# SrinivasBaskar1995/DistributedVolunteerComputing

Hardware: AMD Instinct MI355X
Metric: samples/sec GPT-2-small local-SGD (higher is better)
Workload: dtype bf16; 1 GPU; model=gpt2, global_batch=64, per_peer_batch=64, seq_len=1024, parallelism=local-sgd dp1 H=4 allreduce=direct

## Files before the change

distributedvolunteercomputing_amd/config.py:

```python
from __future__ import annotations

import contextlib
import dataclasses
import os
import threading


def _bool(s: str) -> bool:
    return s.strip().lower() in ("1", "true", "yes", "on")


@dataclasses.dataclass
class RuntimeConfig:
    gemm: str = "lib"
    mlp: str = "fused"
    narrow_gemm: str = "lib"
    mlp_grad_fwd: bool = True
    bwd_batch: bool = True
    fc_dgrad_nt: bool = True
    lmhead_dgrad_nt: bool = True
    gemm_fwd: str = "lib"
    dgrad_ps: bool = True
    gemm_wgrad: str = "vcx"
    wgrad_wide: bool = True
    wgrad_ragged: bool = False
    gemm_select: bool = False
    wgrad_big_split_min_m: int = 16384
    async_wgrad: bool = False
    lmhead_chunk: int = 0
    force_reference_ops: bool = False
    tunableop: str = "on"
    tunableop_file: str = ""
    offload_arch: str = "gfx950"
    colour_native: bool = True
    register_source: bool = True
    sink_gpu: bool = True
    resnet_conv1x1: str = "gemm"
    conv_find: bool = True
    resnet_bn: str = "fused"
    bn_layer_ws: bool = True
    conv3x3_wgrad: str = "vcx"
    conv3x3_fwd: str = "vcx"
    engine_batch: int = 2
    resnet_join: bool = True
    resnet_proj_join: bool = True
    gloo_host: str = "127.0.0.1"
    p2p_backend: str = ""
    elastic_debug: bool = False
    elastic_liveness: bool = True
    elastic_stage_joins: str = "gloo"
    uplink_pipeline: str = "relay"
    shared_source_root: str = ""
    store_port_train: int = 29611
    store_port_video: int = 29612
    trace_dir: str = ""
    metrics_dir: str = ""


_ENV = {
    "gemm": ("VCX_GEMM", str),
    "mlp": ("VCX_MLP", str),
    "dgrad_ps": ("VCX_DGRAD_PS", _bool),
    "mlp_grad_fwd": ("VCX_MLP_GRAD_FWD", _bool),
    "bwd_batch": ("VCX_BWD_BATCH", _bool),
    "fc_dgrad_nt": ("VCX_FC_DGRAD_NT", _bool),
    "lmhead_dgrad_nt": ("VCX_LMHEAD_DGRAD_NT", _bool),
    "narrow_gemm": ("VCX_NARROW_GEMM", str),
    "resnet_conv1x1": ("VCX_RESNET_CONV1X1", str),
    "resnet_bn": ("VCX_RESNET_BN", str),
    "resnet_join": ("VCX_RESNET_JOIN", _bool),
    "engine_batch": ("VCX_ENGINE_BATCH", int),
    "conv3x3_wgrad": ("VCX_CONV3X3_WGRAD", str),
    "conv3x3_fwd": ("VCX_CONV3X3_FWD", str),
    "resnet_proj_join": ("VCX_RESNET_PROJ_JOIN", _bool),
    "bn_layer_ws": ("VCX_BN_LAYER_WS", _bool),
    "conv_find": ("VCX_CONV_FIND", _bool),
    "gemm_wgrad": ("VCX_GEMM_WGRAD", str),
    "gemm_fwd": ("VCX_GEMM_FWD", str),
    "wgrad_wide": ("VCX_WGRAD_WIDE", _bool),
    "wgrad_ragged": ("VCX_WGRAD_RAGGED", _bool),
    "gemm_select": ("VCX_GEMM_SELECT", _bool),
    "wgrad_big_split_min_m": ("VCX_WGRAD_BIG_SPLIT_MIN_M", int),
    "async_wgrad": ("VCX_ASYNC_WGRAD", _bool),
    "lmhead_chunk": ("VCX_LMHEAD_CHUNK", int),
    "force_reference_ops": ("VCX_FORCE_REFERENCE_OPS", _bool),
    "tunableop": ("VCX_TUNABLEOP", str),
    "tunableop_file": ("VCX_TUNABLEOP_FILE", str),
    "offload_arch": ("VCX_OFFLOAD_ARCH", str),
    "colour_native": ("VCX_COLOUR_NATIVE", _bool),
    "register_source": ("VCX_REGISTER_SOURCE", _bool),
    "sink_gpu": ("VCX_SINK_GPU", _bool),
    "gloo_host": ("VCX_GLOO_HOST", str),
    "p2p_backend": ("VCX_P2P_BACKEND", str),
    "elastic_debug": ("VCX_ELASTIC_DEBUG", _bool),
    "elastic_liveness": ("VCX_ELASTIC_LIVENESS", _bool),
    "elastic_stage_joins": ("VCX_ELASTIC_STAGE_JOINS", str),
    "uplink_pipeline": ("VCX_UPLINK_PIPELINE", str),
    "shared_source_root": ("VCX_SHARED_SOURCE_ROOT", str),
    "store_port_train": ("VCX_STORE_PORT", int),
    "store_port_video": ("VCX_STORE_PORT", int),
    "trace_dir": ("VCX_TRACE_DIR", str),
    "metrics_dir": ("VCX_METRICS_DIR", str),
}
_CHOICES = {"narrow_gemm": ("lib", "vision"), "conv3x3_wgrad": ("lib", "vcx"), "conv3x3_fwd": ("lib", "vcx"), "gemm": ("lib", "vcx"), "mlp": ("fused", "lib"), "gemm_wgrad": ("lib", "vcx"), "gemm_fwd": ("lib", "vcx"), "tunableop": ("on", "off"), "p2p_backend": ("", "gloo", "nccl"), "elastic_stage_joins": ("gloo", "off"),
            "uplink_pipeline": ("relay", "all", "off")}

_lock = threading.Lock()


def _validate(cfg: RuntimeConfig):
    for k, allowed in _CHOICES.items():
        if getattr(cfg, k) not in allowed:
            raise ValueError(f"config.{k} must be one of {allowed}, not {getattr(cfg, k)!r}")


def from_env(env=None) -> RuntimeConfig:
    env = os.environ if env is None else env
    cfg = RuntimeConfig()
    for field, (var, parse) in _ENV.items():
        if var in env and env[var] != "":
            try:
                setattr(cfg, field, parse(env[var]))
            except ValueError as e:
                raise ValueError(f"{var}={env[var]!r}: {e}") from None
    _validate(cfg)
    return cfg


_CONFIG = from_env()


def get() -> RuntimeConfig:
    return _CONFIG


def update(**kw) -> RuntimeConfig:
    with _lock:
        unknown = set(kw) - {f.name for f in dataclasses.fields(RuntimeConfig)}
        if unknown:
            raise AttributeError(f"unknown config fields: {sorted(unknown)}")
        new = dataclasses.replace(_CONFIG, **kw)
        _validate(new)
        for k, v in kw.items():
            setattr(_CONFIG, k, v)
    return _CONFIG


@contextlib.contextmanager
def override(**kw):
    old = {k: getattr(_CONFIG, k) for k in kw}
    update(**kw)
    try:
        yield _CONFIG
    finally:
        update(**old)


def describe() -> str:
    rows = []
    for f in dataclasses.fields(RuntimeConfig):
        var = _ENV.get(f.name, ("", None))[0]
        rows.append(f"{f.name:24s} {var:28s} {getattr(_CONFIG, f.name)!r}")
    return "\n".join(rows)
```

distributedvolunteercomputing_amd/csrc/bindings.cpp:

```cpp
#include <torch/extension.h>
#include <map>
#include <mutex>
#include <thread>
#include <tuple>
#include <c10/hip/HIPStream.h>
#include <hip/hip_runtime.h>

#include "kernels/vcx_api.h"

namespace {

hipStream_t cur_stream() { return c10::hip::getCurrentHIPStream().stream(); }

#define CHECK_CUDA(x) TORCH_CHECK((x).is_cuda(), #x " must be a GPU tensor")
#define CHECK_CONTIG(x) TORCH_CHECK((x).is_contiguous(), #x " must be contiguous")
#define CHECK_DT(x, dt) TORCH_CHECK((x).scalar_type() == (dt), #x " has wrong dtype ", (x).scalar_type())
#define CHECK_IN(x, dt) \
  CHECK_CUDA(x);        \
  CHECK_CONTIG(x);      \
  CHECK_DT(x, dt)

const auto kBF = at::kBFloat16;
const auto kF = at::kFloat;

void* opt_ptr(const c10::optional<at::Tensor>& t) { return t.has_value() ? t->data_ptr() : nullptr; }

void grad_sumsq(at::Tensor g, at::Tensor ostate) {
  CHECK_IN(g, kBF);
  CHECK_IN(ostate, kF);
  TORCH_CHECK(g.numel() % 8 == 0, "flat buffer length must be a multiple of 8");
  vcx_grad_sumsq(g.data_ptr(), g.numel(), ostate.data_ptr<float>(), cur_stream());
}

void adam_prologue(at::Tensor ostate, double max_norm) {
  CHECK_IN(ostate, kF);
  TORCH_CHECK(ostate.numel() >= 4);
  vcx_adam_prologue(ostate.data_ptr<float>(), (float)max_norm, cur_stream());
}

void adamw_flat(at::Tensor param, at::Tensor grad, at::Tensor master, at::Tensor m, at::Tensor v, int64_t n_decay,
                at::Tensor ostate, double beta1, double beta2, double eps, double wd) {
  CHECK_IN(param, kBF);
  CHECK_IN(grad, kBF);
  CHECK_IN(master, kF);
  CHECK_IN(m, kF);
  CHECK_IN(v, kF);
  CHECK_IN(ostate, kF);
  const int64_t n = param.numel();
  TORCH_CHECK(n % 8 == 0 && grad.numel() == n && master.numel() == n && m.numel() == n && v.numel() == n,
              "adamw_flat: buffers must share a length that is a multiple of 8");
  TORCH_CHECK(n_decay >= 0 && n_decay <= n && n_decay % 8 == 0);
  vcx_adamw_flat(param.data_ptr(), grad.data_ptr(), master.data_ptr<float>(), m.data_ptr<float>(),
                 v.data_ptr<float>(), n, n_decay, ostate.data_ptr<float>(), (float)beta1, (float)beta2, (float)eps,
                 (float)wd, cur_stream());
}

void check_compact(at::Tensor m_code, at::Tensor m_exp, at::Tensor v_half, at::Tensor v_exp, int64_t n,
                   const char* who) {
  CHECK_IN(m_code, at::kByte);
  CHECK_IN(m_exp, at::kByte);
  CHECK_IN(v_half, at::kHalf);
  CHECK_IN(v_exp, at::kByte);
  TORCH_CHECK(n % 32 == 0 && m_code.numel() == n && v_half.numel() == n && m_exp.numel() == n / 32 &&
                  v_exp.numel() == n / 32,
              who, ": a state of n elements (a multiple of 32) has n codes, n halves and n / 32 bytes of each exponent");
}

void adamw_flat_compact(at::Tensor param, at::Tensor grad, at::Tensor master, at::Tensor m_code, at::Tensor m_exp,
                        at::Tensor v_half, at::Tensor v_exp, int64_t n_decay, at::Tensor ostate, double beta1,
                        double beta2, double eps, double wd) {
  CHECK_IN(param, kBF);
  CHECK_IN(grad, kBF);
  CHECK_IN(master, kF);
  CHECK_IN(ostate, kF);
  const int64_t n = param.numel();
  TORCH_CHECK(grad.numel() == n && master.numel() == n, "adamw_flat_compact: buffers must share a length");
  check_compact(m_code, m_exp, v_half, v_exp, n, "adamw_flat_compact");
  TORCH_CHECK(ostate.numel() >= 4);
  TORCH_CHECK(n_decay >= 0 && n_decay <= n && n_decay % 8 == 0);
  vcx_adamw_flat_compact(param.data_ptr(), grad.data_ptr(), master.data_ptr<float>(), m_code.data_ptr<uint8_t>(),
                         m_exp.data_ptr<uint8_t>(), v_half.data_ptr(), v_exp.data_ptr<uint8_t>(), n, n_decay,
                         ostate.data_ptr<float>(), beta1, beta2, (float)eps, (float)wd, cur_stream());
}

void optstate_encode(at::Tensor m, at::Tensor v, at::Tensor m_code, at::Tensor m_exp, at::Tensor v_half,
                     at::Tensor v_exp) {
  CHECK_IN(m, kF);
  CHECK_IN(v, kF);
  const int64_t n = m.numel();
  TORCH_CHECK(v.numel() == n, "optstate_encode: m and v must share a length");
  check_compact(m_code, m_exp, v_half, v_exp, n, "optstate_encode");
  vcx_optstate_encode(m.data_ptr<float>(), v.data_ptr<float>(), m_code.data_ptr<uint8_t>(), m_exp.data_ptr<uint8_t>(),
                      v_half.data_ptr(), v_exp.data_ptr<uint8_t>(), n, cur_stream());
}

void optstate_decode(at::Tensor m_code, at::Tensor m_exp, at::Tensor v_half, at::Tensor v_exp, at::Tensor m,
                     at::Tensor v) {
  CHECK_IN(m, kF);
  CHECK_IN(v, kF);
  const int64_t n = m.numel();
  TORCH_CHECK(v.numel() == n, "optstate_decode: m and v must share a length");
  check_compact(m_code, m_exp, v_half, v_exp, n, "optstate_decode");
  vcx_optstate_decode(m_code.data_ptr<uint8_t>(), m_exp.data_ptr<uint8_t>(), v_half.data_ptr(),
                      v_exp.data_ptr<uint8_t>(), m.data_ptr<float>(), v.data_ptr<float>(), n, cur_stream());
}

void lsgd_delta(at::Tensor master, at::Tensor anchor, at::Tensor delta) {
  CHECK_IN(master, kF);
  CHECK_IN(anchor, kF);
  CHECK_IN(delta, kBF);
  const int64_t n = master.numel();
  TORCH_CHECK(n % 8 == 0 && anchor.numel() == n && delta.numel() == n);
  vcx_lsgd_delta(master.data_ptr<float>(), anchor.data_ptr<float>(), delta.data_ptr(), n, cur_stream());
}

void lsgd_apply(at::Tensor avg, at::Tensor anchor, at::Tensor master, at::Tensor param,
                c10::optional<at::Tensor> mom, double outer_lr, double mu, bool nesterov, double avg_scale) {
  CHECK_IN(avg, kBF);
  CHECK_IN(anchor, kF);
  CHECK_IN(master, kF);
  CHECK_IN(param, kBF);
  const int64_t n = avg.numel();
  TORCH_CHECK(n % 8 == 0 && anchor.numel() == n && master.numel() == n && param.numel() == n);
  if (mom.has_value()) {
    CHECK_IN((*mom), kF);
    TORCH_CHECK(mom->numel() == n);
  }
  vcx_lsgd_apply(avg.data_ptr(), anchor.data_ptr<float>(), master.data_ptr<float>(), param.data_ptr(),
                 mom.has_value() ? mom->data_ptr<float>() : nullptr, n, (float)outer_lr, (float)mu, nesterov ? 1 : 0,
                 (float)avg_scale, cur_stream());
}

void f32_to_bf16(at::Tensor src, at::Tensor dst) {
  CHECK_IN(src, kF);
  CHECK_IN(dst, kBF);
  TORCH_CHECK(src.numel() == dst.numel() && src.numel() % 8 == 0);
  vcx_f32_to_bf16(src.data_ptr<float>(), dst.data_ptr(), src.numel(), cur_stream());
}

bool gemm_nt_supported(int64_t M, int64_t N, int64_t K) { return vcx_gemm_nt_supported((int)M, (int)N, (int)K); }
bool gemm_nt_supported_epi(int64_t M, int64_t N, int64_t K, int64_t epi) {
  return vcx_gemm_nt_supported_epi((int)M, (int)N, (int)K, (int)epi);
}

void gemm_nt(at::Tensor a, at::Tensor b, at::Tensor c, c10::optional<at::Tensor> c2, c10::optional<at::Tensor> bias,
             c10::optional<at::Tensor> colsum, int64_t epi) {
  TORCH_CHECK(a.is_cuda() && a.dim() == 2 && b.dim() == 2 && c.dim() == 2, "gemm_nt: 2-D cuda tensors");
  TORCH_CHECK(a.scalar_type() == at::kBFloat16 && b.scalar_type() == at::kBFloat16 && c.scalar_type() == at::kBFloat16,
              "gemm_nt: bf16 operands");
  TORCH_CHECK(a.stride(1) == 1 && b.stride(1) == 1 && c.stride(1) == 1, "gemm_nt: K-contiguous rows");
  const int64_t M = a.size(0), K = a.size(1), N = b.size(0);
  TORCH_CHECK(b.size(1) == K && c.size(0) == M && c.size(1) == N, "gemm_nt: shape mismatch");
  TORCH_CHECK(vcx_gemm_nt_supported_epi((int)M, (int)N, (int)K, (int)epi),
              "gemm_nt: needs N % 256 == 0, K % 64 == 0, K >= 128, and M % 256 == 0 for epilogues 2/3");
  TORCH_CHECK(a.stride(0) % 8 == 0 && b.stride(0) % 8 == 0 && c.stride(0) % 8 == 0, "gemm_nt: 16-B aligned rows");
  for (const at::Tensor* t : {&a, &b, &c})
    TORCH_CHECK(reinterpret_cast<uintptr_t>(t->data_ptr()) % 16 == 0, "gemm_nt: 16-B aligned base pointers");
  TORCH_CHECK(epi >= 0 && epi <= 4, "gemm_nt: epilogue 0..4");
  void* c2p = nullptr;
  if (epi == 2 || epi == 3) {
    TORCH_CHECK(c2 && c2->sizes() == c.sizes() && c2->strides() == c.strides() && c2->scalar_type() == at::kBFloat16,
                "gemm_nt: epilogue 2/3 needs c2 like c");
    TORCH_CHECK(reinterpret_cast<uintptr_t>(c2->data_ptr()) % 16 == 0, "gemm_nt: 16-B aligned c2");
    c2p = c2->data_ptr();
  }
  const void* bp = nullptr;
  if (epi == 1 || epi == 2 || epi == 4) {
    TORCH_CHECK(bias && bias->numel() == N && bias->is_contiguous() && bias->scalar_type() == at::kBFloat16,
                "gemm_nt: bias [N] bf16");
    bp = bias->data_ptr();
  }
  float* cs = nullptr;
  if (epi == 3) {
    TORCH_CHECK(colsum && colsum->numel() == N && colsum->scalar_type() == at::kFloat && colsum->is_contiguous(),
                "gemm_nt: colsum [N] fp32");
    cs = colsum->data_ptr<float>();
  }
  vcx_gemm_nt(a.data_ptr(), b.data_ptr(), c.data_ptr(), c2p, bp, cs, (int)M, (int)N, (int)K, (int)a.stride(0),
              (int)b.stride(0), (int)c.stride(0), (int)epi, cur_stream());
}


bool gemm_ps_supported(int64_t M, int64_t N, int64_t K, int64_t epi) {
  return vcx_gemm_ps_supported((int)M, (int)N, (int)K, (int)epi);
}

void gemm_ps(at::Tensor a, at::Tensor b, at::Tensor c, c10::optional<at::Tensor> c2, c10::optional<at::Tensor> bias,
             c10::optional<at::Tensor> colsum, int64_t epi, int64_t grid_cap) {
  TORCH_CHECK(a.is_cuda() && a.dim() == 2 && b.dim() == 2 && c.dim() == 2, "gemm_ps: 2-D cuda tensors");
  TORCH_CHECK(a.scalar_type() == at::kBFloat16 && b.scalar_type() == at::kBFloat16 && c.scalar_type() == at::kBFloat16,
              "gemm_ps: bf16 operands");
  TORCH_CHECK(a.stride(1) == 1 && b.stride(1) == 1 && c.stride(1) == 1, "gemm_ps: K-contiguous rows");
  const int64_t M = a.size(0), K = a.size(1), N = b.size(0);
  TORCH_CHECK(b.size(1) == K && c.size(0) == M && c.size(1) == N, "gemm_ps: shape mismatch");
  TORCH_CHECK(vcx_gemm_ps_supported((int)M, (int)N, (int)K, (int)epi),
              "gemm_ps: needs M, N % 256 == 0, K % 128 == 0, K >= 256, epilogue 0 (store), 1 (bias), 2 (bias+GELU), "
              "4 (DGELU + bias grad), 5 (bias+GELU, c = gelu'(pre)) or 6 (c = acc * c2 + bias grad), N <= 16384 with "
              "a bias");
  TORCH_CHECK(a.stride(0) % 8 == 0 && b.stride(0) % 8 == 0 && c.stride(0) % 8 == 0, "gemm_ps: 16-B aligned rows");
  for (const at::Tensor* t : {&a, &b, &c})
    TORCH_CHECK(reinterpret_cast<uintptr_t>(t->data_ptr()) % 16 == 0, "gemm_ps: 16-B aligned base pointers");
  TORCH_CHECK(256 * std::max({a.stride(0), b.stride(0), c.stride(0)}) * 2 < (int64_t(1) << 31), "gemm_ps: rows too long");
  void* c2p = nullptr;
  if (epi == 2 || epi == 4 || epi == 5 || epi == 6) {
    TORCH_CHECK(c2 && c2->sizes() == c.sizes() && c2->strides() == c.strides() && c2->scalar_type() == at::kBFloat16,
                "gemm_ps: epilogues 2/4/5/6 need c2 like c");
    TORCH_CHECK(reinterpret_cast<uintptr_t>(c2->data_ptr()) % 16 == 0, "gemm_ps: 16-B aligned c2");
    c2p = c2->data_ptr();
  }
  const void* bp = nullptr;
  if (epi == 1 || epi == 2 || epi == 5) {
    TORCH_CHECK(bias && bias->numel() == N && bias->is_contiguous() && bias->scalar_type() == at::kBFloat16,
                "gemm_ps: bias [N] bf16");
    TORCH_CHECK(reinterpret_cast<uintptr_t>(bias->data_ptr()) % 16 == 0, "gemm_ps: 16-B aligned bias");
    bp = bias->data_ptr();
  }
  float* cs = nullptr;
  if (epi == 4 || epi == 6) {
    TORCH_CHECK(colsum && colsum->numel() == N && colsum->scalar_type() == at::kFloat && colsum->is_contiguous(),
                "gemm_ps: colsum [N] fp32");
    cs = colsum->data_ptr<float>();
  }
  vcx_gemm_ps(a.data_ptr(), b.data_ptr(), c.data_ptr(), c2p, bp, cs, (int)M, (int)N, (int)K, (int)a.stride(0),
              (int)b.stride(0), (int)c.stride(0), (int)epi, (int)grid_cap, cur_stream());
}

static float* bn_workspace(const at::Tensor& x, int64_t C) {
  static std::mutex mu;
  static auto* cache = new std::map<std::tuple<int, uintptr_t, int64_t, size_t>, at::Tensor>();
  const auto key = std::make_tuple((int)x.get_device(), (uintptr_t)cur_stream(), C,
                                   std::hash<std::thread::id>{}(std::this_thread::get_id()));
  std::lock_guard<std::mutex> lk(mu);
  auto it = cache->find(key);
  if (it == cache->end()) {
    hipStreamCaptureStatus cs = hipStreamCaptureStatusNone;
    TORCH_CHECK(hipStreamIsCapturing(cur_stream(), &cs) == hipSuccess && cs == hipStreamCaptureStatusNone,
                "bn: first call of this width on this stream/thread inside a graph capture; run one eager step first");
    it = cache->emplace(key, at::zeros({2 * C}, x.options().dtype(at::kFloat))).first;
  }
  return it->second.data_ptr<float>();
}

static float* check_layer_ws(const c10::optional<at::Tensor>& lws, const at::Tensor& x, int64_t C) {
  if (!lws || !lws->defined()) return nullptr;
  TORCH_CHECK(lws->is_cuda() && lws->get_device() == x.get_device() && lws->scalar_type() == at::kFloat &&
                  lws->is_contiguous() && lws->numel() == 4 * C, "bn: layer workspace fp32 [4C] on x's device");
  return lws->data_ptr<float>();
}

std::vector<at::Tensor> bn_fwd_train(at::Tensor x, c10::optional<at::Tensor> res, at::Tensor gamma, at::Tensor beta,
                                     c10::optional<at::Tensor> run_mean, c10::optional<at::Tensor> run_var, double eps,
                                     double momentum, bool relu, c10::optional<at::Tensor> nbt,
                                     c10::optional<at::Tensor> layer_ws) {
  TORCH_CHECK(x.is_cuda() && x.is_contiguous() && x.scalar_type() == at::kBFloat16, "bn: x bf16 contiguous NHWC");
  const int64_t C = x.size(-1), R = x.numel() / C;
  TORCH_CHECK(vcx_bn_supported((int)C) && R > 0, "bn: C must be a power of two in 8..2048");
  TORCH_CHECK(gamma.numel() == C && beta.numel() == C && gamma.scalar_type() == at::kBFloat16 &&
                  beta.scalar_type() == at::kBFloat16 && gamma.is_contiguous() && beta.is_contiguous(), "bn: gamma/beta bf16 [C]");
  if (res) TORCH_CHECK(res->sizes() == x.sizes() && res->is_contiguous() && res->scalar_type() == at::kBFloat16, "bn: residual like x");
  void *rm = nullptr, *rv = nullptr;
  int fp32 = 0;
  if (run_mean && run_mean->defined()) {
    TORCH_CHECK(run_var && run_mean->numel() == C && run_var->numel() == C && run_mean->is_contiguous() &&
                    run_var->is_contiguous() && run_mean->scalar_type() == run_var->scalar_type() &&
                    (run_mean->scalar_type() == at::kBFloat16 || run_mean->scalar_type() == at::kFloat), "bn: running stats [C]");
    rm = run_mean->data_ptr();
    rv = run_var->data_ptr();
    fp32 = run_mean->scalar_type() == at::kFloat;
  }
  int64_t* nb = nullptr;
  if (nbt && nbt->defined()) {
    TORCH_CHECK(nbt->is_cuda() && nbt->scalar_type() == at::kLong && nbt->numel() == 1 && nbt->get_device() == x.get_device(),
                "bn: num_batches_tracked int64 [1] on x's device");
    nb = nbt->data_ptr<int64_t>();
  }
  auto f = x.options().dtype(at::kFloat);
  at::Tensor st = at::empty({4, C}, f);
  at::Tensor y = at::empty_like(x);
  at::Tensor mask = relu ? at::empty({R, C / 8}, x.options().dtype(at::kByte)) : at::Tensor();
  float* lws = check_layer_ws(layer_ws, x, C);
  vcx_bn_fwd_train(x.data_ptr(), res ? res->data_ptr() : nullptr, y.data_ptr(), relu ? mask.data_ptr() : nullptr, R,
                   (int)C, gamma.data_ptr(), beta.data_ptr(), rm, rv, fp32, (float)eps, (float)momentum,
                   lws ? lws : bn_workspace(x, C), st[0].data_ptr<float>(), st[1].data_ptr<float>(),
                   st[2].data_ptr<float>(), st[3].data_ptr<float>(), nb, relu ? 1 : 0, lws ? 1 : 0, cur_stream());
  return {y, st[0], st[1], st[2], mask};
}

std::vector<at::Tensor> maxpool3s2_fwd(at::Tensor x) {
  TORCH_CHECK(x.is_cuda() && x.dim() == 4 && x.is_contiguous() && x.scalar_type() == at::kBFloat16 && x.size(3) % 8 == 0 &&
                  x.size(1) >= 1 && x.size(2) >= 1, "maxpool3s2: x bf16 contiguous NHWC, C % 8 == 0");
  const int64_t N = x.size(0), H = x.size(1), W = x.size(2), C = x.size(3);
  TORCH_CHECK(N * H * W * C < (1ll << 40) && H < (1 << 20) && W < (1 << 20), "maxpool3s2: size");
  const int64_t OH = (H - 1) / 2 + 1, OW = (W - 1) / 2 + 1;
  at::Tensor y = at::empty({N, OH, OW, C}, x.options());
  at::Tensor idx = at::empty({N, OH, OW, C}, x.options().dtype(at::kByte));
  vcx_maxpool3s2_fwd(x.data_ptr(), y.data_ptr(), idx.data_ptr(), (int)N, (int)H, (int)W, (int)C, (int)OH, (int)OW,
                     cur_stream());
  return {y, idx};
}

at::Tensor maxpool3s2_bwd(at::Tensor dy, at::Tensor idx, int64_t H, int64_t W) {
  TORCH_CHECK(dy.is_cuda() && dy.dim() == 4 && dy.is_contiguous() && dy.scalar_type() == at::kBFloat16 &&
                  idx.sizes() == dy.sizes() && idx.is_contiguous() && idx.scalar_type() == at::kByte &&
                  idx.get_device() == dy.get_device() && dy.size(3) % 8 == 0, "maxpool3s2_bwd: dy bf16 / idx u8 NHWC alike");
  const int64_t N = dy.size(0), OH = dy.size(1), OW = dy.size(2), C = dy.size(3);
  TORCH_CHECK(OH == (H - 1) / 2 + 1 && OW == (W - 1) / 2 + 1, "maxpool3s2_bwd: input size does not match");
  at::Tensor dx = at::empty({N, H, W, C}, dy.options());
  vcx_maxpool3s2_bwd(dy.data_ptr(), idx.data_ptr(), dx.data_ptr(), (int)N, (int)H, (int)W, (int)C, (int)OH, (int)OW,
                     cur_stream());
  return dx;
}

static void nhwc_check(const at::Tensor& t, const char* what) {
  TORCH_CHECK(t.is_cuda() && t.dim() == 4 && t.is_contiguous() && t.scalar_type() == at::kBFloat16 && t.size(3) % 8 == 0 &&
                  reinterpret_cast<uintptr_t>(t.data_ptr()) % 16 == 0 && t.numel() < (1ll << 40),
              what, ": bf16 contiguous NHWC [N, H, W, C], C % 8 == 0, 16-B aligned");
}

at::Tensor subsample_nhwc(at::Tensor x, int64_t s) {
  nhwc_check(x, "subsample_nhwc");
  TORCH_CHECK(s >= 1 && s <= 8, "subsample_nhwc: stride 1..8");
  const int64_t N = x.size(0), H = x.size(1), W = x.size(2), C = x.size(3);
  at::Tensor y = at::empty({N, (H - 1) / s + 1, (W - 1) / s + 1, C}, x.options());
  if (y.numel()) vcx_subsample_nhwc(x.data_ptr(), y.data_ptr(), (int)N, (int)H, (int)W, (int)C, (int)s, cur_stream());
  return y;
}

void subsample_add_nhwc(at::Tensor full, at::Tensor g, int64_t s) {
  nhwc_check(full, "subsample_add_nhwc");
  nhwc_check(g, "subsample_add_nhwc");
  TORCH_CHECK(s >= 1 && s <= 8 && full.get_device() == g.get_device(), "subsample_add_nhwc: stride 1..8, one device");
  const int64_t N = full.size(0), H = full.size(1), W = full.size(2), C = full.size(3);
  TORCH_CHECK(g.size(0) == N && g.size(1) == (H - 1) / s + 1 && g.size(2) == (W - 1) / s + 1 && g.size(3) == C,
              "subsample_add_nhwc: g must be [N, ceil(H / s), ceil(W / s), C]");
  if (g.numel()) vcx_subsample_add_nhwc(full.data_ptr(), g.data_ptr(), (int)N, (int)H, (int)W, (int)C, (int)s, cur_stream());
}

at::Tensor bcast_hw_nhwc(at::Tensor g, int64_t H, int64_t W, double scale) {
  TORCH_CHECK(g.is_cuda() && g.dim() == 2 && g.is_contiguous() && g.scalar_type() == at::kBFloat16 && g.size(1) % 8 == 0 &&
                  reinterpret_cast<uintptr_t>(g.data_ptr()) % 16 == 0 && H >= 1 && W >= 1,
              "bcast_hw_nhwc: g bf16 contiguous [N, C], C % 8 == 0");
  const int64_t N = g.size(0), C = g.size(1);
  TORCH_CHECK(N * H * W * C < (1ll << 40), "bcast_hw_nhwc: size");
  at::Tensor out = at::empty({N, H, W, C}, g.options());
  if (out.numel()) vcx_bcast_hw_nhwc(g.data_ptr(), out.data_ptr(), (int)N, (int)(H * W), (int)C, (float)scale, cur_stream());
  return out;
}

at::Tensor bn_apply(at::Tensor x, c10::optional<at::Tensor> res, at::Tensor scale, at::Tensor shift, bool relu) {
  TORCH_CHECK(x.is_cuda() && x.is_contiguous() && x.scalar_type() == at::kBFloat16, "bn: x bf16 contiguous NHWC");
  const int64_t C = x.size(-1), R = x.numel() / C;
  TORCH_CHECK(vcx_bn_supported((int)C), "bn: C must be a power of two in 8..2048");
  TORCH_CHECK(scale.numel() == C && shift.numel() == C && scale.scalar_type() == at::kFloat &&
                  shift.scalar_type() == at::kFloat && scale.is_contiguous() && shift.is_contiguous(), "bn: scale/shift fp32 [C]");
  if (res) TORCH_CHECK(res->sizes() == x.sizes() && res->is_contiguous() && res->scalar_type() == at::kBFloat16, "bn: residual like x");
  at::Tensor y = at::empty_like(x);
  vcx_bn_apply(x.data_ptr(), res ? res->data_ptr() : nullptr, y.data_ptr(), R, (int)C, scale.data_ptr<float>(),
               shift.data_ptr<float>(), relu ? 1 : 0, cur_stream());
  return y;
}

std::vector<at::Tensor> bn_bwd(at::Tensor dy, c10::optional<at::Tensor> mask, at::Tensor x, at::Tensor mean, at::Tensor rstd,
                               at::Tensor scale, bool relu, bool want_dres, c10::optional<at::Tensor> gw,
                               c10::optional<at::Tensor> gb, c10::optional<at::Tensor> layer_ws) {
  TORCH_CHECK(dy.is_cuda() && dy.is_contiguous() && x.is_contiguous() && dy.sizes() == x.sizes() &&
                  dy.scalar_type() == at::kBFloat16 && x.scalar_type() == at::kBFloat16, "bn_bwd: dy, x bf16 NHWC alike");
  const int64_t C = x.size(-1), R = x.numel() / C;
  TORCH_CHECK(relu == (mask && mask->defined()), "bn_bwd: the ReLU mask with relu (and only then)");
  if (relu)
    TORCH_CHECK(mask->is_cuda() && mask->is_contiguous() && mask->scalar_type() == at::kByte &&
                    mask->numel() * 8 == R * C && mask->get_device() == x.get_device(), "bn_bwd: mask uint8 [R, C / 8]");
  TORCH_CHECK(vcx_bn_supported((int)C), "bn: C must be a power of two in 8..2048");
  for (const at::Tensor* t : {&mean, &rstd, &scale})
    TORCH_CHECK(t->numel() == C && t->scalar_type() == at::kFloat && t->is_contiguous(), "bn_bwd: stats fp32 [C]");
  const bool flat = gw && gw->defined();
  TORCH_CHECK(flat == (gb && gb->defined()), "bn_bwd: gw and gb together");
  if (flat)
    for (const at::Tensor* t : {&*gw, &*gb})
      TORCH_CHECK(t->is_cuda() && t->get_device() == x.get_device() && t->numel() == C && t->is_contiguous() &&
                      t->scalar_type() == at::kBFloat16, "bn_bwd: gradient buffers bf16 [C]");
  at::Tensor sums = at::empty({2 * C}, x.options().dtype(at::kFloat));
  at::Tensor dx = at::empty_like(x);
  at::Tensor dres = want_dres ? at::empty_like(x) : at::Tensor();
  float* lws = check_layer_ws(layer_ws, x, C);
  vcx_bn_bwd(dy.data_ptr(), relu ? mask->data_ptr() : nullptr, x.data_ptr(), mean.data_ptr<float>(), rstd.data_ptr<float>(),
             scale.data_ptr<float>(), R, (int)C, lws ? lws : bn_workspace(x, C), sums.data_ptr<float>(),
             flat ? gw->data_ptr() : nullptr, flat ? gb->data_ptr() : nullptr, dx.data_ptr(),
             want_dres ? dres.data_ptr() : nullptr, relu ? 1 : 0, lws ? 1 : 0, cur_stream());
  return {dx, dres, sums.narrow(0, C, C), sums.narrow(0, 0, C)};
}

bool gemm_wg_supported(int64_t M, int64_t N, int64_t K, int64_t splits) {
  return vcx_gemm_wg_supported((int)M, (int)N, (int)K, (int)(splits > 0 ? splits : vcx_gemm_wg_splits((int)M, (int)N, (int)K)));
}

void gemm_wg(at::Tensor a, at::Tensor b, at::Tensor out, bool accumulate, int64_t splits, int64_t loaders) {
  TORCH_CHECK(a.is_cuda() && a.dim() == 2 && b.dim() == 2 && out.dim() == 2, "gemm_wg: 2-D cuda tensors");
  TORCH_CHECK(a.scalar_type() == at::kBFloat16 && b.scalar_type() == at::kBFloat16 && out.scalar_type() == at::kBFloat16,
              "gemm_wg: bf16 operands");
  TORCH_CHECK(a.stride(1) == 1 && b.stride(1) == 1 && out.is_contiguous(), "gemm_wg: row-major operands, contiguous out");
  const int64_t K = a.size(0), M = a.size(1), N = b.size(1);
  TORCH_CHECK(b.size(0) == K && out.size(0) == M && out.size(1) == N, "gemm_wg: shape mismatch");
  if (splits <= 0) splits = vcx_gemm_wg_splits((int)M, (int)N, (int)K);
  TORCH_CHECK(vcx_gemm_wg_supported((int)M, (int)N, (int)K, (int)splits),
              "gemm_wg: needs M % 128 == 0, N % 256 == 0, K % 64 == 0, K / 192 >= splits, split panels under 2 GB");
  TORCH_CHECK(loaders == 4 || loaders == 8, "gemm_wg: loaders 4 or 8");
  TORCH_CHECK(a.stride(0) % 8 == 0 && b.stride(0) % 8 == 0, "gemm_wg: 16-B aligned rows");
  const int64_t tok = ((K / 64 + splits - 1) / splits) * 64;
  TORCH_CHECK(tok * std::max(a.stride(0), b.stride(0)) * 2 < (int64_t(1) << 31) - (int64_t(1) << 20),
              "gemm_wg: a split's operand panel must stay under 2 GB (more splits)");
  for (const at::Tensor* t : {&a, &b, &out})
    TORCH_CHECK(reinterpret_cast<uintptr_t>(t->data_ptr()) % 16 == 0, "gemm_wg: 16-B aligned base pointers");
  at::Tensor ws = at::empty({splits, M, N}, a.options().dtype(at::kFloat));
  vcx_gemm_wg(a.data_ptr(), b.data_ptr(), ws.data_ptr<float>(), out.data_ptr(), (int)M, (int)N, (int)K,
              (int)a.stride(0), (int)b.stride(0), (int)splits, accumulate ? 1 : 0, (int)loaders, cur_stream());
}

bool gemm_f_supported(int64_t M, int64_t N, int64_t K) { return vcx_gemm_f_supported((int)M, (int)N, (int)K); }

static std::pair<int, at::Tensor> f_splits(int64_t M, int64_t N, int64_t K, int64_t splits, const at::Tensor& like) {
  if (splits < 0) splits = vcx_gemm_f_splits((int)M, (int)N, (int)K);
  if (splits == 0) splits = 1;
  TORCH_CHECK(vcx_gemm_f_split_ok((int)M, (int)N, (int)K, (int)splits),
              "gemm_f: the K slices (K / 32) must split into even counts >= 6");
  at::Tensor ws = splits > 1 ? at::empty({splits, M, N}, like.options().dtype(at::kFloat)) : at::Tensor();
  return {(int)splits, ws};
}

int64_t gemm_f_splits(int64_t M, int64_t N, int64_t K) { return vcx_gemm_f_splits((int)M, (int)N, (int)K); }

void gemm_f(at::Tensor a, at::Tensor b, at::Tensor out, c10::optional<at::Tensor> bias, int64_t waves, int64_t splits) {
  TORCH_CHECK(a.is_cuda() && a.dim() == 2 && b.dim() == 2 && out.dim() == 2, "gemm_f: 2-D cuda tensors");
  TORCH_CHECK(a.scalar_type() == at::kBFloat16 && b.scalar_type() == at::kBFloat16 && out.scalar_type() == at::kBFloat16,
              "gemm_f: bf16 operands");
  TORCH_CHECK(a.stride(1) == 1 && b.stride(1) == 1 && out.stride(1) == 1, "gemm_f: row-major operands");
  const int64_t M = a.size(0), K = a.size(1), N = b.size(0);
  TORCH_CHECK(b.size(1) == K && out.size(0) == M && out.size(1) == N, "gemm_f: shape mismatch");
  TORCH_CHECK(vcx_gemm_f_supported((int)M, (int)N, (int)K), "gemm_f: needs N % 128 == 0 or N == 64, K % 64 == 0, K >= 192");
  TORCH_CHECK(a.stride(0) % 8 == 0 && b.stride(0) % 8 == 0 && out.stride(0) % 8 == 0, "gemm_f: 16-B aligned rows");
  for (const at::Tensor* t : {&a, &b, &out})
    TORCH_CHECK(reinterpret_cast<uintptr_t>(t->data_ptr()) % 16 == 0, "gemm_f: 16-B aligned base pointers");
  TORCH_CHECK(a.get_device() == b.get_device() && a.get_device() == out.get_device(), "gemm_f: one device");
  const bool hb = bias && bias->defined();
  if (hb)
    TORCH_CHECK(bias->is_cuda() && bias->get_device() == a.get_device() && bias->numel() == N && bias->is_contiguous() &&
                    bias->scalar_type() == at::kBFloat16 && reinterpret_cast<uintptr_t>(bias->data_ptr()) % 8 == 0,
                "gemm_f: bias bf16 [N], contiguous, 8-B aligned");
  TORCH_CHECK(256 * std::max(a.stride(0), b.stride(0)) * 2 < (int64_t(1) << 31), "gemm_f: tile panels under 2 GB");
  auto [ns, ws] = f_splits(M, N, K, splits, a);
  TORCH_CHECK(ns == 1 || out.stride(0) % 4 == 0, "gemm_f: split output rows 8-B aligned");
  vcx_gemm_f(a.data_ptr(), b.data_ptr(), out.data_ptr(), hb ? bias->data_ptr() : nullptr, (int)M, (int)N, (int)K, (int)a.stride(0), (int)b.stride(0),
             (int)out.stride(0), (int)waves, ns, ns > 1 ? ws.data_ptr<float>() : nullptr, cur_stream());
}

bool gemm_f_conv3x3_supported(int64_t imgs, int64_t H, int64_t W, int64_t Cin, int64_t Cout, int64_t stride) {
  return vcx_gemm_f_conv3x3_supported((int)imgs, (int)H, (int)W, (int)Cin, (int)Cout, (int)stride);
}

void gemm_f_conv3x3(at::Tensor x, at::Tensor w, at::Tensor out, int64_t stride, c10::optional<at::Tensor> bias,
                    int64_t waves, int64_t splits, bool flip_taps) {
  TORCH_CHECK(x.is_cuda() && x.dim() == 4 && (w.dim() == 4 || w.dim() == 3) && out.dim() == 4,
              "gemm_f_conv3x3: x [N, H, W, Cin], w [Cout, 3, 3, Cin] or [9, Cout, Cin], out [N, Ho, Wo, Cout] on the GPU");
  for (const at::Tensor* t : {&x, &w, &out}) {
    TORCH_CHECK(t->scalar_type() == at::kBFloat16 && t->is_contiguous() && t->get_device() == x.get_device(),
                "gemm_f_conv3x3: contiguous bf16 tensors on one device");
    TORCH_CHECK(reinterpret_cast<uintptr_t>(t->data_ptr()) % 16 == 0, "gemm_f_conv3x3: 16-B aligned base pointers");
  }
  const bool tap_major = w.dim() == 3;
  const int64_t imgs = x.size(0), H = x.size(1), W = x.size(2), Cin = x.size(3), Cout = tap_major ? w.size(1) : w.size(0);
  TORCH_CHECK(tap_major ? (w.size(0) == 9 && w.size(2) == Cin) : (w.size(1) == 3 && w.size(2) == 3 && w.size(3) == Cin),
              "gemm_f_conv3x3: w [Cout, 3, 3, Cin] or tap-major [9, Cout, Cin]");
  TORCH_CHECK(stride == 1 || stride == 2, "gemm_f_conv3x3: stride 1 or 2");
  const int64_t Ho = (H - 1) / stride + 1, Wo = (W - 1) / stride + 1;
  TORCH_CHECK(out.size(0) == imgs && out.size(1) == Ho && out.size(2) == Wo && out.size(3) == Cout,
              "gemm_f_conv3x3: out [N, Ho, Wo, Cout]");
  TORCH_CHECK(vcx_gemm_f_conv3x3_supported((int)imgs, (int)H, (int)W, (int)Cin, (int)Cout, (int)stride),
              "gemm_f_conv3x3: needs Cin a power of two >= 64, Cout % 128 == 0 or Cout == 64, x under 2 GB");
  const bool hb = bias && bias->defined();
  if (hb)
    TORCH_CHECK(bias->is_cuda() && bias->get_device() == x.get_device() && bias->numel() == Cout &&
                    bias->is_contiguous() && bias->scalar_type() == at::kBFloat16, "gemm_f_conv3x3: bias bf16 [Cout]");
  auto [ns, ws] = f_splits(imgs * Ho * Wo, Cout, 9 * Cin, splits, x);
  vcx_gemm_f_conv3x3(x.data_ptr(), w.data_ptr(), out.data_ptr(), hb ? bias->data_ptr() : nullptr, (int)imgs, (int)H,
                     (int)W, (int)Cin, (int)Cout, (int)stride, (int)waves, ns, ns > 1 ? ws.data_ptr<float>() : nullptr,
                     flip_taps ? 1 : 0, tap_major ? 1 : 0, cur_stream());
}

bool gemm_wg_conv3x3_supported(int64_t Cout, int64_t Cin, int64_t imgs, int64_t H, int64_t W, int64_t stride) {
  if (stride != 1 && stride != 2) return false;
  const int64_t tokens = imgs * ((H - 1) / stride + 1) * ((W - 1) / stride + 1);
  if (tokens >= (int64_t(1) << 31)) return false;
  const int splits = vcx_gemm_wg_splits((int)Cout, (int)(9 * Cin), (int)tokens);
  return vcx_gemm_wg_conv3x3_supported((int)Cout, (int)Cin, (int)tokens, imgs * H * W * Cin * 2, splits);
}

void gemm_wg_conv3x3(at::Tensor dy, at::Tensor x, at::Tensor out, bool accumulate, int64_t stride, int64_t splits) {
  TORCH_CHECK(dy.is_cuda() && x.is_cuda() && out.is_cuda() && dy.dim() == 4 && x.dim() == 4 && out.dim() == 2,
              "gemm_wg_conv3x3: dy [N, Ho, Wo, Cout], x [N, H, W, Cin], out [Cout, 9 Cin] on the GPU");
  TORCH_CHECK(dy.scalar_type() == at::kBFloat16 && x.scalar_type() == at::kBFloat16 && out.scalar_type() == at::kBFloat16,
              "gemm_wg_conv3x3: bf16");
  TORCH_CHECK(dy.is_contiguous() && x.is_contiguous() && out.is_contiguous(), "gemm_wg_conv3x3: contiguous NHWC");
  const int64_t imgs = x.size(0), H = x.size(1), W = x.size(2), Cin = x.size(3), Cout = dy.size(3);
  TORCH_CHECK(stride == 1 || stride == 2, "gemm_wg_conv3x3: stride 1 or 2");
  const int64_t Ho = (H - 1) / stride + 1, Wo = (W - 1) / stride + 1;
  TORCH_CHECK(dy.size(0) == imgs && dy.size(1) == Ho && dy.size(2) == Wo, "gemm_wg_conv3x3: dy / x shapes");
  TORCH_CHECK(out.size(0) == Cout && out.size(1) == 9 * Cin, "gemm_wg_conv3x3: out [Cout, 9 Cin]");
  const int64_t tokens = imgs * Ho * Wo;
  TORCH_CHECK(tokens < (int64_t(1) << 31), "gemm_wg_conv3x3: size");
  if (splits <= 0) splits = vcx_gemm_wg_splits((int)Cout, (int)(9 * Cin), (int)tokens);
  TORCH_CHECK(vcx_gemm_wg_conv3x3_supported((int)Cout, (int)Cin, (int)tokens, imgs * H * W * Cin * 2, (int)splits),
              "gemm_wg_conv3x3: needs Cout % 128 == 0, Cin % 128 == 0, N Ho Wo % 64 == 0, N Ho Wo / 192 >= splits, "
              "x under 2 GB");
  for (const at::Tensor* t : {&dy, &x, &out})
    TORCH_CHECK(reinterpret_cast<uintptr_t>(t->data_ptr()) % 16 == 0, "gemm_wg_conv3x3: 16-B aligned base pointers");
  at::Tensor ws = at::empty({splits, Cout, 9 * Cin}, dy.options().dtype(at::kFloat));
  vcx_gemm_wg_conv3x3(dy.data_ptr(), x.data_ptr(), ws.data_ptr<float>(), out.data_ptr(), (int)Cout, (int)Cin, (int)imgs,
                      (int)H, (int)W, (int)stride, (int)splits, accumulate ? 1 : 0, cur_stream());
}

at::Tensor transpose_bf16(at::Tensor src, c10::optional<at::Tensor> dst) {
  TORCH_CHECK(src.is_cuda() && src.dim() == 2 && src.is_contiguous() && src.scalar_type() == at::kBFloat16,
              "transpose_bf16: contiguous 2-D bf16");
  at::Tensor out = dst ? *dst : at::empty({src.size(1), src.size(0)}, src.options());
  TORCH_CHECK(out.size(0) == src.size(1) && out.size(1) == src.size(0) && out.is_contiguous(), "transpose_bf16: dst");
  vcx_transpose_bf16(src.data_ptr(), out.data_ptr(), (int)src.size(0), (int)src.size(1), cur_stream());
  return out;
}

std::tuple<std::vector<at::Tensor>, int64_t> transpose_bf16_many(std::vector<at::Tensor> srcs,
                                                                 c10::optional<std::vector<at::Tensor>> dsts) {
  TORCH_CHECK(!dsts || dsts->size() == srcs.size(), "transpose_bf16_many: one dst per src");
  std::vector<at::Tensor> outs;
  std::vector<vcx::TransposeJob> jobs;
  outs.reserve(srcs.size());
  jobs.reserve(srcs.size());
  for (size_t i = 0; i < srcs.size(); ++i) {
    const at::Tensor& src = srcs[i];
    TORCH_CHECK(src.is_cuda() && src.dim() == 2 && src.is_contiguous() && src.scalar_type() == at::kBFloat16 &&
                    src.get_device() == srcs[0].get_device() && src.size(0) <= INT32_MAX && src.size(1) <= INT32_MAX,
                "transpose_bf16_many: contiguous 2-D bf16 on one device");
    at::Tensor out = dsts ? (*dsts)[i] : at::empty({src.size(1), src.size(0)}, src.options());
    TORCH_CHECK(out.dim() == 2 && out.size(0) == src.size(1) && out.size(1) == src.size(0) && out.is_contiguous() &&
                    out.scalar_type() == at::kBFloat16 && out.is_cuda() && out.get_device() == src.get_device(),
                "transpose_bf16_many: dst");
    vcx::TransposeJob j{};
    j.src = src.data_ptr();
    j.dst = out.data_ptr();
    j.R = (int)src.size(0);
    j.Cc = (int)src.size(1);
    jobs.push_back(j);
    outs.push_back(std::move(out));
  }
  int launches = 0;
  if (!jobs.empty()) {
    launches = vcx_transpose_bf16_many(jobs.data(), (int)jobs.size(), cur_stream());
    TORCH_CHECK(launches >= 0, "transpose_bf16_many: a matrix of more than 2^31 tiles");
  }
  return {std::move(outs), (int64_t)launches};
}

void add_f32_into_bf16(at::Tensor in, at::Tensor out, bool accumulate, bool zero_in) {
  TORCH_CHECK(in.is_cuda() && in.scalar_type() == at::kFloat && out.scalar_type() == at::kBFloat16 &&
                  in.numel() == out.numel() && in.is_contiguous() && out.is_contiguous() &&
                  in.get_device() == out.get_device() && in.numel() < (int64_t(1) << 31),
              "add_f32_into_bf16: fp32 in, bf16 out of equal size on one device");
  vcx_add_f32_into_bf16(in.data_ptr<float>(), out.data_ptr(), (int)in.numel(), accumulate ? 1 : 0, zero_in ? 1 : 0,
                        cur_stream());
}

void reduce_bcast_bf16(at::Tensor in, c10::optional<at::Tensor> out, c10::optional<at::Tensor> mine, int64_t P) {
  TORCH_CHECK(in.is_cuda() && in.scalar_type() == at::kBFloat16 && in.is_contiguous(), "reduce_bcast: bf16 cuda in");
  const int64_t n = in.numel() / P;
  TORCH_CHECK(P > 0 && n * P == in.numel() && n % 8 == 0, "reduce_bcast: numel must be P * n with n % 8 == 0");
  if (out) TORCH_CHECK(out->numel() == in.numel() && out->is_contiguous() && out->scalar_type() == at::kBFloat16,
                       "reduce_bcast: out must match in");
  if (mine) TORCH_CHECK(mine->numel() == n && mine->is_contiguous() && mine->scalar_type() == at::kBFloat16,
                        "reduce_bcast: mine must hold n bf16");
  vcx_reduce_bcast_bf16(in.data_ptr(), opt_ptr(out), opt_ptr(mine), (int)P, n, cur_stream());
}

int64_t check_robust_rows(const char* who, const at::Tensor& in, int64_t P, int64_t live_mask,
                          const c10::optional<at::Tensor>& out, const c10::optional<at::Tensor>& mine) {
  TORCH_CHECK(in.is_cuda() && in.scalar_type() == at::kBFloat16 && in.is_contiguous(), who,
              ": in must be a contiguous bf16 GPU tensor");
  TORCH_CHECK(P >= 1 && P <= 16, who, ": P must be in 1..16, got ", P);
  TORCH_CHECK(live_mask > 0 && (live_mask >> P) == 0, who,
              ": live_mask must name at least one of the P rows and no other, got ", live_mask);
  const int64_t n = in.numel() / P;
  TORCH_CHECK(n * P == in.numel() && n % 8 == 0, who, ": numel must be P * n with n % 8 == 0");
  auto aligned = [](const at::Tensor& t, uintptr_t a) { return reinterpret_cast<uintptr_t>(t.data_ptr()) % a == 0; };
  TORCH_CHECK(aligned(in, 16), who, ": in must be 16-byte aligned");
  if (out)
    TORCH_CHECK(out->is_cuda() && out->get_device() == in.get_device() && out->numel() == in.numel() &&
                    out->is_contiguous() && out->scalar_type() == at::kBFloat16 && aligned(*out, 16),
                who, ": out must match in (bf16, same length, 16-byte aligned)");
  if (mine)
    TORCH_CHECK(mine->is_cuda() && mine->get_device() == in.get_device() && mine->numel() == n &&
                    mine->is_contiguous() && mine->scalar_type() == at::kBFloat16 && aligned(*mine, 16),
                who, ": mine must hold n bf16, 16-byte aligned");
  return n;
}

void trimmed_reduce_bcast_bf16(at::Tensor in, c10::optional<at::Tensor> out, c10::optional<at::Tensor> mine, int64_t P,
                               int64_t trim, int64_t live_mask, double inv, c10::optional<at::Tensor> counts) {
  const int64_t n = check_robust_rows("trimmed_reduce_bcast", in, P, live_mask, out, mine);
  TORCH_CHECK(trim >= 0, "trimmed_reduce_bcast: trim must be >= 0");
  if (counts)
    TORCH_CHECK(counts->is_cuda() && counts->get_device() == in.get_device() && counts->numel() == P &&
                    counts->is_contiguous() && counts->scalar_type() == at::kLong,
                "trimmed_reduce_bcast: counts must hold P int64 on in's device");
  vcx_trimmed_reduce_bcast_bf16(in.data_ptr(), opt_ptr(out), opt_ptr(mine), (int)P, n, (int)std::min<int64_t>(trim, 16),
                                (uint32_t)live_mask, (float)inv, counts ? counts->data_ptr<int64_t>() : nullptr,
                                cur_stream());
}

void cclip_reduce_bcast_bf16(at::Tensor in, c10::optional<at::Tensor> out, c10::optional<at::Tensor> mine, int64_t P,
                             int64_t live_mask, double tau, int64_t iters, c10::optional<at::Tensor> weights) {
  const int64_t n = check_robust_rows("cclip_reduce_bcast", in, P, live_mask, out, mine);
  TORCH_CHECK(tau >= 0.0 && tau <= 3.4028234663852886e38,
              "cclip_reduce_bcast: tau must be finite and >= 0 (0: adaptive), got ", tau);
  TORCH_CHECK(iters >= 1 && iters <= 8, "cclip_reduce_bcast: iters must be in 1..8, got ", iters);
  if (weights)
    TORCH_CHECK(weights->is_cuda() && weights->get_device() == in.get_device() && weights->numel() == P &&
                    weights->is_contiguous() && weights->scalar_type() == at::kFloat,
                "cclip_reduce_bcast: weights must hold P fp32 on in's device");
  at::Tensor ws = at::empty({vcx_cclip_workspace_floats((int)P, n)}, in.options().dtype(at::kFloat));
  vcx_cclip_reduce_bcast_bf16(in.data_ptr(), opt_ptr(out), opt_ptr(mine), (int)P, n, (uint32_t)live_mask, (float)tau,
                              (int)iters, weights ? weights->data_ptr<float>() : nullptr, ws.data_ptr<float>(),
                              cur_stream());
}

void axpy_bf16(at::Tensor src, at::Tensor acc, double scale) {
  CHECK_IN(src, kBF);
  CHECK_IN(acc, kBF);
  TORCH_CHECK(src.numel() == acc.numel() && src.numel() % 8 == 0);
  vcx_axpy_bf16(src.data_ptr(), acc.data_ptr(), src.numel(), (float)scale, cur_stream());
}

void splitk_reduce(at::Tensor part, at::Tensor acc, bool accumulate) {
  CHECK_IN(part, kBF);
  CHECK_IN(acc, kBF);
  const int64_t n = acc.numel();
  TORCH_CHECK(n % 8 == 0 && part.numel() % n == 0, "splitk_reduce: part must be [S, acc.numel()], numel % 8 == 0");
  vcx_splitk_reduce(part.data_ptr(), acc.data_ptr(), (int)(part.numel() / n), n, accumulate ? 1 : 0, cur_stream());
}

std::vector<at::Tensor> ln_fwd(at::Tensor a, c10::optional<at::Tensor> b, at::Tensor w, c10::optional<at::Tensor> bias,
                               double eps, bool rms, c10::optional<at::Tensor> bb) {
  CHECK_IN(a, kBF);
  CHECK_IN(w, kBF);
  const int C = (int)a.size(-1);
  const int64_t R = a.numel() / C;
  TORCH_CHECK(C % 8 == 0 && C <= 8192, "layernorm: C must be a multiple of 8 and <= 8192");
  TORCH_CHECK(w.numel() == C);
  TORCH_CHECK(R < INT32_MAX);
  if (b.has_value()) {
    CHECK_IN((*b), kBF);
    TORCH_CHECK(b->sizes() == a.sizes());
  }
  if (bias.has_value()) {
    CHECK_IN((*bias), kBF);
    TORCH_CHECK(bias->numel() == C);
  }
  if (bb.has_value()) {
    CHECK_IN((*bb), kBF);
    TORCH_CHECK(bb->numel() == C && b.has_value(), "branch bias needs a branch tensor");
  }
  auto y = at::empty_like(a);
  at::Tensor xout = b.has_value() ? at::empty_like(a) : a;
  auto mean = at::empty({R}, a.options().dtype(kF));
  auto rstd = at::empty({R}, a.options().dtype(kF));
  vcx_ln_fwd(a.data_ptr(), opt_ptr(b), b.has_value() ? xout.data_ptr() : nullptr, y.data_ptr(), w.data_ptr(),
             opt_ptr(bias), mean.data_ptr<float>(), rstd.data_ptr<float>(), (int)R, C, (float)eps, rms ? 1 : 0,
             opt_ptr(bb), cur_stream());
  return {y, xout, mean, rstd};
}

at::Tensor grad_out(const c10::optional<at::Tensor>& given, int64_t n, const at::Tensor& like, int* mask, int bit) {
  if (given.has_value()) {
    CHECK_IN((*given), kBF);
    TORCH_CHECK(given->numel() == n, "gradient output has the wrong size");
    *mask |= 1 << bit;
    return *given;
  }
  return at::empty({n}, like.options());
}

std::vector<at::Tensor> ln_bwd(at::Tensor dy, at::Tensor x, at::Tensor w, at::Tensor mean, at::Tensor rstd,
                               c10::optional<at::Tensor> dres, bool has_bias, bool rms, bool has_bb,
                               c10::optional<at::Tensor> dw_out, c10::optional<at::Tensor> db_out,
                               c10::optional<at::Tensor> dbb_out) {
  CHECK_IN(dy, kBF);
  CHECK_IN(x, kBF);
  CHECK_IN(w, kBF);
  CHECK_IN(mean, kF);
  CHECK_IN(rstd, kF);
  const int C = (int)x.size(-1);
  const int64_t R = x.numel() / C;
  TORCH_CHECK(C % 8 == 0 && C <= 8192 && dy.sizes() == x.sizes() && w.numel() == C);
  TORCH_CHECK(mean.numel() == R && rstd.numel() == R);
  if (dres.has_value()) {
    CHECK_IN((*dres), kBF);
    TORCH_CHECK(dres->sizes() == x.sizes());
  }
  const int P = vcx_ln_bwd_partials((int)R, C);
  auto dx = at::empty_like(x);
  auto dw_part = at::empty({P, C}, x.options().dtype(kF));
  int mask = 0;
  at::Tensor dw = grad_out(dw_out, C, x, &mask, 0);
  at::Tensor db_part, db;
  if (has_bias) {
    db_part = at::empty({P, C}, x.options().dtype(kF));
    db = grad_out(db_out, C, x, &mask, 1);
  }
  at::Tensor dbb_part, dbb;
  if (has_bb) {
    dbb_part = at::empty({P, C}, x.options().dtype(kF));
    dbb = grad_out(dbb_out, C, x, &mask, 2);
  }
  vcx_ln_bwd(dy.data_ptr(), x.data_ptr(), w.data_ptr(), mean.data_ptr<float>(), rstd.data_ptr<float>(),
             opt_ptr(dres), dx.data_ptr(), dw_part.data_ptr<float>(), has_bias ? db_part.data_ptr<float>() : nullptr,
             dw.data_ptr(), has_bias ? db.data_ptr() : nullptr, (int)R, C, rms ? 1 : 0,
             has_bb ? dbb_part.data_ptr<float>() : nullptr, has_bb ? dbb.data_ptr() : nullptr,
             at::empty({3 * VCX_COLSUM_NB * C}, x.options().dtype(kF)).data_ptr<float>(), mask, cur_stream());
  return {dx, dw, db, dbb};
}

at::Tensor colsum_bf16(at::Tensor y, c10::optional<at::Tensor> out) {
  CHECK_IN(y, kBF);
  const int64_t F = y.size(-1), R = y.numel() / F;
  TORCH_CHECK(F % 8 == 0 && R > 0 && R < INT32_MAX, "colsum_bf16: last dim must be a multiple of 8");
  int mask = 0;
  at::Tensor o = grad_out(out, F, y, &mask, 0);
  auto part = at::empty({vcx_bias_gelu_partials((int)R), F}, y.options().dtype(kF));
  auto stage = at::empty({VCX_COLSUM_NB * F}, y.options().dtype(kF));
  vcx_colsum_bf16(y.data_ptr(), part.data_ptr<float>(), o.data_ptr(), (int)R, (int)F, mask, stage.data_ptr<float>(),
                  cur_stream());
  return o;
}

at::Tensor bias_gelu_fwd(at::Tensor x, at::Tensor b) {
  CHECK_IN(x, kBF);
  CHECK_IN(b, kBF);
  const int64_t F = x.size(-1), R = x.numel() / F;
  TORCH_CHECK(F % 8 == 0 && b.numel() == F && R < INT32_MAX);
  auto y = at::empty_like(x);
  vcx_bias_gelu_fwd(x.data_ptr(), b.data_ptr(), y.data_ptr(), (int)R, (int)F, cur_stream());
  return y;
}

std::vector<at::Tensor> bias_gelu_bwd(at::Tensor x, at::Tensor b, at::Tensor dy, c10::optional<at::Tensor> db_out) {
  CHECK_IN(x, kBF);
  CHECK_IN(b, kBF);
  CHECK_IN(dy, kBF);
  const int64_t F = x.size(-1), R = x.numel() / F;
  TORCH_CHECK(F % 8 == 0 && b.numel() == F && dy.sizes() == x.sizes() && R < INT32_MAX);
  auto dx = at::empty_like(x);
  auto part = at::empty({vcx_bias_gelu_partials((int)R), F}, x.options().dtype(kF));
  int mask = 0;
  auto db = grad_out(db_out, F, x, &mask, 0);
  auto stage = at::empty({VCX_COLSUM_NB * F}, x.options().dtype(kF));
  vcx_bias_gelu_bwd(x.data_ptr(), b.data_ptr(), dy.data_ptr(), dx.data_ptr(), part.data_ptr<float>(), db.data_ptr(),
                    (int)R, (int)F, stage.data_ptr<float>(), mask, cur_stream());
  return {dx, db};
}

at::Tensor gelu_fwd(at::Tensor x) {
  CHECK_IN(x, kBF);
  TORCH_CHECK(x.numel() % 8 == 0);
  auto y = at::empty_like(x);
  vcx_gelu_fwd(x.data_ptr(), y.data_ptr(), x.numel(), cur_stream());
  return y;
}

at::Tensor gelu_bwd(at::Tensor x, at::Tensor dy) {
  CHECK_IN(x, kBF);
  CHECK_IN(dy, kBF);
  TORCH_CHECK(x.numel() % 8 == 0 && dy.numel() == x.numel());
  auto dx = at::empty_like(x);
  vcx_gelu_bwd(x.data_ptr(), dy.data_ptr(), dx.data_ptr(), x.numel(), cur_stream());
  return dx;
}

at::Tensor swiglu_fwd(at::Tensor gu) {
  CHECK_IN(gu, kBF);
  const int64_t F2 = gu.size(-1);
  TORCH_CHECK(F2 % 16 == 0, "swiglu: feature dim must be a multiple of 16");
  const int64_t R = gu.numel() / F2;
  auto sizes = gu.sizes().vec();
  sizes.back() = F2 / 2;
  auto y = at::empty(sizes, gu.options());
  vcx_swiglu_fwd(gu.data_ptr(), y.data_ptr(), R, (int)(F2 / 2), cur_stream());
  return y;
}

at::Tensor swiglu_bwd(at::Tensor gu, at::Tensor dy) {
  CHECK_IN(gu, kBF);
  CHECK_IN(dy, kBF);
  const int64_t F2 = gu.size(-1);
  TORCH_CHECK(F2 % 16 == 0 && dy.numel() * 2 == gu.numel());
  auto dgu = at::empty_like(gu);
  vcx_swiglu_bwd(gu.data_ptr(), dy.data_ptr(), dgu.data_ptr(), gu.numel() / F2, (int)(F2 / 2), cur_stream());
  return dgu;
}

std::vector<at::Tensor> xent_fwd(at::Tensor logits, at::Tensor tgt, int64_t V) {
  CHECK_IN(logits, kBF);
  CHECK_IN(tgt, at::kLong);
  TORCH_CHECK(logits.dim() == 2);
  const int64_t R = logits.size(0), Vp = logits.size(1);
  TORCH_CHECK(Vp % 8 == 0 && V <= Vp && V > 0 && tgt.numel() == R);
  auto lse = at::empty({R}, logits.options().dtype(kF));
  auto loss = at::empty({R}, logits.options().dtype(kF));
  vcx_xent_fwd(logits.data_ptr(), tgt.data_ptr<int64_t>(), lse.data_ptr<float>(), loss.data_ptr<float>(), R, (int)V,
               (int)Vp, cur_stream());
  return {loss, lse};
}

void xent_bwd(at::Tensor logits, at::Tensor tgt, at::Tensor lse, at::Tensor gscale, at::Tensor dlogits, int64_t V) {
  CHECK_IN(logits, kBF);
  CHECK_IN(tgt, at::kLong);
  CHECK_IN(lse, kF);
  CHECK_IN(gscale, kF);
  CHECK_IN(dlogits, kBF);
  const int64_t R = logits.size(0), Vp = logits.size(1);
  TORCH_CHECK(logits.dim() == 2 && dlogits.sizes() == logits.sizes() && tgt.numel() == R && lse.numel() == R);
  TORCH_CHECK(Vp % 8 == 0 && V <= Vp && gscale.numel() >= 1);
  vcx_xent_bwd(logits.data_ptr(), tgt.data_ptr<int64_t>(), lse.data_ptr<float>(), gscale.data_ptr<float>(),
               dlogits.data_ptr(), R, (int)V, (int)Vp, cur_stream());
}

c10::optional<at::Tensor> xent_fused(at::Tensor logits, at::Tensor tgt, at::Tensor nvalid, int64_t V) {
  CHECK_IN(logits, kBF);
  CHECK_IN(tgt, at::kLong);
  CHECK_IN(nvalid, kF);
  TORCH_CHECK(logits.dim() == 2);
  const int64_t R = logits.size(0), Vp = logits.size(1);
  TORCH_CHECK(Vp % 8 == 0 && V <= Vp && V > 0 && tgt.numel() == R && nvalid.numel() >= 1);
  auto loss = at::empty({R}, logits.options().dtype(kF));
  if (!vcx_xent_fused(logits.data_ptr(), tgt.data_ptr<int64_t>(), nvalid.data_ptr<float>(), loss.data_ptr<float>(), R,
                      (int)V, (int)Vp, cur_stream()))
    return c10::nullopt;
  return loss;
}

void xent_rescale(at::Tensor d, at::Tensor dloss) {
  CHECK_IN(d, kBF);
  CHECK_IN(dloss, kF);
  TORCH_CHECK(d.numel() % 8 == 0 && dloss.numel() >= 1);
  vcx_xent_rescale(d.data_ptr(), dloss.data_ptr<float>(), d.numel(), cur_stream());
}

at::Tensor embed_fwd(at::Tensor idx, at::Tensor wte, c10::optional<at::Tensor> wpe, int64_t T) {
  CHECK_IN(idx, at::kLong);
  CHECK_IN(wte, kBF);
  TORCH_CHECK(wte.dim() == 2 && wte.size(1) % 8 == 0);
  const int64_t R = idx.numel(), V = wte.size(0), C = wte.size(1);
  TORCH_CHECK(T > 0 && R % T == 0);
  if (wpe.has_value()) {
    CHECK_IN((*wpe), kBF);
    TORCH_CHECK(wpe->dim() == 2 && wpe->size(1) == C && wpe->size(0) >= T, "position table too short");
  }
  auto out = at::empty({R, C}, wte.options());
  vcx_embed_fwd(idx.data_ptr<int64_t>(), wte.data_ptr(), opt_ptr(wpe), out.data_ptr(), R, (int)T, (int)C, (int)V,
                cur_stream());
  return out;
}

std::vector<at::Tensor> embed_bwd(at::Tensor idx, at::Tensor dx, int64_t V, int64_t T, int64_t Tpos,
                                  c10::optional<at::Tensor> wte_grad, c10::optional<at::Tensor> wpe_grad) {
  CHECK_IN(idx, at::kLong);
  CHECK_IN(dx, kBF);
  const int64_t R = idx.numel(), C = dx.size(-1);
  TORCH_CHECK(dx.numel() == R * C && C % 8 == 0 && C <= 8192 && T > 0 && R % T == 0 && Tpos >= 0 && Tpos >= (Tpos ? T : 0));
  auto scratch = at::zeros({V, C}, dx.options().dtype(kF));
  at::Tensor dwte, dwpe;
  int acc_wte = 0, acc_wpe = 0;
  if (wte_grad.has_value()) {
    CHECK_IN((*wte_grad), kBF);
    TORCH_CHECK(wte_grad->numel() == V * C);
    dwte = *wte_grad;
    acc_wte = 1;
  } else {
    dwte = at::empty({V, C}, dx.options());
  }
  if (Tpos > 0) {
    if (wpe_grad.has_value()) {
      CHECK_IN((*wpe_grad), kBF);
      TORCH_CHECK(wpe_grad->numel() == Tpos * C);
      dwpe = *wpe_grad;
      acc_wpe = 1;
    } else {
      dwpe = at::zeros({Tpos, C}, dx.options());
    }
  }
  vcx_embed_bwd(idx.data_ptr<int64_t>(), dx.data_ptr(), scratch.data_ptr<float>(), dwte.data_ptr(), acc_wte,
                Tpos > 0 ? dwpe.data_ptr() : nullptr, acc_wpe, R, (int)T, (int)C, (int)V, cur_stream());
  return {dwte, dwpe};
}

std::vector<at::Tensor> rope_qkv_fwd(at::Tensor qkv, at::Tensor cosv, at::Tensor sinv, int64_t Hq, int64_t Hkv) {
  CHECK_IN(qkv, kBF);
  CHECK_IN(cosv, kF);
  CHECK_IN(sinv, kF);
  TORCH_CHECK(qkv.dim() == 3, "rope_qkv: qkv must be [B, T, (Hq + 2 Hkv) * D]");
  const int64_t B = qkv.size(0), T = qkv.size(1), W = qkv.size(2);
  TORCH_CHECK(Hq > 0 && Hkv > 0 && W % (Hq + 2 * Hkv) == 0);
  const int64_t D = W / (Hq + 2 * Hkv);
  TORCH_CHECK(D % 8 == 0, "rope_qkv: head dim must be a multiple of 8");
  TORCH_CHECK(cosv.dim() == 2 && cosv.size(0) >= T && cosv.size(1) == D / 2 && sinv.sizes() == cosv.sizes(),
              "rope_qkv: cos/sin tables must be [>= T, D/2]");
  auto q = at::empty({B, Hq, T, D}, qkv.options());
  auto k = at::empty({B, Hkv, T, D}, qkv.options());
  auto v = at::empty({B, Hkv, T, D}, qkv.options());
  vcx_rope_qkv(qkv.data_ptr(), q.data_ptr(), k.data_ptr(), v.data_ptr(), cosv.data_ptr<float>(),
               sinv.data_ptr<float>(), (int)B, (int)T, (int)Hq, (int)Hkv, (int)D, 0, cur_stream());
  return {q, k, v};
}

at::Tensor rope_qkv_bwd(at::Tensor dq, at::Tensor dk, at::Tensor dv, at::Tensor cosv, at::Tensor sinv) {
  CHECK_IN(dq, kBF);
  CHECK_IN(dk, kBF);
  CHECK_IN(dv, kBF);
  CHECK_IN(cosv, kF);
  CHECK_IN(sinv, kF);
  TORCH_CHECK(dq.dim() == 4 && dk.dim() == 4 && dk.sizes() == dv.sizes());
  const int64_t B = dq.size(0), Hq = dq.size(1), T = dq.size(2), D = dq.size(3), Hkv = dk.size(1);
  TORCH_CHECK(dk.size(0) == B && dk.size(2) == T && dk.size(3) == D && D % 8 == 0);
  TORCH_CHECK(cosv.size(0) >= T && cosv.size(1) == D / 2 && sinv.sizes() == cosv.sizes());
  auto dqkv = at::empty({B, T, (Hq + 2 * Hkv) * D}, dq.options());
  vcx_rope_qkv(dqkv.data_ptr(), dq.data_ptr(), dk.data_ptr(), dv.data_ptr(), cosv.data_ptr<float>(),
               sinv.data_ptr<float>(), (int)B, (int)T, (int)Hq, (int)Hkv, (int)D, 1, cur_stream());
  return dqkv;
}

std::vector<at::Tensor> attn_fwd(at::Tensor qkv, double scale) {
  CHECK_IN(qkv, kBF);
  TORCH_CHECK(qkv.dim() == 5 && qkv.size(2) == 3 && qkv.size(4) == 64, "attn_fwd: qkv must be [B, T, 3, H, 64]");
  const int64_t B = qkv.size(0), T = qkv.size(1), H = qkv.size(3);
  TORCH_CHECK(B * H * ((T + 127) / 128) < INT32_MAX && T > 0);
  auto out = at::empty({B, T, H, 64}, qkv.options());
  auto lse = at::empty({B, H, T}, qkv.options().dtype(kF));
  vcx_attn_fwd_d64(qkv.data_ptr(), out.data_ptr(), lse.data_ptr<float>(), (int)B, (int)T, (int)H, (float)scale,
                   cur_stream());
  return {out, lse};
}

at::Tensor attn_bwd(at::Tensor qkv, at::Tensor out, at::Tensor dout, at::Tensor lse, double scale) {
  CHECK_IN(qkv, kBF);
  CHECK_IN(out, kBF);
  CHECK_IN(dout, kBF);
  CHECK_IN(lse, kF);
  TORCH_CHECK(qkv.dim() == 5 && qkv.size(2) == 3 && qkv.size(4) == 64);
  const int64_t B = qkv.size(0), T = qkv.size(1), H = qkv.size(3);
  TORCH_CHECK(out.sizes() == at::IntArrayRef({B, T, H, 64}) && dout.sizes() == out.sizes());
  TORCH_CHECK(lse.numel() == B * H * T);
  auto dqkv = at::empty_like(qkv);
  auto delta = at::empty({B, H, T}, lse.options());
  vcx_attn_bwd_d64(qkv.data_ptr(), out.data_ptr(), dout.data_ptr(), lse.data_ptr<float>(), delta.data_ptr<float>(),
                   dqkv.data_ptr(), nullptr, (int)B, (int)T, (int)H, (float)scale, cur_stream());
  return dqkv;
}

std::vector<at::Tensor> attn_bwd_bias(at::Tensor qkv, at::Tensor out, at::Tensor dout, at::Tensor lse, double scale,
                                      c10::optional<at::Tensor> db_out) {
  CHECK_IN(qkv, kBF);
  CHECK_IN(out, kBF);
  CHECK_IN(dout, kBF);
  CHECK_IN(lse, kF);
  TORCH_CHECK(qkv.dim() == 5 && qkv.size(2) == 3 && qkv.size(4) == 64);
  const int64_t B = qkv.size(0), T = qkv.size(1), H = qkv.size(3), F = 3 * H * 64;
  TORCH_CHECK(out.sizes() == at::IntArrayRef({B, T, H, 64}) && dout.sizes() == out.sizes());
  TORCH_CHECK(lse.numel() == B * H * T);
  auto dqkv = at::empty_like(qkv);
  auto delta = at::empty({B, H, T}, lse.options());
  const int P = vcx_attn_bias_partials((int)B, (int)T);
  auto part = at::empty({P, F}, lse.options());
  int mask = 0;
  at::Tensor db = grad_out(db_out, F, qkv, &mask, 0);
  auto stage = at::empty({VCX_COLSUM_NB * F}, lse.options());
  vcx_attn_bwd_d64(qkv.data_ptr(), out.data_ptr(), dout.data_ptr(), lse.data_ptr<float>(), delta.data_ptr<float>(),
                   dqkv.data_ptr(), part.data_ptr<float>(), (int)B, (int)T, (int)H, (float)scale, cur_stream());
  vcx_colsum_f32(part.data_ptr<float>(), db.data_ptr(), P, (int)F, mask, stage.data_ptr<float>(), cur_stream());
  return {dqkv, db};
}

static void check_hm(const at::Tensor& q, const at::Tensor& k, const at::Tensor& v) {
  CHECK_IN(q, kBF);
  CHECK_IN(k, kBF);
  CHECK_IN(v, kBF);
  TORCH_CHECK(q.dim() == 4 && k.dim() == 4 && k.sizes() == v.sizes(), "attn_hm: q [B,Hq,T,D], k/v [B,Hkv,T,D]");
  TORCH_CHECK(q.size(0) == k.size(0) && q.size(2) == k.size(2) && q.size(3) == k.size(3));
  TORCH_CHECK(q.size(3) == 64 || q.size(3) == 128, "attn_hm: head dim must be 64 or 128");
  TORCH_CHECK(q.size(1) % k.size(1) == 0, "attn_hm: Hq must be a multiple of Hkv");
}

std::vector<at::Tensor> attn_hm_fwd(at::Tensor q, at::Tensor k, at::Tensor v, double scale) {
  check_hm(q, k, v);
  const int64_t B = q.size(0), Hq = q.size(1), T = q.size(2), D = q.size(3), Hkv = k.size(1);
  auto out = at::empty({B, T, Hq, D}, q.options());
  auto lse = at::empty({B, Hq, T}, q.options().dtype(kF));
  vcx_attn_hm_fwd(q.data_ptr(), k.data_ptr(), v.data_ptr(), out.data_ptr(), lse.data_ptr<float>(), (int)B, (int)T,
                  (int)Hq, (int)Hkv, (int)D, (float)scale, cur_stream());
  return {out, lse};
}

std::vector<at::Tensor> attn_hm_bwd(at::Tensor q, at::Tensor k, at::Tensor v, at::Tensor out, at::Tensor dout,
                                    at::Tensor lse, double scale) {
  check_hm(q, k, v);
  CHECK_IN(out, kBF);
  CHECK_IN(dout, kBF);
  CHECK_IN(lse, kF);
  const int64_t B = q.size(0), Hq = q.size(1), T = q.size(2), D = q.size(3), Hkv = k.size(1);
  TORCH_CHECK(out.sizes() == at::IntArrayRef({B, T, Hq, D}) && dout.sizes() == out.sizes());
  TORCH_CHECK(lse.numel() == B * Hq * T);
  auto dq = at::empty_like(q), dk = at::empty_like(k), dv = at::empty_like(v);
  auto delta = at::empty({B, Hq, T}, lse.options());
  vcx_attn_hm_bwd(q.data_ptr(), k.data_ptr(), v.data_ptr(), out.data_ptr(), dout.data_ptr(), lse.data_ptr<float>(),
                  delta.data_ptr<float>(), dq.data_ptr(), dk.data_ptr(), dv.data_ptr(), (int)B, (int)T, (int)Hq,
                  (int)Hkv, (int)D, (float)scale, cur_stream());
  return {dq, dk, dv};
}

}

void vcx_register_vision(pybind11::module& m);
void vcx_register_compress(pybind11::module& m);
void vcx_register_lt(pybind11::module& m);
extern "C" const char* vcx_source_digest();

PYBIND11_MODULE(_C, m) {
  m.doc() = "gfx950 HIP kernels of distributedvolunteercomputing_amd";
  m.def("source_digest", [] { return std::string(vcx_source_digest()); });
  m.def("grad_sumsq", &grad_sumsq);
  m.def("adam_prologue", &adam_prologue);
  m.def("adamw_flat", &adamw_flat);
  m.def("adamw_flat_compact", &adamw_flat_compact);
  m.def("optstate_encode", &optstate_encode);
  m.def("optstate_decode", &optstate_decode);
  m.def("lsgd_delta", &lsgd_delta);
  m.def("lsgd_apply", &lsgd_apply);
  m.def("f32_to_bf16", &f32_to_bf16);
  m.def("axpy_bf16", &axpy_bf16);
  m.def("reduce_bcast_bf16", &reduce_bcast_bf16);
  m.def("trimmed_reduce_bcast_bf16", &trimmed_reduce_bcast_bf16);
  m.def("cclip_reduce_bcast_bf16", &cclip_reduce_bcast_bf16);
  m.def("cclip_max_workgroups", &vcx_cclip_max_workgroups);
  m.def("gemm_nt_supported", &gemm_nt_supported);
  m.def("gemm_nt_supported_epi", &gemm_nt_supported_epi);
  m.def("gemm_ps_supported", &gemm_ps_supported);
  m.def("bn_supported", [](int64_t C) { return vcx_bn_supported((int)C); });
  m.def("bn_fwd_train", &bn_fwd_train, py::arg("x"), py::arg("res"), py::arg("gamma"), py::arg("beta"),
        py::arg("run_mean"), py::arg("run_var"), py::arg("eps"), py::arg("momentum"), py::arg("relu"),
        py::arg("nbt") = py::none(), py::arg("layer_ws") = py::none());
  m.def("bn_apply", &bn_apply);
  m.def("maxpool3s2_fwd", &maxpool3s2_fwd);
  m.def("maxpool3s2_bwd", &maxpool3s2_bwd);
  m.def("bn_bwd", &bn_bwd, py::arg("dy"), py::arg("mask"), py::arg("x"), py::arg("mean"), py::arg("rstd"), py::arg("scale"),
        py::arg("relu"), py::arg("want_dres"), py::arg("gw") = py::none(), py::arg("gb") = py::none(),
        py::arg("layer_ws") = py::none());
  m.def("gemm_ps", &gemm_ps, py::arg("a"), py::arg("b"), py::arg("c"), py::arg("c2") = py::none(),
        py::arg("bias") = py::none(), py::arg("colsum") = py::none(), py::arg("epi") = 0, py::arg("grid_cap") = 0);
  m.def("gemm_f_supported", &gemm_f_supported, py::arg("M"), py::arg("N"), py::arg("K"));
  m.def("gemm_f_conv3x3_supported", &gemm_f_conv3x3_supported, py::arg("imgs"), py::arg("H"), py::arg("W"),
        py::arg("Cin"), py::arg("Cout"), py::arg("stride"));
  m.def("gemm_f_conv3x3", &gemm_f_conv3x3, py::arg("x"), py::arg("w"), py::arg("out"), py::arg("stride"),
        py::arg("bias") = py::none(), py::arg("waves") = 0, py::arg("splits") = -1, py::arg("flip_taps") = false);
  m.def("gemm_f_splits", &gemm_f_splits, py::arg("M"), py::arg("N"), py::arg("K"));
  m.def("gemm_f", &gemm_f, py::arg("a"), py::arg("b"), py::arg("out"), py::arg("bias") = py::none(),
        py::arg("waves") = 0, py::arg("splits") = -1);
  m.def("gemm_wg_supported", &gemm_wg_supported, py::arg("M"), py::arg("N"), py::arg("K"), py::arg("splits") = 0);
  m.def("gemm_wg_conv3x3_supported", &gemm_wg_conv3x3_supported, py::arg("Cout"), py::arg("Cin"), py::arg("imgs"),
        py::arg("H"), py::arg("W"), py::arg("stride"));
  m.def("gemm_wg_conv3x3", &gemm_wg_conv3x3, py::arg("dy"), py::arg("x"), py::arg("out"), py::arg("accumulate") = false,
        py::arg("stride") = 1, py::arg("splits") = 0);
  m.def("gemm_wg", &gemm_wg, py::arg("a"), py::arg("b"), py::arg("out"), py::arg("accumulate") = false,
        py::arg("splits") = 0, py::arg("loaders") = 8);
  m.def("gemm_nt", &gemm_nt, py::arg("a"), py::arg("b"), py::arg("c"), py::arg("c2") = py::none(),
        py::arg("bias") = py::none(), py::arg("colsum") = py::none(), py::arg("epi") = 0);
  m.def("transpose_bf16", &transpose_bf16, py::arg("src"), py::arg("dst") = py::none());
  m.def("transpose_bf16_many", &transpose_bf16_many, py::arg("srcs"), py::arg("dsts") = py::none());
  m.attr("JOB_TABLE_CAP") = (int64_t)vcx::JOBS_MAX;
  m.def("subsample_nhwc", &subsample_nhwc, py::arg("x"), py::arg("stride"));
  m.def("subsample_add_nhwc", &subsample_add_nhwc, py::arg("full"), py::arg("g"), py::arg("stride"));
  m.def("bcast_hw_nhwc", &bcast_hw_nhwc, py::arg("g"), py::arg("H"), py::arg("W"), py::arg("scale"));
  m.def("add_f32_into_bf16", &add_f32_into_bf16, py::arg("src"), py::arg("out"), py::arg("accumulate"),
        py::arg("zero_src") = false);
  m.def("splitk_reduce", &splitk_reduce);
  m.def("ln_fwd", &ln_fwd);
  m.def("ln_bwd", &ln_bwd, pybind11::arg("dy"), pybind11::arg("x"), pybind11::arg("w"), pybind11::arg("mean"),
        pybind11::arg("rstd"), pybind11::arg("dres"), pybind11::arg("has_bias"), pybind11::arg("rms"),
        pybind11::arg("has_bb"), pybind11::arg("dw_out") = pybind11::none(), pybind11::arg("db_out") = pybind11::none(),
        pybind11::arg("dbb_out") = pybind11::none());
  m.def("colsum_bf16", &colsum_bf16, pybind11::arg("y"), pybind11::arg("out") = pybind11::none());
  m.def("gelu_fwd", &gelu_fwd);
  m.def("bias_gelu_fwd", &bias_gelu_fwd);
  m.def("bias_gelu_bwd", &bias_gelu_bwd, pybind11::arg("x"), pybind11::arg("b"), pybind11::arg("dy"),
        pybind11::arg("db_out") = pybind11::none());
  m.def("gelu_bwd", &gelu_bwd);
  m.def("swiglu_fwd", &swiglu_fwd);
  m.def("swiglu_bwd", &swiglu_bwd);
  m.def("xent_fwd", &xent_fwd);
  m.def("xent_bwd", &xent_bwd);
  m.def("xent_fused", &xent_fused);
  m.def("xent_rescale", &xent_rescale);
  m.def("embed_fwd", &embed_fwd);
  m.def("embed_bwd", &embed_bwd, pybind11::arg("idx"), pybind11::arg("dx"), pybind11::arg("V"), pybind11::arg("T"),
        pybind11::arg("Tpos"), pybind11::arg("wte_grad") = pybind11::none(), pybind11::arg("wpe_grad") = pybind11::none());
  m.def("attn_fwd", &attn_fwd);
  m.def("attn_set_variant", &vcx_attn_set_variant, pybind11::arg("fwd_wpe"), pybind11::arg("fwd_dma"),
        pybind11::arg("bwd_dma"), pybind11::arg("stage_epi") = -1);
  m.def("rope_qkv_fwd", &rope_qkv_fwd);
  m.def("rope_qkv_bwd", &rope_qkv_bwd);
  m.def("attn_bwd", &attn_bwd);
  m.def("attn_hm_fwd", &attn_hm_fwd);
  m.def("attn_hm_bwd", &attn_hm_bwd);
  m.def("attn_hm_set_variant", &vcx_attn_hm_set_variant);
  m.def("attn_bwd_bias", &attn_bwd_bias, pybind11::arg("qkv"), pybind11::arg("out"), pybind11::arg("dout"),
        pybind11::arg("lse"), pybind11::arg("scale"), pybind11::arg("db_out") = pybind11::none());
  vcx_register_vision(m);
  vcx_register_compress(m);
  vcx_register_lt(m);
}
```

distributedvolunteercomputing_amd/csrc/kernels/norm_act.hip:

```cpp
#include <algorithm>
#include <cstdlib>
#include <type_traits>

#include "vcx_api.h"
#include "vcx_common.h"

namespace vcx {

template <int CH>
__global__ void __launch_bounds__(256) ln_fwd_kernel(const bf16* __restrict__ a, const bf16* __restrict__ b,
                                                      bf16* __restrict__ xout, bf16* __restrict__ y,
                                                      const bf16* __restrict__ w, const bf16* __restrict__ bias,
                                                      float* __restrict__ mean_out, float* __restrict__ rstd_out,
                                                      int R, int C, float eps, int rms, const bf16* __restrict__ bb) {
  const int lane = threadIdx.x & 63;
  const int row = blockIdx.x * 4 + (threadIdx.x >> 6);
  if (row >= R) return;
  const int C8 = C >> 3;
  const int64_t off = (int64_t)row * C;
  float v[CH][8];
  float sum = 0.f;
#pragma unroll
  for (int k = 0; k < CH; ++k) {
    const int c = lane + k * 64;
    if (c < C8) {
      bf16x8 av = *(const bf16x8*)(a + off + c * 8);
      if (b) {
        bf16x8 bv = *(const bf16x8*)(b + off + c * 8);
        bf16x8 s;
        float bias_b[8] = {0.f, 0.f, 0.f, 0.f, 0.f, 0.f, 0.f, 0.f};
        if (bb) {
          bf16x8 t = *(const bf16x8*)(bb + c * 8);
#pragma unroll
          for (int j = 0; j < 8; ++j) bias_b[j] = (float)t[j];
        }
#pragma unroll
        for (int j = 0; j < 8; ++j) {
          s[j] = (bf16)((float)av[j] + ((float)bv[j] + bias_b[j]));
          v[k][j] = (float)s[j];
        }
        *(bf16x8*)(xout + off + c * 8) = s;
      } else {
#pragma unroll
        for (int j = 0; j < 8; ++j) v[k][j] = (float)av[j];
      }
#pragma unroll
      for (int j = 0; j < 8; ++j) sum += v[k][j];
    }
  }
  const float invC = 1.f / (float)C;
  float mean = rms ? 0.f : wave_sum(sum) * invC;
  float var = 0.f;
#pragma unroll
  for (int k = 0; k < CH; ++k) {
    const int c = lane + k * 64;
    if (c < C8) {
#pragma unroll
      for (int j = 0; j < 8; ++j) {
        float d = v[k][j] - mean;
        var = fmaf(d, d, var);
      }
    }
  }
  var = wave_sum(var) * invC;
  const float rstd = rsqrtf(var + eps);
#pragma unroll
  for (int k = 0; k < CH; ++k) {
    const int c = lane + k * 64;
    if (c < C8) {
      bf16x8 wv = *(const bf16x8*)(w + c * 8);
      bf16x8 o;
      if (bias) {
        bf16x8 bv = *(const bf16x8*)(bias + c * 8);
#pragma unroll
        for (int j = 0; j < 8; ++j) o[j] = (bf16)fmaf((v[k][j] - mean) * rstd, (float)wv[j], (float)bv[j]);
      } else {
#pragma unroll
        for (int j = 0; j < 8; ++j) o[j] = (bf16)((v[k][j] - mean) * rstd * (float)wv[j]);
      }
      *(bf16x8*)(y + off + c * 8) = o;
    }
  }
  if (lane == 0) {
    mean_out[row] = mean;
    rstd_out[row] = rstd;
  }
}

template <int Q>
__global__ void __launch_bounds__(256) ln_fwd4_kernel(const bf16* __restrict__ a, const bf16* __restrict__ b,
                                                       bf16* __restrict__ xout, bf16* __restrict__ y,
                                                       const bf16* __restrict__ w, const bf16* __restrict__ bias,
                                                       float* __restrict__ mean_out, float* __restrict__ rstd_out,
                                                       int R, int C, float eps, int rms, const bf16* __restrict__ bb) {
  const int lane = threadIdx.x & 63;
  const int nw = gridDim.x * 4, gw = blockIdx.x * 4 + (threadIdx.x >> 6);
  float wv[Q][4], bv_[Q][4], bbv[Q][4];
#pragma unroll
  for (int k = 0; k < Q; ++k) {
    const int c = k * 256 + lane * 4;
    const bf16x4 t = *(const bf16x4*)(w + c);
    const bf16x4 u = bias ? *(const bf16x4*)(bias + c) : bf16x4{};
    const bf16x4 v = bb ? *(const bf16x4*)(bb + c) : bf16x4{};
#pragma unroll
    for (int j = 0; j < 4; ++j) {
      wv[k][j] = (float)t[j];
      bv_[k][j] = bias ? (float)u[j] : 0.f;
      bbv[k][j] = bb ? (float)v[j] : 0.f;
    }
  }
  const float invC = 1.f / (float)C;
  bf16x4 av[Q], bvv[Q];
  auto load_row = [&](int row, bf16x4(&aa)[Q], bf16x4(&bbx)[Q]) {
    const int64_t off = (int64_t)row * C + lane * 4;
#pragma unroll
    for (int k = 0; k < Q; ++k) {
      aa[k] = *(const bf16x4*)(a + off + k * 256);
      if (b) bbx[k] = *(const bf16x4*)(b + off + k * 256);
    }
  };
  if (gw < R) load_row(gw, av, bvv);
  for (int row = gw; row < R; row += nw) {
    bf16x4 nav[Q], nbv[Q];
    const int nxt = row + nw;
    if (nxt < R) load_row(nxt, nav, nbv);
    const int64_t off = (int64_t)row * C + lane * 4;
    float v[Q][4];
    float sum = 0.f;
#pragma unroll
    for (int k = 0; k < Q; ++k) {
      if (b) {
        bf16x4 sres;
#pragma unroll
        for (int j = 0; j < 4; ++j) {
          sres[j] = (bf16)((float)av[k][j] + ((float)bvv[k][j] + bbv[k][j]));
          v[k][j] = (float)sres[j];
        }
        *(bf16x4*)(xout + off + k * 256) = sres;
      } else {
#pragma unroll
        for (int j = 0; j < 4; ++j) v[k][j] = (float)av[k][j];
      }
#pragma unroll
      for (int j = 0; j < 4; ++j) sum += v[k][j];
    }
    const float mean = rms ? 0.f : wave_sum(sum) * invC;
    float var = 0.f;
#pragma unroll
    for (int k = 0; k < Q; ++k)
#pragma unroll
      for (int j = 0; j < 4; ++j) {
        const float d = v[k][j] - mean;
        var = fmaf(d, d, var);
      }
    const float rstd = rsqrtf(wave_sum(var) * invC + eps);
#pragma unroll
    for (int k = 0; k < Q; ++k) {
      bf16x4 o;
#pragma unroll
      for (int j = 0; j < 4; ++j) o[j] = (bf16)fmaf((v[k][j] - mean) * rstd, wv[k][j], bv_[k][j]);
      *(bf16x4*)(y + off + k * 256) = o;
    }
    if (lane == 0) {
      mean_out[row] = mean;
      rstd_out[row] = rstd;
    }
#pragma unroll
    for (int k = 0; k < Q; ++k) {
      av[k] = nav[k];
      if (b) bvv[k] = nbv[k];
    }
  }
}

template <int CH, bool RES, int VEC>
__global__ void __launch_bounds__(256) __attribute__((amdgpu_waves_per_eu(VEC == 4 ? 3 : 1))) ln_bwd_kernel(const bf16* __restrict__ dy, const bf16* __restrict__ x,
                                                      const bf16* __restrict__ w, const float* __restrict__ mean_in,
                                                      const float* __restrict__ rstd_in,
                                                      const bf16* __restrict__ dres, bf16* __restrict__ dx,
                                                      float* __restrict__ dw_part, float* __restrict__ db_part,
                                                      int R, int C, int rms, float* __restrict__ dbb_part) {
  const int lane = threadIdx.x & 63;
  const int gw = blockIdx.x * 4 + (threadIdx.x >> 6);
  const int nw = gridDim.x * 4;
  using BV = std::conditional_t<VEC == 8, bf16x8, bf16x4>;
  const int C8 = C / VEC;
  const float invC = 1.f / (float)C;
  float dwacc[CH][VEC], dbacc[CH][VEC], wreg[CH][VEC], dxacc[CH][VEC];
#pragma unroll
  for (int k = 0; k < CH; ++k) {
    const int c = lane + k * 64;
#pragma unroll
    for (int j = 0; j < VEC; ++j) {
      dwacc[k][j] = 0.f;
      dbacc[k][j] = 0.f;
      wreg[k][j] = 0.f;
      dxacc[k][j] = 0.f;
    }
    if (c < C8) {
      BV wv = *(const BV*)(w + c * VEC);
#pragma unroll
      for (int j = 0; j < VEC; ++j) wreg[k][j] = (float)wv[j];
    }
  }
  BV cd[CH], cx[CH], cr[CH];
  float cmean = 0.f, crstd = 0.f;
  auto load = [&](int row, BV(&d)[CH], BV(&xv)[CH], BV(&rv)[CH], float& mu, float& rs) {
    const int64_t off = (int64_t)row * C;
    mu = mean_in[row];
    rs = rstd_in[row];
#pragma unroll
    for (int k = 0; k < CH; ++k) {
      const int c = lane + k * 64;
      if (c < C8) {
        d[k] = *(const BV*)(dy + off + c * VEC);
        xv[k] = *(const BV*)(x + off + c * VEC);
        if (RES) rv[k] = *(const BV*)(dres + off + c * VEC);
      }
    }
  };
  if (gw < R) load(gw, cd, cx, cr, cmean, crstd);
  for (int row = gw; row < R; row += nw) {
    BV nd[CH], nx[CH], nr[CH];
    float nmean = 0.f, nrstd = 0.f;
    if (row + nw < R) load(row + nw, nd, nx, nr, nmean, nrstd);
    const int64_t off = (int64_t)row * C;
    float s1 = 0.f, s2 = 0.f;
#pragma unroll
    for (int k = 0; k < CH; ++k) {
      const int c = lane + k * 64;
      if (c < C8) {
#pragma unroll
        for (int j = 0; j < VEC; ++j) {
          const float d = (float)cd[k][j];
          const float xh = ((float)cx[k][j] - cmean) * crstd;
          const float g = d * wreg[k][j];
          s1 += g;
          s2 = fmaf(g, xh, s2);
          dwacc[k][j] = fmaf(d, xh, dwacc[k][j]);
          dbacc[k][j] += d;
        }
      }
    }
    s1 = rms ? 0.f : wave_sum(s1) * invC;
    s2 = wave_sum(s2) * invC;
    const float k2 = crstd * crstd * s2, mk2 = cmean * k2;
#pragma unroll
    for (int k = 0; k < CH; ++k) {
      const int c = lane + k * 64;
      if (c < C8) {
        BV o;
#pragma unroll
        for (int j = 0; j < VEC; ++j) {
          const float gs = fmaf((float)cd[k][j], wreg[k][j], -s1);
          const float v = fmaf(crstd, gs, -fmaf((float)cx[k][j], k2, -mk2)) + (RES ? (float)cr[k][j] : 0.f);
          o[j] = (bf16)v;
          dxacc[k][j] += v;
        }
        *(BV*)(dx + off + c * VEC) = o;
      }
    }
#pragma unroll
    for (int k = 0; k < CH; ++k) {
      cd[k] = nd[k];
      cx[k] = nx[k];
      if (RES) cr[k] = nr[k];
    }
    cmean = nmean;
    crstd = nrstd;
  }
  if constexpr (CH * VEC <= 32) {
    __shared__ __attribute__((aligned(16))) float red[4][CH * 64 * VEC];
    const int w = threadIdx.x >> 6;
    auto reduce_out = [&](float(&acc)[CH][VEC], float* part) {
#pragma unroll
      for (int k = 0; k < CH; ++k) {
        const int c = lane + k * 64;
        if (c < C8) {
#pragma unroll
          for (int j = 0; j < VEC; j += 4)
            *(f32x4*)(&red[w][c * VEC + j]) = f32x4{acc[k][j], acc[k][j + 1], acc[k][j + 2], acc[k][j + 3]};
        }
      }
      __syncthreads();
      for (int i = threadIdx.x; i < C; i += 256)
        part[(int64_t)blockIdx.x * C + i] = (red[0][i] + red[1][i]) + (red[2][i] + red[3][i]);
      __syncthreads();
    };
    reduce_out(dwacc, dw_part);
    if (db_part) reduce_out(dbacc, db_part);
    if (dbb_part) reduce_out(dxacc, dbb_part);
  } else {
    static_assert(VEC == 8, "per-wave partial rows are written as 8-column chunks");
#pragma unroll
    for (int k = 0; k < CH; ++k) {
      const int c = lane + k * 64;
      if (c < C8) {
        float* dwp = dw_part + (int64_t)gw * C + c * 8;
        *(f32x4*)dwp = f32x4{dwacc[k][0], dwacc[k][1], dwacc[k][2], dwacc[k][3]};
        *(f32x4*)(dwp + 4) = f32x4{dwacc[k][4], dwacc[k][5], dwacc[k][6], dwacc[k][7]};
        if (db_part) {
          float* dbp = db_part + (int64_t)gw * C + c * 8;
          *(f32x4*)dbp = f32x4{dbacc[k][0], dbacc[k][1], dbacc[k][2], dbacc[k][3]};
          *(f32x4*)(dbp + 4) = f32x4{dbacc[k][4], dbacc[k][5], dbacc[k][6], dbacc[k][7]};
        }
        if (dbb_part) {
          float* p = dbb_part + (int64_t)gw * C + c * 8;
          *(f32x4*)p = f32x4{dxacc[k][0], dxacc[k][1], dxacc[k][2], dxacc[k][3]};
          *(f32x4*)(p + 4) = f32x4{dxacc[k][4], dxacc[k][5], dxacc[k][6], dxacc[k][7]};
        }
      }
    }
  }
}

__device__ __forceinline__ float gelu_f(float x);
__device__ __forceinline__ float gelu_grad_f(float x);

template <int TPB>
__global__ void __launch_bounds__(TPB) bias_gelu_fwd_kernel(const bf16* __restrict__ x, const bf16* __restrict__ b,
                                                            bf16* __restrict__ y, int R, int F) {
  const int c8 = blockIdx.x * TPB + threadIdx.x;
  if (c8 * 8 >= F) return;
  bf16x8 bv = *(const bf16x8*)(b + c8 * 8);
  float bf[8];
#pragma unroll
  for (int j = 0; j < 8; ++j) bf[j] = (float)bv[j];
  const int G = gridDim.y;
  int r = blockIdx.y;
  bf16x8 v[4];
  auto load4 = [&](int r0, bf16x8(&vv)[4]) {
#pragma unroll
    for (int u = 0; u < 4; ++u) vv[u] = *(const bf16x8*)(x + (int64_t)(r0 + u * G) * F + c8 * 8);
  };
  if (r + 3 * G < R) load4(r, v);
  for (; r + 3 * G < R; r += 4 * G) {
    bf16x8 nv[4];
    const bool more = r + 7 * G < R;
    if (more) load4(r + 4 * G, nv);
#pragma unroll
    for (int u = 0; u < 4; ++u) {
      bf16x8 o;
#pragma unroll
      for (int j = 0; j < 8; ++j) o[j] = (bf16)gelu_f((float)v[u][j] + bf[j]);
      *(bf16x8*)(y + (int64_t)(r + u * G) * F + c8 * 8) = o;
    }
    if (more) {
#pragma unroll
      for (int u = 0; u < 4; ++u) v[u] = nv[u];
    }
  }
  for (; r < R; r += G) {
    const int64_t off = (int64_t)r * F + c8 * 8;
    bf16x8 v1 = *(const bf16x8*)(x + off);
    bf16x8 o;
#pragma unroll
    for (int j = 0; j < 8; ++j) o[j] = (bf16)gelu_f((float)v1[j] + bf[j]);
    *(bf16x8*)(y + off) = o;
  }
}

template <int TPB>
__global__ void __launch_bounds__(TPB) bias_gelu_bwd_kernel(const bf16* __restrict__ x, const bf16* __restrict__ b,
                                                            const bf16* __restrict__ dy, bf16* __restrict__ dx,
                                                            float* __restrict__ dbias_part, int R, int F) {
  const int c8 = blockIdx.x * TPB + threadIdx.x;
  if (c8 * 8 >= F) return;
  bf16x8 bv = *(const bf16x8*)(b + c8 * 8);
  float bf[8], acc[8];
#pragma unroll
  for (int j = 0; j < 8; ++j) {
    bf[j] = (float)bv[j];
    acc[j] = 0.f;
  }
  const int G = gridDim.y;
  int r = blockIdx.y;
  bf16x8 v[4], g[4];
  auto load4 = [&](int r0, bf16x8(&vv)[4], bf16x8(&gg)[4]) {
#pragma unroll
    for (int u = 0; u < 4; ++u) {
      const int64_t off = (int64_t)(r0 + u * G) * F + c8 * 8;
      vv[u] = *(const bf16x8*)(x + off);
      gg[u] = *(const bf16x8*)(dy + off);
    }
  };
  if (r + 3 * G < R) load4(r, v, g);
  for (; r + 3 * G < R; r += 4 * G) {
    bf16x8 nv[4], ng[4];
    const bool more = r + 7 * G < R;
    if (more) load4(r + 4 * G, nv, ng);
#pragma unroll
    for (int u = 0; u < 4; ++u) {
      bf16x8 o;
#pragma unroll
      for (int j = 0; j < 8; ++j) {
        const float d = (float)g[u][j] * gelu_grad_f((float)v[u][j] + bf[j]);
        o[j] = (bf16)d;
        acc[j] += d;
      }
      *(bf16x8*)(dx + (int64_t)(r + u * G) * F + c8 * 8) = o;
    }
    if (more) {
#pragma unroll
      for (int u = 0; u < 4; ++u) {
        v[u] = nv[u];
        g[u] = ng[u];
      }
    }
  }
  for (; r < R; r += G) {
    const int64_t off = (int64_t)r * F + c8 * 8;
    bf16x8 v1 = *(const bf16x8*)(x + off);
    bf16x8 g1 = *(const bf16x8*)(dy + off);
    bf16x8 o;
#pragma unroll
    for (int j = 0; j < 8; ++j) {
      const float d = (float)g1[j] * gelu_grad_f((float)v1[j] + bf[j]);
      o[j] = (bf16)d;
      acc[j] += d;
    }
    *(bf16x8*)(dx + off) = o;
  }
  float* p = dbias_part + (int64_t)blockIdx.y * F + c8 * 8;
  *(f32x4*)p = f32x4{acc[0], acc[1], acc[2], acc[3]};
  *(f32x4*)(p + 4) = f32x4{acc[4], acc[5], acc[6], acc[7]};
}



template <int TPB>
__global__ void __launch_bounds__(TPB) colsum_part_bf16_kernel(const bf16* __restrict__ y, float* __restrict__ part,
                                                               int R, int F) {
  const int c8 = blockIdx.x * TPB + threadIdx.x;
  if (c8 * 8 >= F) return;
  float acc[8] = {0.f, 0.f, 0.f, 0.f, 0.f, 0.f, 0.f, 0.f};
  const int G = gridDim.y;
  int r = blockIdx.y;
  for (; r + 3 * G < R; r += 4 * G) {
    bf16x8 v[4];
#pragma unroll
    for (int u = 0; u < 4; ++u) v[u] = *(const bf16x8*)(y + (int64_t)(r + u * G) * F + c8 * 8);
#pragma unroll
    for (int u = 0; u < 4; ++u)
#pragma unroll
      for (int j = 0; j < 8; ++j) acc[j] += (float)v[u][j];
  }
  for (; r < R; r += G) {
    bf16x8 v = *(const bf16x8*)(y + (int64_t)r * F + c8 * 8);
#pragma unroll
    for (int j = 0; j < 8; ++j) acc[j] += (float)v[j];
  }
  float* p = part + (int64_t)blockIdx.y * F + c8 * 8;
  *(f32x4*)p = f32x4{acc[0], acc[1], acc[2], acc[3]};
  *(f32x4*)(p + 4) = f32x4{acc[4], acc[5], acc[6], acc[7]};
}

__global__ void __launch_bounds__(256) colsum_stage1_kernel(const float* __restrict__ p0, const float* __restrict__ p1,
                                                            const float* __restrict__ p2, float* __restrict__ stage,
                                                            int P, int C) {
  __shared__ float red[4][64];
  const int lane = threadIdx.x & 63, w = threadIdx.x >> 6;
  const int out = blockIdx.z, NB = gridDim.y, by = blockIdx.y;
  const float* part = out == 0 ? p0 : (out == 1 ? p1 : p2);
  const int c = blockIdx.x * 64 + lane;
  const int r0 = (int)((int64_t)P * by / NB), r1 = (int)((int64_t)P * (by + 1) / NB);
  float acc = 0.f;
  if (c < C) {
    int r = r0 + w;
    for (; r + 12 < r1; r += 16) {
      const float a0 = part[(int64_t)r * C + c], a1 = part[(int64_t)(r + 4) * C + c];
      const float a2 = part[(int64_t)(r + 8) * C + c], a3 = part[(int64_t)(r + 12) * C + c];
      acc += (a0 + a1) + (a2 + a3);
    }
    for (; r < r1; r += 4) acc += part[(int64_t)r * C + c];
  }
  red[w][lane] = acc;
  __syncthreads();
  if (w == 0 && c < C) stage[((int64_t)out * NB + by) * C + c] = (red[0][lane] + red[1][lane]) + (red[2][lane] + red[3][lane]);
}

__global__ void __launch_bounds__(64) colsum_stage2_kernel(const float* __restrict__ stage, int NB, int C,
                                                           bf16* __restrict__ o0, bf16* __restrict__ o1,
                                                           bf16* __restrict__ o2, int accum_mask) {
  const int out = blockIdx.y;
  const int c = blockIdx.x * 64 + threadIdx.x;
  if (c >= C) return;
  const float* st = stage + (int64_t)out * NB * C + c;
  float v[VCX_COLSUM_NB];
#pragma unroll
  for (int i = 0; i < VCX_COLSUM_NB; ++i) v[i] = st[(int64_t)i * C];
  float acc = 0.f;
#pragma unroll
  for (int i = 0; i < VCX_COLSUM_NB; ++i) acc += v[i];
  bf16* o = out == 0 ? o0 : (out == 1 ? o1 : o2);
  if ((accum_mask >> out) & 1) acc += (float)o[c];
  o[c] = (bf16)acc;
}

__device__ __forceinline__ float gelu_f(float x) {
  const float c0 = -2.f * 0.7978845608028654f * 1.4426950408889634f, k1 = 0.044715f;
  const float e = __builtin_amdgcn_exp2f(c0 * fmaf(k1 * x, x * x, x));
  return x * __builtin_amdgcn_rcpf(1.f + e);
}
__device__ __forceinline__ float gelu_grad_f(float x) {
  const float k0 = 0.7978845608028654f, k1 = 0.044715f;
  const float c0 = -2.f * k0 * 1.4426950408889634f;
  const float x2 = x * x;
  const float e = __builtin_amdgcn_exp2f(c0 * fmaf(k1 * x, x2, x));
  const float sg = __builtin_amdgcn_rcpf(1.f + e);
  const float du2 = 2.f * k0 * fmaf(3.f * k1, x2, 1.f);
  return fmaf(x * sg * (1.f - sg), du2, sg);
}

__global__ void __launch_bounds__(256) gelu_fwd_kernel(const bf16* __restrict__ x, bf16* __restrict__ y,
                                                        int64_t n8) {
  for (int64_t i = blockIdx.x * 256ll + threadIdx.x; i < n8; i += (int64_t)gridDim.x * 256) {
    bf16x8 v = *(const bf16x8*)(x + i * 8);
    bf16x8 o;
#pragma unroll
    for (int j = 0; j < 8; ++j) o[j] = (bf16)gelu_f((float)v[j]);
    *(bf16x8*)(y + i * 8) = o;
  }
}

__global__ void __launch_bounds__(256) gelu_bwd_kernel(const bf16* __restrict__ x, const bf16* __restrict__ dy,
                                                        bf16* __restrict__ dx, int64_t n8) {
  for (int64_t i = blockIdx.x * 256ll + threadIdx.x; i < n8; i += (int64_t)gridDim.x * 256) {
    bf16x8 v = *(const bf16x8*)(x + i * 8);
    bf16x8 g = *(const bf16x8*)(dy + i * 8);
    bf16x8 o;
#pragma unroll
    for (int j = 0; j < 8; ++j) o[j] = (bf16)((float)g[j] * gelu_grad_f((float)v[j]));
    *(bf16x8*)(dx + i * 8) = o;
  }
}

__global__ void __launch_bounds__(256) swiglu_fwd_kernel(const bf16* __restrict__ gu, bf16* __restrict__ y,
                                                          int64_t R, int F) {
  const int F8 = F >> 3;
  const int64_t n8 = R * F8;
  for (int64_t i = blockIdx.x * 256ll + threadIdx.x; i < n8; i += (int64_t)gridDim.x * 256) {
    const int64_t r = i / F8, c = i - r * F8;
    bf16x8 g = *(const bf16x8*)(gu + r * 2 * F + c * 8);
    bf16x8 u = *(const bf16x8*)(gu + r * 2 * F + F + c * 8);
    bf16x8 o;
#pragma unroll
    for (int j = 0; j < 8; ++j) {
      float gf = (float)g[j];
      o[j] = (bf16)(gf / (1.f + __expf(-gf)) * (float)u[j]);
    }
    *(bf16x8*)(y + r * F + c * 8) = o;
  }
}

__global__ void __launch_bounds__(256) swiglu_bwd_kernel(const bf16* __restrict__ gu, const bf16* __restrict__ dy,
                                                          bf16* __restrict__ dgu, int64_t R, int F) {
  const int F8 = F >> 3;
  const int64_t n8 = R * F8;
  for (int64_t i = blockIdx.x * 256ll + threadIdx.x; i < n8; i += (int64_t)gridDim.x * 256) {
    const int64_t r = i / F8, c = i - r * F8;
    bf16x8 g = *(const bf16x8*)(gu + r * 2 * F + c * 8);
    bf16x8 u = *(const bf16x8*)(gu + r * 2 * F + F + c * 8);
    bf16x8 d = *(const bf16x8*)(dy + r * F + c * 8);
    bf16x8 dg, du;
#pragma unroll
    for (int j = 0; j < 8; ++j) {
      float gf = (float)g[j], uf = (float)u[j], df = (float)d[j];
      float sg = 1.f / (1.f + __expf(-gf));
      float silu = gf * sg;
      du[j] = (bf16)(df * silu);
      dg[j] = (bf16)(df * uf * sg * (1.f + gf * (1.f - sg)));
    }
    *(bf16x8*)(dgu + r * 2 * F + c * 8) = dg;
    *(bf16x8*)(dgu + r * 2 * F + F + c * 8) = du;
  }
}

__global__ void __launch_bounds__(256) xent_fwd_kernel(const bf16* __restrict__ logits, const int64_t* __restrict__ tgt,
                                                        float* __restrict__ lse_out, float* __restrict__ loss_out,
                                                        int V, int Vp) {
  __shared__ float sm[4], ss[4];
  const int64_t row = blockIdx.x;
  const bf16* lr = logits + row * Vp;
  const int V8 = V >> 3;
  float m = -INFINITY, s = 0.f;
  for (int c = threadIdx.x; c < V8; c += 256) {
    bf16x8 v = *(const bf16x8*)(lr + c * 8);
    float f[8], cm = -INFINITY;
#pragma unroll
    for (int j = 0; j < 8; ++j) {
      f[j] = (float)v[j];
      cm = fmaxf(cm, f[j]);
    }
    if (cm > m) {
      s *= __expf(m - cm);
      m = cm;
    }
#pragma unroll
    for (int j = 0; j < 8; ++j) s += __expf(f[j] - m);
  }
  for (int c = V8 * 8 + threadIdx.x; c < V; c += 256) {
    float f = (float)lr[c];
    if (f > m) {
      s *= __expf(m - f);
      m = f;
    }
    s += __expf(f - m);
  }
#pragma unroll
  for (int o = 32; o > 0; o >>= 1) {
    float om = __shfl_xor(m, o, 64), os = __shfl_xor(s, o, 64);
    float nm = fmaxf(m, om);
    s = (m == -INFINITY ? 0.f : s * __expf(m - nm)) + (om == -INFINITY ? 0.f : os * __expf(om - nm));
    m = nm;
  }
  const int lane = threadIdx.x & 63, wid = threadIdx.x >> 6;
  if (lane == 0) {
    sm[wid] = m;
    ss[wid] = s;
  }
  __syncthreads();
  if (threadIdx.x == 0) {
    float M = sm[0];
    for (int i = 1; i < 4; ++i) M = fmaxf(M, sm[i]);
    float S = 0.f;
    for (int i = 0; i < 4; ++i) S += (sm[i] == -INFINITY) ? 0.f : ss[i] * __expf(sm[i] - M);
    const float lse = M + __logf(S);
    lse_out[row] = lse;
    const int64_t t = tgt[row];
    loss_out[row] = (t >= 0 && t < V) ? (lse - (float)lr[t]) : 0.f;
  }
}

__global__ void __launch_bounds__(256) xent_bwd_kernel(const bf16* logits, const int64_t* __restrict__ tgt,
                                                        const float* __restrict__ lse_in,
                                                        const float* __restrict__ gscale, bf16* dlogits, int V,
                                                        int Vp) {
  const int64_t row = blockIdx.x;
  const int64_t t = tgt[row];
  const float lse = lse_in[row];
  const float sc = (t >= 0) ? gscale[0] : 0.f;
  const bf16* lr = logits + row * Vp;
  bf16* dr = dlogits + row * Vp;
  const int Vp8 = Vp >> 3;
  for (int c = threadIdx.x; c < Vp8; c += 256) {
    bf16x8 v = *(const bf16x8*)(lr + c * 8);
    bf16x8 o;
#pragma unroll
    for (int j = 0; j < 8; ++j) {
      const int col = c * 8 + j;
      float p = (col < V) ? __expf((float)v[j] - lse) : 0.f;
      if (col == t) p -= 1.f;
      o[j] = (bf16)(p * sc);
    }
    *(bf16x8*)(dr + c * 8) = o;
  }
}

template <int TPB, int NV, int WPE = 6, bool KEEP_E = false>
__global__ void __launch_bounds__(TPB) __attribute__((amdgpu_waves_per_eu(WPE))) xent_fused_kernel(
    bf16* __restrict__ logits, const int64_t* __restrict__ tgt, const float* __restrict__ nvalid,
    float* __restrict__ loss_out, int V, int Vp) {
  constexpr int NW = TPB / 64;
  __shared__ float red[2][NW];
  __shared__ float tlogit;
  const int64_t row = blockIdx.x;
  bf16* lr = logits + row * Vp;
  const int tid = threadIdx.x, lane = tid & 63, wid = tid >> 6;
  const int Vp8 = Vp >> 3;
  const int64_t t = tgt[row];
  if (tid == 0) tlogit = (t >= 0 && t < V) ? (float)lr[t] : 0.f;
  constexpr float L2E = 1.4426950408889634f;
  bf16x8 v[NV];
#pragma unroll
  for (int k = 0; k < NV; ++k) {
    const int c = tid + k * TPB;
    if (c < Vp8) v[k] = *(const bf16x8*)(lr + c * 8);
  }
  float m = -INFINITY;
#pragma unroll
  for (int k = 0; k < NV; ++k) {
    const int c = tid + k * TPB;
    if (c < Vp8) {
#pragma unroll
      for (int j = 0; j < 8; ++j)
        if (c * 8 + j < V) m = fmaxf(m, (float)v[k][j]);
    }
  }
  m = wave_max(m);
  if (lane == 0) red[0][wid] = m;
  __syncthreads();
  float M = red[0][0];
#pragma unroll
  for (int i = 1; i < NW; ++i) M = fmaxf(M, red[0][i]);
  const float M2 = M * L2E;
  float sum = 0.f;
#pragma unroll
  for (int k = 0; k < NV; ++k) {
    const int c = tid + k * TPB;
    if (c < Vp8) {
#pragma unroll
      for (int j = 0; j < 8; ++j) {
        if (c * 8 + j < V) {
          const float e = __builtin_amdgcn_exp2f(fmaf((float)v[k][j], L2E, -M2));
          sum += e;
          if constexpr (KEEP_E) v[k][j] = (bf16)e;
        }
      }
    }
  }
  sum = wave_sum(sum);
  if (lane == 0) red[1][wid] = sum;
  __syncthreads();
  float S = 0.f;
#pragma unroll
  for (int i = 0; i < NW; ++i) S += red[1][i];
  const float lse2 = M2 + __builtin_amdgcn_logf(S);
  const float sc = (t >= 0) ? 1.f / nvalid[0] : 0.f;
  const float invS = 1.f / S;
#pragma unroll
  for (int k = 0; k < NV; ++k) {
    const int c = tid + k * TPB;
    if (c < Vp8) {
      bf16x8 o;
#pragma unroll
      for (int j = 0; j < 8; ++j) {
        const int col = c * 8 + j;
        float p;
        if constexpr (KEEP_E)
          p = (col < V) ? (float)v[k][j] * invS : 0.f;
        else
          p = (col < V) ? __builtin_amdgcn_exp2f(fmaf((float)v[k][j], L2E, -lse2)) : 0.f;
        if (col == t) p -= 1.f;
        o[j] = (bf16)(p * sc);
      }
      *(bf16x8*)(lr + c * 8) = o;
    }
  }
  if (tid == 0) loss_out[row] = (t >= 0) ? lse2 * (1.f / L2E) - tlogit : 0.f;
}

__global__ void __launch_bounds__(256) xent_rescale_kernel(bf16* __restrict__ d, const float* __restrict__ dloss,
                                                           int64_t n8) {
  const float g = dloss[0];
  if (g == 1.f) return;
  for (int64_t i = blockIdx.x * 256ll + threadIdx.x; i < n8; i += (int64_t)gridDim.x * 256) {
    bf16x8 v = *(const bf16x8*)(d + i * 8);
#pragma unroll
    for (int j = 0; j < 8; ++j) v[j] = (bf16)((float)v[j] * g);
    *(bf16x8*)(d + i * 8) = v;
  }
}

}

using namespace vcx;

#define VCX_LN_DISPATCH(CHV, ...)                     \
  switch (CHV) {                                      \
    case 1: { constexpr int CH = 1; __VA_ARGS__; } break; \
    case 2: { constexpr int CH = 2; __VA_ARGS__; } break; \
    case 3: { constexpr int CH = 3; __VA_ARGS__; } break; \
    case 4: { constexpr int CH = 4; __VA_ARGS__; } break; \
    case 5: case 6: { constexpr int CH = 6; __VA_ARGS__; } break; \
    case 7: case 8: { constexpr int CH = 8; __VA_ARGS__; } break; \
    default: { constexpr int CH = 16; __VA_ARGS__; } break; \
  }

void vcx_ln_fwd(const void* a, const void* b, void* xout, void* y, const void* w, const void* bias, float* mean,
                float* rstd, int R, int C, float eps, int rms, const void* bb, hipStream_t s) {
  static const bool fwd4 = [] {
    const char* e = getenv("VCX_LN_FWD4");
    return !(e && atoi(e) == 0);
  }();
  if (fwd4 && C % 256 == 0 && C <= 1024) {
    static const int resident = [] {
      int dev = 0, n = 256;
      (void)hipGetDevice(&dev);
      (void)hipDeviceGetAttribute(&n, hipDeviceAttributeMultiprocessorCount, dev);
      return 5 * n;
    }();
    const int blocks = std::min((R + 3) / 4, resident);
    auto go = [&](auto kern) {
      hipLaunchKernelGGL(kern, dim3(blocks), dim3(256), 0, s, (const bf16*)a, (const bf16*)b, (bf16*)xout, (bf16*)y,
                         (const bf16*)w, (const bf16*)bias, mean, rstd, R, C, eps, rms, (const bf16*)bb);
    };
    switch (C / 256) {
      case 1: go(ln_fwd4_kernel<1>); return;
      case 2: go(ln_fwd4_kernel<2>); return;
      case 3: go(ln_fwd4_kernel<3>); return;
      default: go(ln_fwd4_kernel<4>); return;
    }
  }
  const int ch = (C / 8 + 63) / 64;
  dim3 grid((R + 3) / 4);
  VCX_LN_DISPATCH(ch, hipLaunchKernelGGL(ln_fwd_kernel<CH>, grid, dim3(256), 0, s, (const bf16*)a,
                                         (const bf16*)b, (bf16*)xout, (bf16*)y, (const bf16*)w,
                                         (const bf16*)bias, mean, rstd, R, C, eps, rms, (const bf16*)bb));
}


static void colsums(const float* p0, const float* p1, const float* p2, void* o0, void* o1, void* o2, int nout, int P,
                    int C, float* stage, hipStream_t s, int accum_mask = 0) {
  hipLaunchKernelGGL(colsum_stage1_kernel, dim3((C + 63) / 64, VCX_COLSUM_NB, nout), dim3(256), 0, s, p0, p1, p2,
                     stage, P, C);
  hipLaunchKernelGGL(colsum_stage2_kernel, dim3((C + 63) / 64, nout), dim3(64), 0, s, stage, VCX_COLSUM_NB, C,
                     (bf16*)o0, (bf16*)o1, (bf16*)o2, accum_mask);
}

static int bias_gelu_groups(int R) { return R < 1024 ? (R > 0 ? R : 1) : 1024; }

int vcx_bias_gelu_partials(int R) { return bias_gelu_groups(R); }

static int bias_gelu_tpb(int F) {
  const int F8 = F / 8;
  return F8 % 256 == 0 ? 256 : F8 % 128 == 0 ? 128 : 64;
}

#define VCX_TPB_DISPATCH(tpb, ...) \
  do {                               \
    if (tpb == 256) {                \
      constexpr int TPB = 256;       \
      __VA_ARGS__;                   \
    } else if (tpb == 128) {         \
      constexpr int TPB = 128;       \
      __VA_ARGS__;                   \
    } else {                         \
      constexpr int TPB = 64;        \
      __VA_ARGS__;                   \
    }                                \
  } while (0)

void vcx_bias_gelu_fwd(const void* x, const void* b, void* y, int R, int F, hipStream_t s) {
  const int tpb = bias_gelu_tpb(F);
  dim3 grid((F / 8 + tpb - 1) / tpb, R < 1024 ? (R > 0 ? R : 1) : 1024);
  VCX_TPB_DISPATCH(tpb, hipLaunchKernelGGL(bias_gelu_fwd_kernel<TPB>, grid, dim3(TPB), 0, s, (const bf16*)x,
                                           (const bf16*)b, (bf16*)y, R, F));
}

void vcx_bias_gelu_bwd(const void* x, const void* b, const void* dy, void* dx, float* part, void* db, int R, int F,
                       float* stage, int accumulate, hipStream_t s) {
  const int G = bias_gelu_groups(R);
  const int tpb = bias_gelu_tpb(F);
  dim3 grid((F / 8 + tpb - 1) / tpb, G);
  VCX_TPB_DISPATCH(tpb, hipLaunchKernelGGL(bias_gelu_bwd_kernel<TPB>, grid, dim3(TPB), 0, s, (const bf16*)x,
                                           (const bf16*)b, (const bf16*)dy, (bf16*)dx, part, R, F));
  colsums(part, nullptr, nullptr, db, nullptr, nullptr, 1, G, F, stage, s, accumulate ? 1 : 0);
}

static int ln_bwd_blocks(int R, int C) {
  const int cap = C == 768 ? 768 : 1024;
  const int g = (R + 3) / 4;
  return g > cap ? cap : g;
}

int vcx_ln_bwd_partials(int R, int C) {
  const int ch = (C / 8 + 63) / 64;
  return ch <= 4 ? ln_bwd_blocks(R, C) : ln_bwd_blocks(R, C) * 4;
}

void vcx_ln_bwd(const void* dy, const void* x, const void* w, const float* mean, const float* rstd, const void* dres,
                void* dx, float* dw_part, float* db_part, void* dw, void* db, int R, int C, int rms, float* dbb_part,
                void* dbb, float* stage, int accum_mask, hipStream_t s) {
  const int ch = (C / 8 + 63) / 64;
  const int P = vcx_ln_bwd_partials(R, C);
  dim3 grid(ln_bwd_blocks(R, C));
  if (C == 768) {
    if (dres)
      hipLaunchKernelGGL((ln_bwd_kernel<3, true, 4>), grid, dim3(256), 0, s, (const bf16*)dy, (const bf16*)x,
                         (const bf16*)w, mean, rstd, (const bf16*)dres, (bf16*)dx, dw_part, db_part, R, C, rms,
                         dbb_part);
    else
      hipLaunchKernelGGL((ln_bwd_kernel<3, false, 4>), grid, dim3(256), 0, s, (const bf16*)dy, (const bf16*)x,
                         (const bf16*)w, mean, rstd, (const bf16*)nullptr, (bf16*)dx, dw_part, db_part, R, C, rms,
                         dbb_part);
  } else if (dres) {
    VCX_LN_DISPATCH(ch, hipLaunchKernelGGL((ln_bwd_kernel<CH, true, 8>), grid, dim3(256), 0, s, (const bf16*)dy,
                                           (const bf16*)x, (const bf16*)w, mean, rstd, (const bf16*)dres,
                                           (bf16*)dx, dw_part, db_part, R, C, rms, dbb_part));
  } else {
    VCX_LN_DISPATCH(ch, hipLaunchKernelGGL((ln_bwd_kernel<CH, false, 8>), grid, dim3(256), 0, s, (const bf16*)dy,
                                           (const bf16*)x, (const bf16*)w, mean, rstd, (const bf16*)nullptr,
                                           (bf16*)dx, dw_part, db_part, R, C, rms, dbb_part));
  }
  const float* ps[3] = {dw_part, nullptr, nullptr};
  void* os[3] = {dw, nullptr, nullptr};
  int slot_mask = accum_mask & 1;
  int n = 1;
  if (db_part && db) {
    slot_mask |= ((accum_mask >> 1) & 1) << n;
    ps[n] = db_part;
    os[n++] = db;
  }
  if (dbb_part && dbb) {
    slot_mask |= ((accum_mask >> 2) & 1) << n;
    ps[n] = dbb_part;
    os[n++] = dbb;
  }
  colsums(ps[0], ps[1], ps[2], os[0], os[1], os[2], n, P, C, stage, s, slot_mask);
}

void vcx_colsum_f32(const float* part, void* out, int P, int C, int accumulate, float* stage, hipStream_t s) {
  colsums(part, nullptr, nullptr, out, nullptr, nullptr, 1, P, C, stage, s, accumulate ? 1 : 0);
}

void vcx_colsum_bf16(const void* y, float* part, void* out, int R, int F, int accumulate, float* stage,
                     hipStream_t s) {
  const int G = bias_gelu_groups(R);
  const int tpb = bias_gelu_tpb(F);
  dim3 grid((F / 8 + tpb - 1) / tpb, G);
  VCX_TPB_DISPATCH(tpb, hipLaunchKernelGGL(colsum_part_bf16_kernel<TPB>, grid, dim3(TPB), 0, s, (const bf16*)y, part,
                                           R, F));
  colsums(part, nullptr, nullptr, out, nullptr, nullptr, 1, G, F, stage, s, accumulate ? 1 : 0);
}

void vcx_gelu_fwd(const void* x, void* y, int64_t n, hipStream_t s) {
  hipLaunchKernelGGL(gelu_fwd_kernel, dim3(stream_grid(n / 8, 256)), dim3(256), 0, s, (const bf16*)x, (bf16*)y,
                     n / 8);
}

void vcx_gelu_bwd(const void* x, const void* dy, void* dx, int64_t n, hipStream_t s) {
  hipLaunchKernelGGL(gelu_bwd_kernel, dim3(stream_grid(n / 8, 256)), dim3(256), 0, s, (const bf16*)x,
                     (const bf16*)dy, (bf16*)dx, n / 8);
}

void vcx_swiglu_fwd(const void* gu, void* y, int64_t R, int F, hipStream_t s) {
  hipLaunchKernelGGL(swiglu_fwd_kernel, dim3(stream_grid(R * (F / 8), 256)), dim3(256), 0, s, (const bf16*)gu,
                     (bf16*)y, R, F);
}

void vcx_swiglu_bwd(const void* gu, const void* dy, void* dgu, int64_t R, int F, hipStream_t s) {
  hipLaunchKernelGGL(swiglu_bwd_kernel, dim3(stream_grid(R * (F / 8), 256)), dim3(256), 0, s, (const bf16*)gu,
                     (const bf16*)dy, (bf16*)dgu, R, F);
}

void vcx_xent_fwd(const void* logits, const int64_t* tgt, float* lse, float* loss, int64_t R, int V, int Vp,
                  hipStream_t s) {
  hipLaunchKernelGGL(xent_fwd_kernel, dim3(R), dim3(256), 0, s, (const bf16*)logits, tgt, lse, loss, V, Vp);
}

void vcx_xent_bwd(const void* logits, const int64_t* tgt, const float* lse, const float* gscale, void* dlogits,
                  int64_t R, int V, int Vp, hipStream_t s) {
  hipLaunchKernelGGL(xent_bwd_kernel, dim3(R), dim3(256), 0, s, (const bf16*)logits, tgt, lse, gscale,
                     (bf16*)dlogits, V, Vp);
}

int vcx_xent_fused(void* logits, const int64_t* tgt, const float* nvalid, float* loss, int64_t R, int V, int Vp,
                   hipStream_t s) {
  const int Vp8 = Vp / 8;
  dim3 grid(R);
  static const int tpb = [] {
    const char* e = getenv("VCX_XENT_TPB");
    return e ? atoi(e) : 768;
  }();
  if (tpb == 256 && Vp8 <= 256 * 25) {
    hipLaunchKernelGGL((xent_fused_kernel<256, 25, 4>), grid, dim3(256), 0, s, (bf16*)logits, tgt, nvalid, loss, V, Vp);
    return 1;
  }
  if (tpb == 512 && Vp8 <= 512 * 13) {
    hipLaunchKernelGGL((xent_fused_kernel<512, 13, 5>), grid, dim3(512), 0, s, (bf16*)logits, tgt, nvalid, loss, V, Vp);
    return 1;
  }
  static const bool keep_e = [] {
    const char* e = getenv("VCX_XENT_KEEP_E");
    return !(e && atoi(e) == 0);
  }();
  if (Vp8 <= 768 * 4)
    hipLaunchKernelGGL((xent_fused_kernel<768, 4>), grid, dim3(768), 0, s, (bf16*)logits, tgt, nvalid, loss, V, Vp);
  else if (Vp8 <= 768 * 9 && keep_e)
    hipLaunchKernelGGL((xent_fused_kernel<768, 9, 6, true>), grid, dim3(768), 0, s, (bf16*)logits, tgt, nvalid, loss,
                       V, Vp);
  else if (Vp8 <= 768 * 9)
    hipLaunchKernelGGL((xent_fused_kernel<768, 9>), grid, dim3(768), 0, s, (bf16*)logits, tgt, nvalid, loss, V, Vp);
  else
    return 0;
  return 1;
}

void vcx_xent_rescale(void* d, const float* dloss, int64_t n, hipStream_t s) {
  hipLaunchKernelGGL(xent_rescale_kernel, dim3(stream_grid(n / 8, 256)), dim3(256), 0, s, (bf16*)d, dloss, n / 8);
}
```

distributedvolunteercomputing_amd/csrc/kernels/vcx_api.h:

```cpp
#pragma once
#include <hip/hip_runtime.h>
#include <stdint.h>

#include "job_table.h"

void vcx_grad_sumsq(const void* g, int64_t n, float* ostate, hipStream_t s);
void vcx_adam_prologue(float* ostate, float max_norm, hipStream_t s);
void vcx_adamw_flat(void* param, const void* grad, float* master, float* m, float* v, int64_t n, int64_t n_decay,
                    const float* ostate, float beta1, float beta2, float eps, float wd, hipStream_t s);
void vcx_adamw_flat_compact(void* param, const void* grad, float* master, uint8_t* m_code, uint8_t* m_exp,
                            void* v_half, uint8_t* v_exp, int64_t n, int64_t n_decay, const float* ostate,
                            double beta1, double beta2, float eps, float wd, hipStream_t s);
void vcx_optstate_encode(const float* m, const float* v, uint8_t* m_code, uint8_t* m_exp, void* v_half,
                         uint8_t* v_exp, int64_t n, hipStream_t s);
void vcx_optstate_decode(const uint8_t* m_code, const uint8_t* m_exp, const void* v_half, const uint8_t* v_exp,
                         float* m, float* v, int64_t n, hipStream_t s);
void vcx_lsgd_delta(const float* master, const float* anchor, void* delta, int64_t n, hipStream_t s);
void vcx_lsgd_apply(const void* avg, float* anchor, float* master, void* param, float* mom, int64_t n,
                    float outer_lr, float mu, int nesterov, float avg_scale, hipStream_t s);
void vcx_f32_to_bf16(const float* src, void* dst, int64_t n, hipStream_t s);
void vcx_axpy_bf16(const void* src, void* acc, int64_t n, float scale, hipStream_t s);
bool vcx_gemm_wg_supported(int M, int N, int K, int splits);
int vcx_gemm_wg_splits(int M, int N, int K);
void vcx_gemm_wg(const void* A, const void* B, float* Cpart, void* out, int M, int N, int K, int lda, int ldb,
                 int splits, int accumulate, int loaders, hipStream_t s);
bool vcx_gemm_wg_conv3x3_supported(int Cout, int Cin, int tokens, int64_t xbytes, int splits);
void vcx_gemm_wg_conv3x3(const void* dy, const void* x, float* Cpart, void* out, int Cout, int Cin, int imgs, int H,
                         int W, int stride, int splits, int accumulate, hipStream_t s);
bool vcx_gemm_f_supported(int M, int N, int K);
bool vcx_gemm_f_split_ok(int M, int N, int K, int splits);
int vcx_gemm_f_splits(int M, int N, int K);
void vcx_gemm_f(const void* A, const void* B, void* C, const void* bias, int M, int N, int K, int lda, int ldb,
                int ldc, int waves, int splits, float* ws, hipStream_t s);
bool vcx_gemm_f_conv3x3_supported(int imgs, int H, int W, int Cin, int Cout, int stride);
void vcx_gemm_f_conv3x3(const void* x, const void* w, void* y, const void* bias, int imgs, int H, int W, int Cin,
                        int Cout, int stride, int waves, int splits, float* ws, int flip, int tap_major,
                        hipStream_t s);
bool vcx_gemm_nt_supported(int M, int N, int K);
bool vcx_gemm_nt_supported_epi(int M, int N, int K, int epi);
void vcx_gemm_nt(const void* A, const void* B, void* C, void* C2, const void* bias, float* colsum, int M, int N, int K,
                 int lda, int ldb, int ldc, int epi, hipStream_t s);
bool vcx_gemm_ps_supported(int M, int N, int K, int epi);
int vcx_gemm_ps_grid(int M, int N, int grid_cap);
void vcx_gemm_ps(const void* A, const void* B, void* C, void* C2, const void* bias, float* colsum, int M, int N,
                 int K, int lda, int ldb, int ldc, int epi, int grid_cap, hipStream_t s);
void vcx_transpose_bf16(const void* src, void* dst, int R, int Cc, hipStream_t s);
int vcx_transpose_bf16_many(const vcx::TransposeJob* jobs, int n, hipStream_t s);
void vcx_add_f32_into_bf16(float* in, void* out, int n, int accumulate, int zero_in, hipStream_t s);
void vcx_reduce_bcast_bf16(const void* in, void* out, void* mine, int P, int64_t n, hipStream_t s);
void vcx_splitk_reduce(const void* part, void* acc, int S, int64_t n, int accumulate, hipStream_t s);

void vcx_trimmed_reduce_bcast_bf16(const void* in, void* out, void* mine, int P, int64_t n, int trim,
                                   uint32_t live_mask, float inv, int64_t* counts, hipStream_t s);
void vcx_cclip_reduce_bcast_bf16(const void* in, void* out, void* mine, int P, int64_t n, uint32_t live_mask, float tau,
                                 int iters, float* weights, float* workspace, hipStream_t s);
int64_t vcx_cclip_workspace_floats(int P, int64_t n);
int vcx_cclip_max_workgroups();

void vcx_ln_fwd(const void* a, const void* b, void* xout, void* y, const void* w, const void* bias, float* mean,
                float* rstd, int R, int C, float eps, int rms, const void* bb, hipStream_t s);
int vcx_bias_gelu_partials(int R);
void vcx_bias_gelu_fwd(const void* x, const void* b, void* y, int R, int F, hipStream_t s);
constexpr int VCX_COLSUM_NB = 32;
void vcx_bias_gelu_bwd(const void* x, const void* b, const void* dy, void* dx, float* part, void* db, int R, int F,
                       float* stage, int accumulate, hipStream_t s);
void vcx_colsum_f32(const float* part, void* out, int P, int C, int accumulate, float* stage, hipStream_t s);
void vcx_colsum_bf16(const void* y, float* part, void* out, int R, int F, int accumulate, float* stage,
                     hipStream_t s);
int vcx_ln_bwd_partials(int R, int C);
void vcx_ln_bwd(const void* dy, const void* x, const void* w, const float* mean, const float* rstd, const void* dres,
                void* dx, float* dw_part, float* db_part, void* dw, void* db, int R, int C, int rms, float* dbb_part,
                void* dbb, float* stage, int accum_mask, hipStream_t s);
void vcx_gelu_fwd(const void* x, void* y, int64_t n, hipStream_t s);
void vcx_gelu_bwd(const void* x, const void* dy, void* dx, int64_t n, hipStream_t s);
void vcx_swiglu_fwd(const void* gu, void* y, int64_t R, int F, hipStream_t s);
void vcx_swiglu_bwd(const void* gu, const void* dy, void* dgu, int64_t R, int F, hipStream_t s);
void vcx_xent_fwd(const void* logits, const int64_t* tgt, float* lse, float* loss, int64_t R, int V, int Vp,
                  hipStream_t s);
int vcx_xent_fused(void* logits, const int64_t* tgt, const float* nvalid, float* loss, int64_t R, int V, int Vp,
                   hipStream_t s);
void vcx_xent_rescale(void* d, const float* dloss, int64_t n, hipStream_t s);
void vcx_xent_bwd(const void* logits, const int64_t* tgt, const float* lse, const float* gscale, void* dlogits,
                  int64_t R, int V, int Vp, hipStream_t s);

void vcx_attn_fwd_d64(const void* qkv, void* out, float* lse, int B, int T, int H, float scale, hipStream_t s);
void vcx_attn_set_variant(int fwd_wpe, int fwd_dma, int bwd_dma, int stage_epi);
void vcx_attn_bwd_d64(const void* qkv, const void* out, const void* dout, const float* lse, float* delta, void* dqkv,
                      float* bias_part, int B, int T, int H, float scale, hipStream_t s);
int vcx_attn_bias_partials(int B, int T);
void vcx_attn_hm_fwd(const void* q, const void* k, const void* v, void* out, float* lse, int B, int T, int Hq, int Hkv,
                     int D, float scale, hipStream_t s);
void vcx_attn_hm_set_variant(int dkv_split);
void vcx_attn_hm_bwd(const void* q, const void* k, const void* v, const void* out, const void* dout, const float* lse,
                     float* delta, void* dq, void* dk, void* dv, int B, int T, int Hq, int Hkv, int D, float scale,
                     hipStream_t s);

void vcx_rope_qkv(void* qkv, void* q, void* k, void* v, const float* cosv, const float* sinv, int B, int T, int Hq,
                  int Hkv, int D, int backward, hipStream_t s);

void vcx_embed_fwd(const int64_t* idx, const void* wte, const void* wpe, void* out, int64_t R, int T, int C, int V,
                   hipStream_t s);
void vcx_embed_bwd(const int64_t* idx, const void* dx, float* dwte_scratch, void* dwte, int accum_wte, void* dwpe,
                   int accum_wpe, int64_t R, int T, int C, int V, hipStream_t s);
bool vcx_bn_supported(int C);
void vcx_bn_fwd_train(const void* x, const void* res, void* y, void* mask, int64_t R, int C, const void* gamma,
                      const void* beta, void* run_mean, void* run_var, int run_fp32, float eps, float momentum, float* ws,
                      float* mean, float* rstd, float* scale, float* shift, int64_t* nbt, int relu, int layer_ws,
                      hipStream_t s);
void vcx_subsample_nhwc(const void* x, void* y, int N, int H, int W, int C, int s, hipStream_t st);
void vcx_subsample_add_nhwc(void* full, const void* g, int N, int H, int W, int C, int s, hipStream_t st);
void vcx_bcast_hw_nhwc(const void* g, void* out, int N, int HW, int C, float scale, hipStream_t st);
void vcx_maxpool3s2_fwd(const void* x, void* y, void* idx, int N, int H, int W, int C, int OH, int OW, hipStream_t s);
void vcx_maxpool3s2_bwd(const void* dy, const void* idx, void* dx, int N, int H, int W, int C, int OH, int OW,
                        hipStream_t s);
void vcx_bn_apply(const void* x, const void* res, void* y, int64_t R, int C, const float* scale, const float* shift,
                  int relu, hipStream_t s);
void vcx_bn_bwd(const void* dy, const void* mask, const void* x, const float* mean, const float* rstd, const float* scale,
                int64_t R, int C, float* ws, float* sums, void* gw, void* gb, void* dx, void* dres, int relu,
                int layer_ws, hipStream_t s);
```

distributedvolunteercomputing_amd/ops/__init__.py:

```python
from ._lib import available as native_available, native
from .activations import bias_gelu, gelu, swiglu
from .attention import causal_attention, fused_bias_grad_ok, gqa_attention
from .embedding import embed
from .linear import gemm_nt, linear, mlp_gelu, native_linear_ok, set_gemm_backend, wgrad
from .linear import linear_wants_wt, mlp_wants_wt, transpose_weights
from .loss import cross_entropy, lm_head_cross_entropy
from .norm import add_layernorm, add_rmsnorm, layernorm, rmsnorm
from .rope import rope_qkv
from .optim import (CompactState, adamw_flat_compact, adamw_step, adamw_step_compact, axpy_bf16,
                    check_compact_betas, f32_to_bf16, lsgd_apply, lsgd_delta, new_ostate, reduce_bcast_bf16)
from .robust import (centered_clip_reference, cclip_reduce_bcast_bf16, trimmed_mean_reference,
                     trimmed_reduce_bcast_bf16)
```

distributedvolunteercomputing_amd/ops/attention.py:

```python
from __future__ import annotations

import math

import torch
import torch.nn.functional as F

from ._lib import grad_buffer, native, use_native


class _Attn(torch.autograd.Function):
    @staticmethod
    def forward(ctx, qkv, scale, bias):
        C = native()
        out, lse = C.attn_fwd(qkv, scale)
        ctx.save_for_backward(qkv, out, lse)
        ctx.scale = scale
        ctx.bias = bias
        return out

    @staticmethod
    def backward(ctx, dout):
        qkv, out, lse = ctx.saved_tensors
        C = native()
        bias, ctx.bias = ctx.bias, None
        if bias is None or not ctx.needs_input_grad[2]:
            return C.attn_bwd(qkv, out, dout.contiguous(), lse, ctx.scale), None, None
        gb = grad_buffer(bias)
        dqkv, db = C.attn_bwd_bias(qkv, out, dout.contiguous(), lse, ctx.scale, gb)
        return dqkv, None, (None if gb is not None else db.view_as(bias))


def _ref(qkv, scale):
    q, k, v = qkv.permute(2, 0, 3, 1, 4).unbind(0)
    y = F.scaled_dot_product_attention(q, k, v, is_causal=True, scale=scale)
    return y.transpose(1, 2)


def fused_bias_grad_ok(qkv: torch.Tensor) -> bool:
    return use_native(qkv) and qkv.shape[-1] == 64 and qkv.dtype == torch.bfloat16


def causal_attention(qkv: torch.Tensor, scale: float | None = None, bias: torch.Tensor | None = None) -> torch.Tensor:
    D = qkv.shape[-1]
    scale = 1.0 / math.sqrt(D) if scale is None else scale
    if fused_bias_grad_ok(qkv):
        return _Attn.apply(qkv.contiguous(), scale, bias)
    assert bias is None, "bias gradient fusion needs the native hd64 bf16 attention path"
    return _ref(qkv, scale)


class _AttnHM(torch.autograd.Function):
    @staticmethod
    def forward(ctx, q, k, v, scale):
        out, lse = native().attn_hm_fwd(q, k, v, scale)
        ctx.save_for_backward(q, k, v, out, lse)
        ctx.scale = scale
        return out

    @staticmethod
    def backward(ctx, dout):
        q, k, v, out, lse = ctx.saved_tensors
        dq, dk, dv = native().attn_hm_bwd(q, k, v, out, dout.contiguous(), lse, ctx.scale)
        return dq, dk, dv, None


_GQA_SDPA = [True]


def _ref_gqa(q, k, v, scale):
    rep = q.shape[1] // k.shape[1]
    if rep > 1 and _GQA_SDPA[0]:
        try:
            return F.scaled_dot_product_attention(q, k, v, is_causal=True, scale=scale, enable_gqa=True).transpose(1, 2)
        except (RuntimeError, TypeError):
            _GQA_SDPA[0] = False
    if rep > 1:
        k = k.repeat_interleave(rep, dim=1)
        v = v.repeat_interleave(rep, dim=1)
    return F.scaled_dot_product_attention(q, k, v, is_causal=True, scale=scale).transpose(1, 2)


def gqa_attention(q: torch.Tensor, k: torch.Tensor, v: torch.Tensor, scale: float | None = None) -> torch.Tensor:
    D = q.shape[-1]
    scale = 1.0 / math.sqrt(D) if scale is None else scale
    if use_native(q) and q.dtype == torch.bfloat16 and D in (64, 128) and q.shape[1] % k.shape[1] == 0:
        return _AttnHM.apply(q.contiguous(), k.contiguous(), v.contiguous(), scale)
    return _ref_gqa(q, k, v, scale)
```

distributedvolunteercomputing_amd/ops/linear.py:

```python
from __future__ import annotations

import torch
import torch.nn.functional as F


from .. import config
from ._lib import grad_buffer, native, use_native

MIN_ROWS_PER_SPLIT = 2048


def set_gemm_backend(name: str):
    config.update(gemm="lib" if name == "lib" else "vcx")


def gemm_nt_ok(M: int, N: int, K: int, t) -> bool:
    return (config.get().gemm == "vcx" and use_native(t) and t.dtype == torch.bfloat16
            and bool(native().gemm_nt_supported(M, N, K)))


def gemm_nt(a, b, bias=None, out=None):
    a = a if a.stride(-1) == 1 else a.contiguous()
    out = torch.empty(a.shape[0], b.shape[0], device=a.device, dtype=a.dtype) if out is None else out
    native().gemm_nt(a, b, out, None, bias, None, 1 if bias is not None else 0)
    return out


_ZERO_BIAS: dict = {}


def narrow_gemm_ok(M: int, N: int, K: int, t) -> bool:
    return (config.get().narrow_gemm == "vision" and ((N <= 64 and M >= 131072) or (N <= 128 and M >= 393216))
            and K % 32 == 0 and use_native(t) and t.dtype == torch.bfloat16 and t.is_contiguous())


def narrow_gemm(a, w):
    from . import vision as V

    zb = _ZERO_BIAS.get((w.shape[0], w.device))
    if zb is None:
        zb = _ZERO_BIAS[(w.shape[0], w.device)] = torch.zeros(w.shape[0], device=w.device)
    return V.gemm_bias_act(a, w.contiguous(), zb, False)


def gemm_f_ok(M: int, N: int, K: int, t) -> bool:
    return (config.get().gemm_fwd == "vcx" and use_native(t) and t.dtype == torch.bfloat16 and t.is_contiguous()
            and bool(native().gemm_f_supported(M, N, K)))


def gemm_f(a, w, bias=None):
    out = torch.empty(a.shape[0], w.shape[0], device=a.device, dtype=a.dtype)
    native().gemm_f(a, w.contiguous(), out, bias)
    return out


def transpose_weight(w):
    return native().transpose_bf16(w.contiguous())


def transpose_weights(ws, out=None):
    ws = [w.contiguous() for w in ws]
    if out is not None and not (len(out) == len(ws) and all(
            o.shape == (w.shape[1], w.shape[0]) and o.device == w.device and o.dtype == w.dtype for o, w in zip(out, ws))):
        out = None
    return native().transpose_bf16_many(ws, out)[0]


def linear_wants_wt(M: int, w, t) -> bool:
    N, K = _w2(w).shape
    return (gemm_nt_ok(M, K, N, t) or gemm_f_ok(M, K, N, t) or narrow_gemm_ok(M, K, N, t) or dgrad_ps_ok(M, K, N, t))


def mlp_wants_wt(x, w1, w2):
    mode = _mlp_mode(x, w1, w2)
    if mode is None:
        M = x.numel() // x.shape[-1]
        return linear_wants_wt(M, w1, x), linear_wants_wt(M, w2, x)
    return mode == "nt" or bool(config.get().fc_dgrad_nt), True


_CHOICE: dict = {}


def _torch_mm(a, b, trans_a, trans_b, bias):
    if trans_b and not trans_a:
        return F.linear(a, b, bias)
    y = torch.mm(a.t() if trans_a else a, b.t() if trans_b else b)
    return y if bias is None else y.add_(bias)


def _lt_mm(a, b, trans_a, trans_b, bias):
    C = native()
    M = a.shape[1] if trans_a else a.shape[0]
    N = b.shape[0] if trans_b else b.shape[1]
    out = torch.empty(M, N, device=a.device, dtype=a.dtype)
    epi = C.LT_EPI_DEFAULT if bias is None else C.LT_EPI_BIAS
    if not C.lt_matmul(a, b, out, trans_a, trans_b, epi, bias):
        return None
    return out


def _time_ms(fn, reps=3):
    fn()
    e0, e1 = torch.cuda.Event(enable_timing=True), torch.cuda.Event(enable_timing=True)
    e0.record()
    for _ in range(reps):
        fn()
    e1.record()
    e1.synchronize()
    return e0.elapsed_time(e1) / reps


def mm(a, b, trans_a: bool = False, trans_b: bool = False, bias=None):
    if not (config.get().gemm_select and a.is_cuda and a.dtype == torch.bfloat16 and a.is_contiguous() and b.is_contiguous()):
        return _torch_mm(a, b, trans_a, trans_b, bias)
    key = (tuple(a.shape), tuple(b.shape), trans_a, trans_b, bias is not None)
    c = _CHOICE.get(key)
    if c is None:
        if torch.cuda.is_current_stream_capturing():
            return _torch_mm(a, b, trans_a, trans_b, bias)
        t_torch = _time_ms(lambda: _torch_mm(a, b, trans_a, trans_b, bias))
        c = "torch"
        if _lt_mm(a, b, trans_a, trans_b, bias) is not None:
            if _time_ms(lambda: _lt_mm(a, b, trans_a, trans_b, bias)) < 0.97 * t_torch:
                c = "lt"
        _CHOICE[key] = c
    if c == "lt":
        y = _lt_mm(a, b, trans_a, trans_b, bias)
        if y is not None:
            return y
    return _torch_mm(a, b, trans_a, trans_b, bias)


def gemm_choices() -> dict:
    return dict(_CHOICE)




def _splits(M: int, N: int, K: int) -> int:
    if N * K >= 16 * 1024 * 1024:
        if M < config.get().wgrad_big_split_min_m:
            return 1
        s = 4
    elif M >= 262144:
        s = 64
    else:
        s = 16
    while s > 1 and (M % s or M // s < MIN_ROWS_PER_SPLIT):
        s //= 2
    return s


def gemm_wg_ok(M: int, N: int, K: int, t) -> bool:
    cfg = config.get()
    tiles = ((N + 255) // 256) * (K // 256)
    wide = cfg.wgrad_wide and K <= 1024 and M >= 32768 and tiles > 128
    one_round = 128 < tiles <= 256 and M >= 4096
    return (cfg.gemm_wgrad == "vcx" and use_native(t) and t.dtype == torch.bfloat16
            and (tiles <= 128 or one_round or wide) and (N % 256 == 0 or wide or cfg.wgrad_ragged)
            and bool(native().gemm_wg_supported(N, K, M)))


def wgrad(dy2: torch.Tensor, x2: torch.Tensor, out: torch.Tensor | None = None, accumulate: bool = False):
    M, N = dy2.shape
    K = x2.shape[1]
    if gemm_wg_ok(M, N, K, dy2) and dy2.stride(1) == 1 and x2.stride(1) == 1 and (out is None or out.is_contiguous()):
        if out is None:
            out = torch.empty(N, K, device=dy2.device, dtype=dy2.dtype)
            accumulate = False
        native().gemm_wg(dy2, x2, out, accumulate)
        return out
    S = _splits(M, N, K)
    if S == 1 or not use_native(dy2) or (N * K) % 8:
        if out is None:
            return dy2.t().mm(x2)
        if accumulate:
            out.addmm_(dy2.t(), x2)
        else:
            torch.mm(dy2.t(), x2, out=out)
        return out
    part = torch.bmm(dy2.view(S, M // S, N).transpose(1, 2), x2.view(S, M // S, K))
    if out is None:
        out = torch.empty(N, K, device=dy2.device, dtype=dy2.dtype)
        accumulate = False
    native().splitk_reduce(part, out, accumulate)
    return out


_SIDE: dict = {}
_JOIN_PENDING: dict = {}


def _side_stream(dev):
    st = _SIDE.get(dev)
    if st is None:
        st = _SIDE[dev] = torch.cuda.Stream(device=dev)
    return st


def _queue_join(main, side, key):
    if _JOIN_PENDING.get(key):
        return
    _JOIN_PENDING[key] = True

    def _join():
        main.wait_stream(side)
        _JOIN_PENDING[key] = False

    torch.autograd.Variable._execution_engine.queue_callback(_join)


def _param_grads(dy2, x2, w, bias, want_w, want_b):
    dw = db = None
    N = w.shape[0]
    g = w.grad if want_w else None
    gw = g if g is not None and g.is_contiguous() and g.dtype == w.dtype and g.shape == w.shape else None
    gb = grad_buffer(bias) if want_b else None
    if want_w:
        if gw is not None:
            wgrad(dy2, x2, out=gw.view(N, -1), accumulate=True)
        else:
            dw = wgrad(dy2, x2).view(w.shape)
    if want_b:
        if gb is not None and (N % 8) == 0:
            native().colsum_bf16(dy2, gb)
        elif (N % 8) == 0:
            db = native().colsum_bf16(dy2)
        else:
            db = dy2.sum(0, dtype=torch.float32).to(dy2.dtype)
    return dw, db


def _w2(w):
    return w if w.dim() == 2 else w.view(w.shape[0], -1)


class GradJoin:

    def __init__(self):
        self.pending = None
        self.ran = False

    def take(self):
        g, self.pending = self.pending, None
        return g


class _ResidualTap(torch.autograd.Function):
    @staticmethod
    def forward(ctx, x, join):
        ctx.join = join
        join.pending, join.ran = None, False
        return x.view_as(x)

    @staticmethod
    def backward(ctx, g):
        join, ctx.join = ctx.join, None
        if join.ran or g.dim() != 4:
            return g, None
        gh = g.permute(0, 2, 3, 1)
        if not gh.is_contiguous():
            return g, None
        join.pending = gh.reshape(-1, gh.shape[-1])
        return None, None


def residual_tap(x: torch.Tensor, join: GradJoin) -> torch.Tensor:
    return _ResidualTap.apply(x, join)


class _SubsampleTap(torch.autograd.Function):
    @staticmethod
    def forward(ctx, x, join, s):
        ctx.join, ctx.s = join, s
        ctx.full = (x.shape[0], x.shape[2], x.shape[3], x.shape[1])
        join.ran = False
        xh = x.permute(0, 2, 3, 1)
        ctx.hip = _nhwc_hip_ok(xh)
        if ctx.hip:
            return native().subsample_nhwc(xh, s)
        return xh[:, ::s, ::s, :].contiguous()

    @staticmethod
    def backward(ctx, g):
        join, ctx.join = ctx.join, None
        s, (N, H, W, C) = ctx.s, ctx.full
        base = join.take()
        if base is not None and base.is_contiguous() and base.numel() == N * H * W * C:
            full = base.view(N, H, W, C)
            if ctx.hip and g.is_contiguous() and _nhwc_hip_ok(g) and full.dtype == g.dtype:
                native().subsample_add_nhwc(full, g, s)
            else:
                full[:, ::s, ::s, :].add_(g)
        else:
            join.ran = True
            full = g.new_zeros(N, H, W, C)
            full[:, ::s, ::s, :] = g
        return full.permute(0, 3, 1, 2), None, None


def _nhwc_hip_ok(t: torch.Tensor) -> bool:
    return (use_native(t) and t.dtype == torch.bfloat16 and t.dim() == 4 and t.is_contiguous() and t.shape[3] % 8 == 0
            and t.data_ptr() % 16 == 0)


def subsample_tap(x: torch.Tensor, join: GradJoin, stride: int) -> torch.Tensor:
    return _SubsampleTap.apply(x, join, stride)


class _Linear(torch.autograd.Function):
    @staticmethod
    def forward(ctx, x, w, b, bias_grad_elsewhere=False, join=None, deposit=False, wt=None):
        ctx.save_for_backward(x, w)
        ctx.has_bias = b is not None and not bias_grad_elsewhere
        ctx.bias = b
        ctx.join, ctx.deposit = join, deposit
        ctx.wt = wt
        if deposit:
            join.pending, join.ran = None, False
        x2 = x.reshape(-1, x.shape[-1])
        w = _w2(w)
        if gemm_nt_ok(x2.shape[0], w.shape[0], x2.shape[1], x2):
            return gemm_nt(x2, w, b).view(*x.shape[:-1], w.shape[0])
        if gemm_f_ok(x2.shape[0], w.shape[0], x2.shape[1], x2) and (b is None or b.is_contiguous()):
            return gemm_f(x2, w, b).view(*x.shape[:-1], w.shape[0])
        if b is None and narrow_gemm_ok(x2.shape[0], w.shape[0], x2.shape[1], x2):
            return narrow_gemm(x2, w).view(*x.shape[:-1], w.shape[0])
        return mm(x2, w, trans_b=True, bias=b).view(*x.shape[:-1], w.shape[0])

    @staticmethod
    def backward(ctx, dy):
        x, w_param = ctx.saved_tensors
        w = _w2(w_param)
        N, K = w.shape
        dy2 = dy.reshape(-1, N)
        x2 = x.reshape(-1, K)
        dy2 = dy2.contiguous()
        dx = None
        join, ctx.join = ctx.join, None
        deposit = ctx.deposit
        if deposit:
            join, depo = None, join
        base = join.take() if join is not None else None
        if join is not None and base is None:
            join.ran = True
        if ctx.needs_input_grad[0] and base is not None and base.shape == (dy2.shape[0], K) and base.is_contiguous():
            dx = base.addmm_(dy2, w).view(x.shape)
        elif base is not None:
            dx = (mm(dy2, w) + base).view(x.shape) if ctx.needs_input_grad[0] else None
        elif ctx.needs_input_grad[0]:
            wt = ctx.wt
            if gemm_nt_ok(dy2.shape[0], K, N, dy2):
                dx = gemm_nt(dy2, transpose_weight(w) if wt is None else wt).view(x.shape)
            elif gemm_f_ok(dy2.shape[0], K, N, dy2):
                dx = gemm_f(dy2, transpose_weight(w) if wt is None else wt).view(x.shape)
            elif narrow_gemm_ok(dy2.shape[0], K, N, dy2):
                dx = narrow_gemm(dy2, transpose_weight(w) if wt is None else wt).view(x.shape)
            elif dgrad_ps_ok(dy2.shape[0], K, N, dy2):
                dx = torch.empty(dy2.shape[0], K, device=dy2.device, dtype=dy2.dtype)
                native().gemm_ps(dy2, transpose_weight(w) if wt is None else wt, dx)
                dx = dx.view(x.shape)
            elif wt is not None:
                dx = mm(dy2, wt, trans_b=True).view(x.shape)
            else:
                dx = mm(dy2, w).view(x.shape)
        if deposit and dx is not None and not depo.ran and dx.is_contiguous():
            depo.pending, dx = dx.view(-1, K), None
        want_w = bool(ctx.needs_input_grad[1])
        want_b = bool(ctx.has_bias and ctx.needs_input_grad[2])
        bias, ctx.bias = ctx.bias, None
        w = w_param
        flat_w = w.grad is not None and w.grad.is_contiguous() and w.grad.dtype == w.dtype
        flat_b = (not want_b) or grad_buffer(bias) is not None
        if config.get().async_wgrad and dy2.is_cuda and flat_w and flat_b and (want_w or want_b):
            main = torch.cuda.current_stream(dy2.device)
            side = _side_stream(dy2.device)
            side.wait_stream(main)
            with torch.cuda.stream(side):
                _param_grads(dy2, x2, w, bias, want_w, want_b)
            dy2.record_stream(side)
            x2.record_stream(side)
            _queue_join(main, side, dy2.device)
            return dx, None, None, None, None, None, None
        dw, db = _param_grads(dy2, x2, w, bias, want_w, want_b)
        return dx, dw, db, None, None, None, None


def native_linear_ok(w: torch.Tensor) -> bool:
    return use_native(w) and w.dtype == torch.bfloat16 and torch.is_grad_enabled() and w.requires_grad


def linear(x: torch.Tensor, w: torch.Tensor, b: torch.Tensor | None = None,
           bias_grad_elsewhere: bool = False, join: GradJoin | None = None, deposit: bool = False,
           wt: torch.Tensor | None = None) -> torch.Tensor:
    if native_linear_ok(w):
        return _Linear.apply(x, w, b, bias_grad_elsewhere, join, deposit, wt)
    assert join is None, "a GradJoin needs the native linear path (its backward consumes the joined gradient)"
    return F.linear(x, _w2(w), b)


def dgrad_ps_ok(M: int, N: int, K: int, t) -> bool:
    return (config.get().dgrad_ps and K <= 2304 and use_native(t) and t.dtype == torch.bfloat16
            and t.is_contiguous() and bool(native().gemm_ps_supported(M, N, K, 0)))


def gemm_ps_ok(M: int, N: int, K: int, epi: int, t) -> bool:
    return (config.get().mlp == "fused" and use_native(t) and t.dtype == torch.bfloat16
            and bool(native().gemm_ps_supported(M, N, K, epi)))


class _MlpGelu(torch.autograd.Function):

    @staticmethod
    def forward(ctx, x, w1, b1, w2, ps, w1t=None, w2t=None):
        C = native()
        x2 = x.reshape(-1, x.shape[-1])
        M, F_ = x2.shape[0], w1.shape[0]
        pre = torch.empty(M, F_, device=x.device, dtype=x.dtype)
        act = torch.empty_like(pre)
        if ps:
            C.gemm_ps(x2, w1, pre, act, b1, None, 5 if config.get().mlp_grad_fwd else 2)
            y = gemm_f(act, w2) if gemm_f_ok(M, w2.shape[0], F_, act) else mm(act, w2, trans_b=True)
        else:
            C.gemm_nt(x2, w1, pre, act, b1, None, 2)
            y = gemm_nt(act, w2)
        ctx.save_for_backward(x2, w1, b1, w2, pre, act)
        ctx.xshape = x.shape
        ctx.ps = ps
        ctx.w1t, ctx.w2t = w1t, w2t
        ctx.grad_fwd = bool(ps and config.get().mlp_grad_fwd)
        return y.view(*x.shape[:-1], w2.shape[0])

    @staticmethod
    def backward(ctx, dy):
        C = native()
        x2, w1, b1, w2, pre, act = ctx.saved_tensors
        dy2 = dy.reshape(-1, dy.shape[-1]).contiguous()
        M, F_ = pre.shape
        gb = grad_buffer(b1) if ctx.needs_input_grad[2] else None
        cs = _colsum_buffer(F_, dy.device) if gb is not None else torch.zeros(F_, device=dy.device, dtype=torch.float32)
        dpre = torch.empty_like(pre)
        w1t = ctx.w1t
        w2t = transpose_weight(w2) if ctx.w2t is None else ctx.w2t
        if ctx.ps:
            C.gemm_ps(dy2, w2t, dpre, pre, None, cs, 6 if ctx.grad_fwd else 4)
        else:
            C.gemm_nt(dy2, w2t, dpre, pre, None, cs, 3)
        dw2, _ = _param_grads(dy2, act, w2, None, ctx.needs_input_grad[3], False)
        dw1, _ = _param_grads(dpre, x2, w1, None, ctx.needs_input_grad[1], False)
        db1 = None
        if ctx.needs_input_grad[2]:
            if gb is not None:
                C.add_f32_into_bf16(cs, gb, True, True)
            else:
                db1 = cs.to(b1.dtype)
        dx = None
        if ctx.needs_input_grad[0]:
            if not ctx.ps:
                dx = gemm_nt(dpre, transpose_weight(w1) if w1t is None else w1t)
            elif w1t is not None and config.get().fc_dgrad_nt:
                dx = mm(dpre, w1t, trans_b=True)
            else:
                dx = mm(dpre, w1)
            dx = dx.view(ctx.xshape)
        return dx, dw1, db1, dw2, None, None, None


_COLSUM = {}


def _colsum_buffer(n: int, device) -> torch.Tensor:
    key = (n, device, torch.cuda.current_stream(device).cuda_stream)
    buf = _COLSUM.get(key)
    if buf is None:
        buf = _COLSUM[key] = torch.zeros(n, device=device, dtype=torch.float32)
    return buf


def mlp_gelu_ok(x, w1, w2) -> bool:
    return _mlp_mode(x, w1, w2) is not None


def _mlp_mode(x, w1, w2):
    if not (native_linear_ok(w1) and x.dtype == torch.bfloat16):
        return None
    M = x.numel() // x.shape[-1]
    F_, C_ = w1.shape
    if gemm_ps_ok(M, F_, C_, 2, x) and gemm_ps_ok(M, F_, w2.shape[0], 4, x):
        return "ps"
    if (gemm_nt_ok(M, F_, C_, x) and gemm_nt_ok(M, w2.shape[0], F_, x) and gemm_nt_ok(M, C_, w2.shape[0], x)
            and gemm_nt_ok(M, F_, w2.shape[0], x)):
        return "nt"
    return None


def mlp_gelu(x, w1, b1, w2, w1t=None, w2t=None):
    mode = _mlp_mode(x, w1, w2)
    if mode is not None:
        return _MlpGelu.apply(x, w1, b1, w2, mode == "ps", w1t, w2t)
    from .activations import bias_gelu

    return linear(bias_gelu(linear(x, w1, wt=w1t), b1), w2, wt=w2t)
```

distributedvolunteercomputing_amd/ops/norm.py:

```python
from __future__ import annotations

import torch

from ._lib import grad_buffer, native, use_native


def _ref_ln(x, w, b, eps, rms):
    xf = x.float()
    if rms:
        var = xf.pow(2).mean(-1, keepdim=True)
        y = xf * torch.rsqrt(var + eps)
    else:
        mu = xf.mean(-1, keepdim=True)
        var = (xf - mu).pow(2).mean(-1, keepdim=True)
        y = (xf - mu) * torch.rsqrt(var + eps)
    y = y * w.float()
    if b is not None:
        y = y + b.float()
    return y.to(x.dtype)


class _AddLN(torch.autograd.Function):
    @staticmethod
    def forward(ctx, a, b, w, bias, eps, rms, bb):
        C = native()
        y, x, mean, rstd = C.ln_fwd(a.contiguous(), None if b is None else b.contiguous(), w, bias, eps, rms, bb)
        ctx.save_for_backward(x, w, mean, rstd)
        ctx.params = (w, bias, bb)
        ctx.has_b = b is not None
        ctx.has_bias = bias is not None
        ctx.has_bb = bb is not None
        ctx.rms = rms
        ctx.set_materialize_grads(False)
        if b is None:
            x = x.view_as(x)
        return y, x

    @staticmethod
    def backward(ctx, dy, dx_res):
        if dy is None:
            if dx_res is None:
                return None, None, None, None, None, None, None
            dbb = None
            if ctx.has_bb:
                dbb = dx_res.reshape(-1, dx_res.shape[-1]).float().sum(0).to(dx_res.dtype)
            return dx_res, (dx_res if ctx.has_b else None), None, None, None, None, dbb
        x, w, mean, rstd = ctx.saved_tensors
        C = native()
        dres = None if dx_res is None else dx_res.contiguous()
        pw, pbias, pbb = ctx.params
        gw, gb, gbb = grad_buffer(pw), grad_buffer(pbias) if ctx.has_bias else None, grad_buffer(pbb) if ctx.has_bb else None
        dx, dw, dbias, dbb = C.ln_bwd(dy.contiguous(), x, w, mean, rstd, dres, ctx.has_bias, ctx.rms, ctx.has_bb,
                                      gw, gb, gbb)
        dw = None if gw is not None else dw
        dbias = None if gb is not None else dbias
        dbb = None if gbb is not None else dbb
        return dx, (dx if ctx.has_b else None), dw, dbias, None, None, dbb


def add_layernorm(a, b, weight, bias=None, eps: float = 1e-5, rms: bool = False, branch_bias=None):
    if use_native(a):
        y, x = _AddLN.apply(a, b, weight, bias, eps, rms, branch_bias)
        return y, x
    if b is None:
        x = a
    else:
        x = a + (b if branch_bias is None else b + branch_bias)
    return _ref_ln(x, weight, bias, eps, rms), x


def layernorm(x, weight, bias=None, eps: float = 1e-5):
    return add_layernorm(x, None, weight, bias, eps, False)[0]


def rmsnorm(x, weight, eps: float = 1e-6):
    return add_layernorm(x, None, weight, None, eps, True)[0]


def add_rmsnorm(a, b, weight, eps: float = 1e-6):
    return add_layernorm(a, b, weight, None, eps, True)
```

distributedvolunteercomputing_amd/parallel/local_sgd.py:

```python
from __future__ import annotations

import contextlib
import time
from dataclasses import dataclass, field

import torch

from .. import ops
from ..utils.trace import NULL_TRACER
from ..ops.robust import AGGREGATES, check_clip, effective_trim
from .collectives import allreduce_sum_, cclip_mean_, robust_mean_
from .compression import Quant8Compressor
from .flat_params import FlatBuffers, FlatParams
from .peer_group import PeerFailure


@dataclass
class LocalSGDConfig:
    lr: float = 6e-4
    betas: tuple = (0.9, 0.95)
    eps: float = 1e-8
    weight_decay: float = 0.1
    max_grad_norm: float = 1.0
    H: int = 4
    algo: str = "direct"
    outer_lr: float = 1.0
    outer_momentum: float = 0.0
    nesterov: bool = False
    comm_dtype: torch.dtype = torch.bfloat16
    compression: str = "none"
    topk_ratio: float = 0.01
    powersgd_rank: int = 4
    opt_state: str = "fp32"
    aggregate: str = "mean"
    trim: int = 1
    clip_tau: float = 0.0
    clip_iters: int = 3
    robust_q8: bool = False

    def __post_init__(self):
        check_aggregate(self.aggregate, self.trim, self.clip_tau, self.clip_iters)


def check_aggregate(aggregate, trim, clip_tau=0.0, clip_iters=3):
    if aggregate not in AGGREGATES:
        raise ValueError(f"aggregate must be one of {AGGREGATES}, got {aggregate!r}")
    if not isinstance(trim, int) or trim < 0:
        raise ValueError(f"trim must be an integer >= 0, got {trim!r}")
    check_clip(clip_tau, clip_iters)


@dataclass
class StepStats:
    step: int
    loss: float | None
    synced: bool
    sync_ms: float = 0.0
    members: int = 1
    extra: dict = field(default_factory=dict)


class LocalSGDTrainer:
    def __init__(self, model: torch.nn.Module, cfg: LocalSGDConfig, *, group=None, membership=None,
                 device=None, compressor=None, tracer=None):
        self.model = model
        self.cfg = cfg
        self.device = device or next(model.parameters()).device
        self.flat = FlatParams(model, dtype=torch.bfloat16, device=self.device)
        self.buffers = FlatBuffers(model)
        n = self.flat.numel
        self.master = self.flat.param.float()
        if cfg.opt_state not in ("fp32", "compact"):
            raise ValueError(f"opt_state must be 'fp32' or 'compact', got {cfg.opt_state!r}")
        check_aggregate(cfg.aggregate, cfg.trim, cfg.clip_tau, cfg.clip_iters)
        self.delta_hook = None
        self.wire_hook = None
        self.trim_share = None
        self.nonfinite_share = None
        self.clip_weight = None
        self._trim_clip_logged = False
        self.cstate = None
        if cfg.opt_state == "compact":
            ops.check_compact_betas(cfg.betas)
            self.m = self.v = None
            self.cstate = ops.CompactState.zeros(n, self.device)
        else:
            self.m = torch.zeros(n, dtype=torch.float32, device=self.device)
            self.v = torch.zeros(n, dtype=torch.float32, device=self.device)
        self.anchor = self.master.clone()
        self.delta = torch.zeros(n, dtype=cfg.comm_dtype, device=self.device)
        self.outer_mom = torch.zeros(n, dtype=torch.float32, device=self.device) if cfg.outer_momentum > 0 else None
        self.ostate = ops.new_ostate(self.device, cfg.lr)
        self.membership = membership
        self.group = membership.group if membership is not None else group
        self.compressor = compressor
        self.tracer = tracer or NULL_TRACER
        self.t = 0
        self.sync_count = 0
        self.last_sync_ms = 0.0
        self.t_sync_end = None
        self.failed_rounds = 0
        self.admit_split = None
        self.last_round_stages = None
        self.time_reduce = False
        self.reduce_log: list[tuple[float, int]] = []

    def set_lr(self, lr: float):
        self.ostate[1].fill_(lr)

    def forward_backward(self, x, y):
        self.flat.zero_grad()
        loss = self.model(x, y)
        loss.backward()
        return loss

    def optimizer_step(self):
        c = self.cfg
        kw = dict(n_decay=self.flat.n_decay, beta1=c.betas[0], beta2=c.betas[1], eps=c.eps, wd=c.weight_decay,
                  max_norm=c.max_grad_norm)
        if self.cstate is not None:
            ops.adamw_step_compact(self.flat.param, self.flat.grad, self.master, self.cstate, self.ostate, **kw)
        else:
            ops.adamw_step(self.flat.param, self.flat.grad, self.master, self.m, self.v, self.ostate, **kw)

    def capture(self, x, y, warmup: int = 3):
        assert x.is_cuda, "graph capture needs GPU tensors"
        self.graph = None
        self._gx = x.clone()
        self._gy = y.clone()
        s = torch.cuda.Stream()
        s.wait_stream(torch.cuda.current_stream())
        with torch.cuda.stream(s):
            for _ in range(warmup):
                self.step(self._gx, self._gy)
        torch.cuda.current_stream().wait_stream(s)
        torch.cuda.synchronize()
        graph = torch.cuda.CUDAGraph()
        with torch.cuda.graph(graph, capture_error_mode="thread_local"):
            self._gloss = self.forward_backward(self._gx, self._gy)
            self.optimizer_step()
        self.graph = graph
        return self

    def step(self, x, y) -> StepStats:
        tr = self.tracer
        if getattr(self, "graph", None) is not None:
            if x.data_ptr() != self._gx.data_ptr():
                self._gx.copy_(x, non_blocking=True)
                self._gy.copy_(y, non_blocking=True)
            with tr.span("local_step_graph"):
                self.graph.replay()
            loss = self._gloss
        else:
            with tr.span("fwd_bwd"):
                loss = self.forward_backward(x, y)
            with tr.span("adamw"):
                self.optimizer_step()
        self.t += 1
        synced = False
        if self.t % self.cfg.H == 0:
            with tr.span("average"):
                self.sync()
            synced = True
        return StepStats(self.t, None, synced, self.last_sync_ms, self.group.size if self.group else 1,
                         {"loss_t": loss.detach()})

    def sync(self):
        t0 = time.perf_counter()
        if self.membership is None:
            res = self._reduce(())
            self._apply(res)
            self.buffers.average_(self.group, self.cfg.aggregate, self.cfg.trim)
        else:
            self._sync_elastic()
        self.sync_count += 1
        self.last_sync_ms = (time.perf_counter() - t0) * 1e3
        self.t_sync_end = time.time()

    def _sync_elastic(self):
        mem = self.membership
        t0 = time.perf_counter()
        grp, _, newcomers = mem.sync_round()
        t1 = time.perf_counter()
        self.last_round_stages = None
        while True:
            self.group = grp
            snap = self.compressor.snapshot() if (self.compressor is not None and grp.size > 1) else None
            try:
                with mem.guard():
                    t2 = time.perf_counter()
                    adopted = self._admit_newcomers(newcomers) if newcomers else None
                    self._dev_sync()
                    t3 = time.perf_counter()
                    res = self._reduce(newcomers)
                    bufs = self.buffers.averaged(grp, self.cfg.aggregate, self.cfg.trim, self._voters(grp, newcomers))
                    self._dev_sync()
                    t4 = time.perf_counter()
                self._adopt(adopted)
                self._apply(res, bufs)
                if newcomers:
                    self._dev_sync()
                    t5 = time.perf_counter()
                    ad = self.admit_split or {}
                    self.last_round_stages = {
                        "sync_round_ms": round((t1 - t0) * 1e3, 3),
                        "peer_wait_ms": round(ad.get("peer_wait_ms", 0.0), 3),
                        "comm_init_ms": round(ad.get("comm_init_ms", 0.0), 3),
                        "broadcast_ms": round(ad.get("broadcast_ms", 0.0), 3),
                        "reduce_ms": round((t4 - t3) * 1e3, 3),
                        "guard_verdict_apply_ms": round(((t5 - t1) - (t4 - t2)) * 1e3, 3),
                        "broadcast_bytes": ad.get("bytes", 0),
                    }
                return
            except PeerFailure:
                if snap is not None:
                    self.compressor.restore(snap)
                self.delta = torch.zeros_like(self.delta)
                self.failed_rounds += 1
                grp, _, newcomers = mem.recover()

    def _reduce(self, newcomers=()):
        g = self.group
        c = self.cfg
        robust = c.aggregate != "mean"
        if robust:
            check_aggregate(c.aggregate, c.trim, c.clip_tau, c.clip_iters)
            if c.aggregate == "cclip" and self.compressor is not None:
                raise ValueError(f"aggregate='cclip' cannot be combined with the {type(self.compressor).__name__} "
                                 "compressor: the rule measures every peer's l2 distance from the centre on the "
                                 "uncompressed shard; top-k and PowerSGD never put the peers' own values on the "
                                 "shard owner, and over the q8 records the rule is not defined yet")
            if self.compressor is not None and not isinstance(self.compressor, Quant8Compressor):
                raise ValueError(f"aggregate={c.aggregate!r} cannot be combined with the "
                                 f"{type(self.compressor).__name__} compressor: a coordinate-wise rule needs every "
                                 "peer's own value of every coordinate on the shard owner, and top-k sends a "
                                 "different set of coordinates from every peer while PowerSGD sums low-rank "
                                 "factors; q8 is the compressor that works with the robust rules")
            if self.compressor is not None and not c.robust_q8:
                raise ValueError(f"aggregate={c.aggregate!r} is combined with the q8 compressor only on request: set "
                                 "LocalSGDConfig.robust_q8 (the rule then runs on the peers' decoded 8-bit records: "
                                 "the aggregate is quantised again, and a non-finite coordinate comes out as 0 and "
                                 "is counted in nonfinite_share)")
            if c.algo != "direct":
                raise ValueError(f"aggregate={c.aggregate!r} runs over the 'direct' exchange only, got "
                                 f"algo={c.algo!r}")
        if g is None or g.size == 1:
            return None
        ops.lsgd_delta(self.master, self.anchor, self.delta)
        if self.delta_hook is not None:
            self.delta_hook(self.delta)
        if isinstance(self.compressor, Quant8Compressor):
            self.compressor.wire_hook = self.wire_hook
        if robust:
            return self._reduce_robust(g, newcomers)
        contributors = max(1, g.size - len(newcomers))
        if self.compressor is not None:
            avg = self.compressor.allreduce_mean(self.delta, g)
            return avg, g.size / contributors
        with self._timed_reduce():
            allreduce_sum_(self.delta, g, self.cfg.algo)
        return self.delta, 1.0 / contributors

    @contextlib.contextmanager
    def _timed_reduce(self):
        if not self.time_reduce:
            yield
            return
        self._dev_sync()
        t0 = time.perf_counter()
        yield
        self._dev_sync()
        self.reduce_log.append(((time.perf_counter() - t0) * 1e3, self.delta.numel() * self.delta.element_size()))

    @staticmethod
    def _voters(g, newcomers):
        if not newcomers:
            return None
        live = [i for i, m in enumerate(g.members) if m not in newcomers]
        return live or None

    def _reduce_robust(self, g, newcomers):
        c = self.cfg
        live = self._voters(g, newcomers)
        K = g.size if live is None else len(live)
        if c.aggregate == "cclip":
            with self._timed_reduce():
                w = cclip_mean_(self.delta, g, c.clip_tau, c.clip_iters, live)
            self.clip_weight = w.tolist()
            return self.delta, 1.0
        trim = effective_trim(c.aggregate, c.trim, K)
        if trim > (K - 1) // 2 and not self._trim_clip_logged:
            self._trim_clip_logged = True
            print(f"[local-sgd] trim={trim} clipped to {(K - 1) // 2}: only {K} peers vote "
                  f"(a trimmed mean needs K >= 2 trim + 1)", flush=True)
        if self.compressor is not None:
            avg, counts, nonfinite = self.compressor.allreduce_robust(self.delta, g, trim, live)
            self.trim_share = (counts.double() / self.delta.numel()).tolist()
            self.nonfinite_share = nonfinite / self.delta.numel()
            return avg, 1.0
        with self._timed_reduce():
            counts = robust_mean_(self.delta, g, trim, live)
        self.trim_share = (counts.double() / self.delta.numel()).tolist()
        return self.delta, 1.0

    def _apply(self, res, bufs=None):
        if bufs is not None:
            self.buffers.load_fp32(bufs)
        if res is None:
            self.anchor.copy_(self.master)
            return
        avg, scale = res
        c = self.cfg
        ops.lsgd_apply(avg, self.anchor, self.master, self.flat.param, self.outer_mom, outer_lr=c.outer_lr,
                       mu=c.outer_momentum, nesterov=c.nesterov, avg_scale=scale)

    def _average(self, newcomers=()):
        self._apply(self._reduce(newcomers))

    def _admit_newcomers(self, newcomers):
        g = self.group
        members = g.members
        cont = [i for i, m in enumerate(members) if m not in newcomers]
        if not cont:
            return None
        root = cont[0]
        dev = self.anchor.device
        parts = [self.anchor] + ([self.outer_mom] if self.outer_mom is not None else [])
        nb = self.buffers.numel if self.buffers else 0
        n = sum(p.numel() for p in parts) + nb
        bdev = dev if g.backend == "nccl" else torch.device("cpu")
        if g.rank == root:
            pack = torch.cat([p.reshape(-1).to(bdev) for p in parts]
                             + ([self.buffers.as_fp32().to(bdev)] if nb else []))
        else:
            pack = torch.empty(n, dtype=torch.float32, device=bdev)
        tw = time.perf_counter()
        self._admission_checkin(g)
        t0 = time.perf_counter()
        g.broadcast_(torch.zeros(1, dtype=torch.float32, device=bdev), root)
        self._dev_sync()
        t1 = time.perf_counter()
        g.broadcast_(pack, root)
        self._dev_sync()
        t2 = time.perf_counter()
        self.admit_split = {"peer_wait_ms": (t0 - tw) * 1e3, "comm_init_ms": (t1 - t0) * 1e3,
                            "broadcast_ms": (t2 - t1) * 1e3, "bytes": int(n * 4)}
        return pack if members[g.rank] in newcomers else None

    def _admission_checkin(self, g):
        mem = self.membership
        if mem is None or g.size <= 1:
            return
        key = f"vcx/el/admit_in/{mem.gen}"
        mem.store.add(key, 1)
        while int(mem.store.add(key, 0)) < g.size:
            if mem.tripped():
                raise PeerFailure(f"gen {mem.gen}: aborted during the admission check-in ({mem.abort_reason()})")
            time.sleep(0.001)

    def _dev_sync(self):
        if self.anchor.is_cuda:
            torch.cuda.synchronize(self.anchor.device)

    def _adopt(self, pack):
        if pack is None:
            return
        pack = pack.to(self.anchor.device)
        n0 = self.anchor.numel()
        self.anchor.copy_(pack[:n0])
        pos = n0
        if self.outer_mom is not None:
            self.outer_mom.copy_(pack[pos:pos + n0])
            pos += n0
        if self.buffers:
            self.buffers.load_fp32(pack[pos:pos + self.buffers.numel])
        self.master.copy_(self.anchor)
        ops.f32_to_bf16(self.anchor, self.flat.param)

    def join_running_job(self):
        mem = self.membership
        grp, newcomers = mem.group, mem.newcomers
        dev_sync = (lambda: torch.cuda.synchronize(self.anchor.device)) if self.anchor.is_cuda else (lambda: None)
        while True:
            self.group = grp
            try:
                t0 = time.perf_counter()
                with mem.guard():
                    dev_sync()
                    t2 = time.perf_counter()
                    t1 = t2 - mem.last_go_wait_ms * 1e-3
                    adopted = self._admit_newcomers(newcomers)
                    dev_sync()
                    t3 = time.perf_counter()
                    res = self._reduce(newcomers)
                    bufs = self.buffers.averaged(grp, self.cfg.aggregate, self.cfg.trim, self._voters(grp, newcomers))
                    dev_sync()
                    t4 = time.perf_counter()
                self._adopt(adopted)
                self._apply(res, bufs)
                dev_sync()
                t5 = time.perf_counter()
                ad = self.admit_split or {}
                st = {"connect_ms": (t1 - t0) * 1e3, "wait_round_ms": (t2 - t1) * 1e3,
                      "peer_wait_ms": ad.get("peer_wait_ms", 0.0), "comm_init_ms": ad.get("comm_init_ms", 0.0), "broadcast_ms": ad.get("broadcast_ms", (t3 - t2) * 1e3),
                      "reduce_ms": (t4 - t3) * 1e3,
                      "verdict_apply_ms": (t5 - t4) * 1e3, "admission_round_ms": (t5 - t2) * 1e3,
                      "broadcast_bytes": ad.get("bytes", int(self.anchor.numel() * 4 * (2 if self.outer_mom is not None else 1)))}
                self.admit_stages = {k: (round(v, 2) if isinstance(v, float) else v) for k, v in st.items()}
                return
            except PeerFailure:
                self.delta = torch.zeros_like(self.delta)
                self.failed_rounds += 1
                grp, _, newcomers = mem.recover()

    def state_tensors(self):
        if self.cstate is not None:
            moments = dict(zip(self.cstate.FIELDS, self.cstate.arrays()))
        else:
            moments = {"m": self.m, "v": self.v}
        return {"master": self.master, **moments, "anchor": self.anchor, "ostate": self.ostate}

    def checkpoint_slice(self):
        P = 1 if self.group is None else self.group.size
        r = 0 if self.group is None else self.group.rank
        lo, hi = self.flat.shard_bounds(r, P)
        m, v = self.cstate.to_fp32() if self.cstate is not None else (self.m, self.v)
        t = {"master": self.anchor[lo:hi], "m": mean_slice(self.group, m, lo, hi),
             "v": mean_slice(self.group, v, lo, hi)}
        if self.outer_mom is not None:
            t["outer_mom"] = self.outer_mom[lo:hi]
        if self.compressor is not None:
            t["ef"] = mean_slice(self.group, self.compressor.state_dict()["ef"], lo, hi)
        return lo, hi, t

    def checkpoint_global(self) -> dict:
        out = {}
        if self.buffers:
            out["buffers"] = self.buffers.as_fp32()
        if self.compressor is not None and "Q" in self.compressor.state_dict():
            out["psgd_Q"] = self.compressor.state_dict()["Q"]
        return out

    def restore(self, reader):
        reader.check_layout(self.flat)
        n = self.flat.numel
        dev = self.device
        self.master.copy_(reader.read_range("master", 0, n).to(dev))
        self.anchor.copy_(self.master)
        m, v = reader.read_range("m", 0, n).to(dev), reader.read_range("v", 0, n).to(dev)
        if self.cstate is not None:
            self.cstate.load_fp32(m, v)
        else:
            self.m.copy_(m)
            self.v.copy_(v)
        if self.outer_mom is not None:
            self.outer_mom.copy_(reader.read_range("outer_mom", 0, n).to(dev))
        _, ost = reader.params()
        self.ostate.copy_(ost.to(dev))
        ops.f32_to_bf16(self.master, self.flat.param)
        restore_extras(self, reader)
        self.t = reader.step


def mean_slice(group, buf, lo, hi):
    if group is None or group.size == 1:
        return buf[lo:hi]
    P = group.size
    if buf.numel() % P == 0 and hi - lo == buf.numel() // P:
        out = torch.empty(hi - lo, dtype=buf.dtype, device=buf.device)
        group.reduce_scatter_(out, buf)
    else:
        tmp = buf.clone()
        group.allreduce_(tmp)
        out = tmp[lo:hi]
    return out.div_(P)


def restore_extras(trainer, reader):
    bufs = reader.global_tensor("buffers")
    if bufs is not None and trainer.buffers:
        trainer.buffers.load_fp32(bufs)
    comp = trainer.compressor
    if comp is not None and reader.has_key("ef"):
        d = {"ef": reader.read_range("ef", 0, trainer.flat.numel)}
        q = reader.global_tensor("psgd_Q")
        if q is not None:
            d["Q"] = q
        elif "Q" in comp.state_dict():
            d["Q"] = comp.state_dict()["Q"]
        comp.load_state_dict(d)
```

Baseline: 1112 samples/s.

## Defer bias/norm column-sum reductions to one batched launch after backward

Adds a ColsumPool that, during loss.backward, collects the fp32 partial-sum buffers from layernorm, attention-bias and MLP-bias backward passes instead of reducing each one immediately. After backward it runs batched two-stage column-sum kernels over a job table. This replaces many small per-layer reduction launches and their staging allocations with a few launches, and reuses the partial buffers across steps. Separately, attention-style linears that have a cached transposed weight no longer take the gemm_ps dgrad path and use the NT dgrad path instead. The cost is extra persistent fp32 partial memory and the deferred reductions losing any overlap with the rest of backward.

```diff
diff --git a/distributedvolunteercomputing_amd/config.py b/distributedvolunteercomputing_amd/config.py
--- a/distributedvolunteercomputing_amd/config.py
+++ b/distributedvolunteercomputing_amd/config.py
@@ -19,6 +19,8 @@
     bwd_batch: bool = True
     fc_dgrad_nt: bool = True
     lmhead_dgrad_nt: bool = True
+    dgrad_nt_attn: bool = True
+    colsum_defer: bool = True
     gemm_fwd: str = "lib"
     dgrad_ps: bool = True
     gemm_wgrad: str = "vcx"
@@ -65,6 +67,8 @@
     "bwd_batch": ("VCX_BWD_BATCH", _bool),
     "fc_dgrad_nt": ("VCX_FC_DGRAD_NT", _bool),
     "lmhead_dgrad_nt": ("VCX_LMHEAD_DGRAD_NT", _bool),
+    "dgrad_nt_attn": ("VCX_DGRAD_NT_ATTN", _bool),
+    "colsum_defer": ("VCX_COLSUM_DEFER", _bool),
     "narrow_gemm": ("VCX_NARROW_GEMM", str),
     "resnet_conv1x1": ("VCX_RESNET_CONV1X1", str),
     "resnet_bn": ("VCX_RESNET_BN", str),
diff --git a/distributedvolunteercomputing_amd/csrc/bindings.cpp b/distributedvolunteercomputing_amd/csrc/bindings.cpp
--- a/distributedvolunteercomputing_amd/csrc/bindings.cpp
+++ b/distributedvolunteercomputing_amd/csrc/bindings.cpp
@@ -689,7 +689,7 @@
 std::vector<at::Tensor> ln_bwd(at::Tensor dy, at::Tensor x, at::Tensor w, at::Tensor mean, at::Tensor rstd,
                                c10::optional<at::Tensor> dres, bool has_bias, bool rms, bool has_bb,
                                c10::optional<at::Tensor> dw_out, c10::optional<at::Tensor> db_out,
-                               c10::optional<at::Tensor> dbb_out) {
+                               c10::optional<at::Tensor> dbb_out, c10::optional<at::Tensor> parts, bool defer) {
   CHECK_IN(dy, kBF);
   CHECK_IN(x, kBF);
   CHECK_IN(w, kBF);
@@ -704,26 +704,90 @@
     TORCH_CHECK(dres->sizes() == x.sizes());
   }
   const int P = vcx_ln_bwd_partials((int)R, C);
+  const int64_t nparts = 1 + (has_bias ? 1 : 0) + (has_bb ? 1 : 0);
+  if (parts) {
+    CHECK_IN((*parts), kF);
+    TORCH_CHECK(parts->dim() == 3 && parts->size(0) == nparts && parts->size(1) == P && parts->size(2) == C,
+                "ln_bwd: parts must be [outputs, ln_bwd_partials(R, C), C] fp32");
+  }
+  TORCH_CHECK(!defer || parts, "ln_bwd: defer needs the caller's parts");
+  int64_t slot = 0;
+  auto part_rows = [&]() { return parts ? parts->select(0, slot++) : at::empty({P, C}, x.options().dtype(kF)); };
   auto dx = at::empty_like(x);
-  auto dw_part = at::empty({P, C}, x.options().dtype(kF));
+  auto dw_part = part_rows();
   int mask = 0;
   at::Tensor dw = grad_out(dw_out, C, x, &mask, 0);
   at::Tensor db_part, db;
   if (has_bias) {
-    db_part = at::empty({P, C}, x.options().dtype(kF));
+    db_part = part_rows();
     db = grad_out(db_out, C, x, &mask, 1);
   }
   at::Tensor dbb_part, dbb;
   if (has_bb) {
-    dbb_part = at::empty({P, C}, x.options().dtype(kF));
+    dbb_part = part_rows();
     dbb = grad_out(dbb_out, C, x, &mask, 2);
   }
   vcx_ln_bwd(dy.data_ptr(), x.data_ptr(), w.data_ptr(), mean.data_ptr<float>(), rstd.data_ptr<float>(),
              opt_ptr(dres), dx.data_ptr(), dw_part.data_ptr<float>(), has_bias ? db_part.data_ptr<float>() : nullptr,
              dw.data_ptr(), has_bias ? db.data_ptr() : nullptr, (int)R, C, rms ? 1 : 0,
              has_bb ? dbb_part.data_ptr<float>() : nullptr, has_bb ? dbb.data_ptr() : nullptr,
-             at::empty({3 * VCX_COLSUM_NB * C}, x.options().dtype(kF)).data_ptr<float>(), mask, cur_stream());
+             defer ? nullptr : at::empty({3 * VCX_COLSUM_NB * C}, x.options().dtype(kF)).data_ptr<float>(), mask,
+             defer ? 1 : 0, cur_stream());
   return {dx, dw, db, dbb};
+}
+
+at::Tensor colsum_f32(at::Tensor part, c10::optional<at::Tensor> out) {
+  CHECK_IN(part, kF);
+  TORCH_CHECK(part.dim() == 2 && part.size(0) < INT32_MAX && part.size(1) > 0 && part.size(1) < INT32_MAX,
+              "colsum_f32: part [P, C] fp32");
+  const int64_t P = part.size(0), C = part.size(1);
+  int mask = 0;
+  at::Tensor o = out ? grad_out(out, C, part, &mask, 0) : at::empty({C}, part.options().dtype(kBF));
+  auto stage = at::empty({VCX_COLSUM_NB * C}, part.options());
+  vcx_colsum_f32(part.data_ptr<float>(), o.data_ptr(), (int)P, (int)C, mask, stage.data_ptr<float>(), cur_stream());
+  return o;
+}
+
+int64_t colsum_finish_stage_floats(std::vector<int64_t> widths) {
+  std::vector<vcx::ColsumJob> jobs(widths.size());
+  for (size_t i = 0; i < widths.size(); ++i) {
+    TORCH_CHECK(widths[i] >= 0 && widths[i] < INT32_MAX, "colsum_finish_stage_floats: width");
+    jobs[i] = vcx::ColsumJob{};
+    jobs[i].C = (int)widths[i];
+  }
+  return vcx::colsum_stage_floats_max(jobs.data(), (int)jobs.size());
+}
+
+int64_t colsum_finish_many(std::vector<at::Tensor> parts, std::vector<at::Tensor> outs, std::vector<bool> accumulate,
+                           std::vector<bool> zero_src, at::Tensor stage) {
+  const size_t n = parts.size();
+  TORCH_CHECK(outs.size() == n && accumulate.size() == n && zero_src.size() == n,
+              "colsum_finish_many: one out, accumulate and zero_src per part");
+  if (n == 0) return 0;
+  CHECK_IN(stage, kF);
+  std::vector<vcx::ColsumJob> jobs(n);
+  for (size_t i = 0; i < n; ++i) {
+    const at::Tensor& p = parts[i];
+    const at::Tensor& o = outs[i];
+    CHECK_IN(p, kF);
+    CHECK_IN(o, kBF);
+    const int64_t C = o.numel();
+    TORCH_CHECK((p.dim() == 1 || p.dim() == 2) && p.size(-1) == C && C < INT32_MAX && p.numel() / (C ? C : 1) < INT32_MAX &&
+                    p.get_device() == stage.get_device() && o.get_device() == stage.get_device(),
+                "colsum_finish_many: part [P, C] fp32 and out [C] bf16 on the stage's device");
+    vcx::ColsumJob j{};
+    j.part = p.data_ptr<float>();
+    j.P = C ? (int)(p.numel() / C) : 0;
+    j.C = (int)C;
+    j.out = o.data_ptr();
+    j.accumulate = accumulate[i] ? 1 : 0;
+    j.zero_src = zero_src[i] ? 1 : 0;
+    jobs[i] = j;
+  }
+  TORCH_CHECK(stage.numel() >= vcx::colsum_stage_floats_max(jobs.data(), (int)n), "colsum_finish_many: stage too small");
+  const int launches = vcx_colsum_finish_many(jobs.data(), (int)n, stage.data_ptr<float>(), stage.numel(), cur_stream());
+  TORCH_CHECK(launches >= 0, "colsum_finish_many: a job the table does not take");
+  return launches;
 }
 
 at::Tensor colsum_bf16(at::Tensor y, c10::optional<at::Tensor> out) {
@@ -963,7 +1027,7 @@
 }
 
 std::vector<at::Tensor> attn_bwd_bias(at::Tensor qkv, at::Tensor out, at::Tensor dout, at::Tensor lse, double scale,
-                                      c10::optional<at::Tensor> db_out) {
+                                      c10::optional<at::Tensor> db_out, c10::optional<at::Tensor> part_in, bool defer) {
   CHECK_IN(qkv, kBF);
   CHECK_IN(out, kBF);
   CHECK_IN(dout, kBF);
@@ -975,13 +1039,21 @@
   auto dqkv = at::empty_like(qkv);
   auto delta = at::empty({B, H, T}, lse.options());
   const int P = vcx_attn_bias_partials((int)B, (int)T);
-  auto part = at::empty({P, F}, lse.options());
+  if (part_in) {
+    CHECK_IN((*part_in), kF);
+    TORCH_CHECK(part_in->dim() == 2 && part_in->size(0) == P && part_in->size(1) == F,
+                "attn_bwd_bias: part must be [attn_bias_partials(B, T), 3 * H * 64] fp32");
+  }
+  TORCH_CHECK(!defer || part_in, "attn_bwd_bias: defer needs the caller's part");
+  auto part = part_in ? *part_in : at::empty({P, F}, lse.options());
   int mask = 0;
   at::Tensor db = grad_out(db_out, F, qkv, &mask, 0);
-  auto stage = at::empty({VCX_COLSUM_NB * F}, lse.options());
   vcx_attn_bwd_d64(qkv.data_ptr(), out.data_ptr(), dout.data_ptr(), lse.data_ptr<float>(), delta.data_ptr<float>(),
                    dqkv.data_ptr(), part.data_ptr<float>(), (int)B, (int)T, (int)H, (float)scale, cur_stream());
-  vcx_colsum_f32(part.data_ptr<float>(), db.data_ptr(), P, (int)F, mask, stage.data_ptr<float>(), cur_stream());
+  if (!defer) {
+    auto stage = at::empty({VCX_COLSUM_NB * F}, lse.options());
+    vcx_colsum_f32(part.data_ptr<float>(), db.data_ptr(), P, (int)F, mask, stage.data_ptr<float>(), cur_stream());
+  }
   return {dqkv, db};
 }
 
@@ -1091,7 +1163,15 @@
   m.def("ln_bwd", &ln_bwd, pybind11::arg("dy"), pybind11::arg("x"), pybind11::arg("w"), pybind11::arg("mean"),
         pybind11::arg("rstd"), pybind11::arg("dres"), pybind11::arg("has_bias"), pybind11::arg("rms"),
         pybind11::arg("has_bb"), pybind11::arg("dw_out") = pybind11::none(), pybind11::arg("db_out") = pybind11::none(),
-        pybind11::arg("dbb_out") = pybind11::none());
+        pybind11::arg("dbb_out") = pybind11::none(), pybind11::arg("parts") = pybind11::none(),
+        pybind11::arg("defer") = false);
+  m.def("ln_bwd_partials", [](int64_t R, int64_t C) { return (int64_t)vcx_ln_bwd_partials((int)R, (int)C); });
+  m.def("attn_bias_partials", [](int64_t B, int64_t T) { return (int64_t)vcx_attn_bias_partials((int)B, (int)T); });
+  m.attr("COLSUM_NB") = (int64_t)VCX_COLSUM_NB;
+  m.def("colsum_f32", &colsum_f32, pybind11::arg("part"), pybind11::arg("out") = pybind11::none());
+  m.def("colsum_finish_stage_floats", &colsum_finish_stage_floats, pybind11::arg("widths"));
+  m.def("colsum_finish_many", &colsum_finish_many, pybind11::arg("parts"), pybind11::arg("outs"),
+        pybind11::arg("accumulate"), pybind11::arg("zero_src"), pybind11::arg("stage"));
   m.def("colsum_bf16", &colsum_bf16, pybind11::arg("y"), pybind11::arg("out") = pybind11::none());
   m.def("gelu_fwd", &gelu_fwd);
   m.def("bias_gelu_fwd", &bias_gelu_fwd);
@@ -1117,7 +1197,8 @@
   m.def("attn_hm_bwd", &attn_hm_bwd);
   m.def("attn_hm_set_variant", &vcx_attn_hm_set_variant);
   m.def("attn_bwd_bias", &attn_bwd_bias, pybind11::arg("qkv"), pybind11::arg("out"), pybind11::arg("dout"),
-        pybind11::arg("lse"), pybind11::arg("scale"), pybind11::arg("db_out") = pybind11::none());
+        pybind11::arg("lse"), pybind11::arg("scale"), pybind11::arg("db_out") = pybind11::none(),
+        pybind11::arg("part") = pybind11::none(), pybind11::arg("defer") = false);
   vcx_register_vision(m);
   vcx_register_compress(m);
   vcx_register_lt(m);
diff --git a/distributedvolunteercomputing_amd/csrc/kernels/colsum_table.h b/distributedvolunteercomputing_amd/csrc/kernels/colsum_table.h
--- /dev/null
+++ b/distributedvolunteercomputing_amd/csrc/kernels/colsum_table.h
@@ -0,0 +1,70 @@
+#pragma once
+#include <stdint.h>
+
+#include "job_table.h"
+
+#if defined(__HIPCC__)
+#define VCX_HD __host__ __device__
+#else
+#define VCX_HD
+#endif
+
+namespace vcx {
+
+constexpr int COLSUM_NB = 32;
+
+struct ColsumJob {
+  const float* part;
+  int P, C;
+  void* out;
+  int accumulate;
+  int zero_src;
+};
+
+struct ColsumTable {
+  int njobs;
+  int Cmax;
+  ColsumJob job[JOBS_MAX];
+};
+
+inline int pack_colsum_jobs(const ColsumJob* jobs, int n, int start, ColsumTable* t) {
+  t->njobs = 0;
+  t->Cmax = 0;
+  int i = start < 0 ? 0 : start;
+  for (; i < n && t->njobs < JOBS_MAX; ++i) {
+    const ColsumJob& in = jobs[i];
+    if (in.C <= 0) continue;
+    if (in.P < 0 || !in.out || (in.P > 0 && !in.part)) return -1;
+    ColsumJob& o = t->job[t->njobs++];
+    o = in;
+    o.accumulate = in.accumulate ? 1 : 0;
+    o.zero_src = in.zero_src ? 1 : 0;
+    if (in.C > t->Cmax) t->Cmax = in.C;
+  }
+  return i;
+}
+
+inline int colsum_grid_x(const ColsumTable& t) { return (t.Cmax + 63) / 64; }
+
+inline int64_t colsum_stage_floats(const ColsumTable& t) { return (int64_t)t.njobs * COLSUM_NB * t.Cmax; }
+
+inline int64_t colsum_stage_floats_max(const ColsumJob* jobs, int n) {
+  int cmax = 0, live = 0;
+  for (int i = 0; i < n; ++i)
+    if (jobs[i].C > 0) {
+      ++live;
+      if (jobs[i].C > cmax) cmax = jobs[i].C;
+    }
+  return (int64_t)(live < JOBS_MAX ? live : JOBS_MAX) * COLSUM_NB * cmax;
+}
+
+VCX_HD inline void colsum_rows(int P, int by, int NB, int* r0, int* r1) {
+  *r0 = (int)((int64_t)P * by / NB);
+  *r1 = (int)((int64_t)P * (by + 1) / NB);
+}
+
+VCX_HD inline int64_t colsum_stage_row(int slot, int by, int NB, int width) {
+  return ((int64_t)slot * NB + by) * width;
+}
+
+}
diff --git a/distributedvolunteercomputing_amd/csrc/kernels/norm_act.hip b/distributedvolunteercomputing_amd/csrc/kernels/norm_act.hip
--- a/distributedvolunteercomputing_amd/csrc/kernels/norm_act.hip
+++ b/distributedvolunteercomputing_amd/csrc/kernels/norm_act.hip
@@ -455,15 +455,13 @@
   *(f32x4*)(p + 4) = f32x4{acc[4], acc[5], acc[6], acc[7]};
 }
 
-__global__ void __launch_bounds__(256) colsum_stage1_kernel(const float* __restrict__ p0, const float* __restrict__ p1,
-                                                            const float* __restrict__ p2, float* __restrict__ stage,
-                                                            int P, int C) {
-  __shared__ float red[4][64];
+template <bool ZERO>
+__device__ __forceinline__ void colsum_stage1_body(const float* __restrict__ part, float* __restrict__ stage_row,
+                                                   int P, int C, int by, int NB, float (*red)[64]) {
   const int lane = threadIdx.x & 63, w = threadIdx.x >> 6;
-  const int out = blockIdx.z, NB = gridDim.y, by = blockIdx.y;
-  const float* part = out == 0 ? p0 : (out == 1 ? p1 : p2);
   const int c = blockIdx.x * 64 + lane;
-  const int r0 = (int)((int64_t)P * by / NB), r1 = (int)((int64_t)P * (by + 1) / NB);
+  int r0, r1;
+  colsum_rows(P, by, NB, &r0, &r1);
   float acc = 0.f;
   if (c < C) {
     int r = r0 + w;
@@ -471,12 +469,43 @@
       const float a0 = part[(int64_t)r * C + c], a1 = part[(int64_t)(r + 4) * C + c];
       const float a2 = part[(int64_t)(r + 8) * C + c], a3 = part[(int64_t)(r + 12) * C + c];
       acc += (a0 + a1) + (a2 + a3);
-    }
-    for (; r < r1; r += 4) acc += part[(int64_t)r * C + c];
+      if (ZERO) {
+        float* z = const_cast<float*>(part);
+        z[(int64_t)r * C + c] = 0.f;
+        z[(int64_t)(r + 4) * C + c] = 0.f;
+        z[(int64_t)(r + 8) * C + c] = 0.f;
+        z[(int64_t)(r + 12) * C + c] = 0.f;
+      }
+    }
+    for (; r < r1; r += 4) {
+      acc += part[(int64_t)r * C + c];
+      if (ZERO) const_cast<float*>(part)[(int64_t)r * C + c] = 0.f;
+    }
   }
   red[w][lane] = acc;
   __syncthreads();
-  if (w == 0 && c < C) stage[((int64_t)out * NB + by) * C + c] = (red[0][lane] + red[1][lane]) + (red[2][lane] + red[3][lane]);
+  if (w == 0 && c < C) stage_row[c] = (red[0][lane] + red[1][lane]) + (red[2][lane] + red[3][lane]);
+}
+
+__device__ __forceinline__ void colsum_stage2_body(const float* __restrict__ st, int64_t stride, bf16* __restrict__ o,
+                                                   int c, int accumulate) {
+  float v[VCX_COLSUM_NB];
+#pragma unroll
+  for (int i = 0; i < VCX_COLSUM_NB; ++i) v[i] = st[(int64_t)i * stride];
+  float acc = 0.f;
+#pragma unroll
+  for (int i = 0; i < VCX_COLSUM_NB; ++i) acc += v[i];
+  if (accumulate) acc += (float)o[c];
+  o[c] = (bf16)acc;
+}
+
+__global__ void __launch_bounds__(256) colsum_stage1_kernel(const float* __restrict__ p0, const float* __restrict__ p1,
+                                                            const float* __restrict__ p2, float* __restrict__ stage,
+                                                            int P, int C) {
+  __shared__ float red[4][64];
+  const int out = blockIdx.z, NB = gridDim.y, by = blockIdx.y;
+  const float* part = out == 0 ? p0 : (out == 1 ? p1 : p2);
+  colsum_stage1_body<false>(part, stage + colsum_stage_row(out, by, NB, C), P, C, by, NB, red);
 }
 
 __global__ void __launch_bounds__(64) colsum_stage2_kernel(const float* __restrict__ stage, int NB, int C,
@@ -485,16 +514,29 @@
   const int out = blockIdx.y;
   const int c = blockIdx.x * 64 + threadIdx.x;
   if (c >= C) return;
-  const float* st = stage + (int64_t)out * NB * C + c;
-  float v[VCX_COLSUM_NB];
-#pragma unroll
-  for (int i = 0; i < VCX_COLSUM_NB; ++i) v[i] = st[(int64_t)i * C];
-  float acc = 0.f;
-#pragma unroll
-  for (int i = 0; i < VCX_COLSUM_NB; ++i) acc += v[i];
   bf16* o = out == 0 ? o0 : (out == 1 ? o1 : o2);
-  if ((accum_mask >> out) & 1) acc += (float)o[c];
-  o[c] = (bf16)acc;
+  colsum_stage2_body(stage + colsum_stage_row(out, 0, NB, C) + c, C, o, c, (accum_mask >> out) & 1);
+}
+
+__global__ void __launch_bounds__(256) colsum_stage1_many_kernel(const ColsumTable tab, float* __restrict__ stage) {
+  __shared__ float red[4][64];
+  const int j = blockIdx.z, by = blockIdx.y;
+  const int C = tab.job[j].C;
+  if ((int)blockIdx.x * 64 >= C) return;
+  float* row = stage + colsum_stage_row(j, by, VCX_COLSUM_NB, tab.Cmax);
+  if (tab.job[j].zero_src)
+    colsum_stage1_body<true>(tab.job[j].part, row, tab.job[j].P, C, by, VCX_COLSUM_NB, red);
+  else
+    colsum_stage1_body<false>(tab.job[j].part, row, tab.job[j].P, C, by, VCX_COLSUM_NB, red);
+}
+
+__global__ void __launch_bounds__(64) colsum_stage2_many_kernel(const ColsumTable tab,
+                                                                const float* __restrict__ stage) {
+  const int j = blockIdx.y;
+  const int c = blockIdx.x * 64 + threadIdx.x;
+  if (c >= tab.job[j].C) return;
+  colsum_stage2_body(stage + colsum_stage_row(j, 0, VCX_COLSUM_NB, tab.Cmax) + c, tab.Cmax, (bf16*)tab.job[j].out, c,
+                     tab.job[j].accumulate);
 }
 
 __device__ __forceinline__ float gelu_f(float x) {
@@ -861,7 +903,7 @@
 
 void vcx_ln_bwd(const void* dy, const void* x, const void* w, const float* mean, const float* rstd, const void* dres,
                 void* dx, float* dw_part, float* db_part, void* dw, void* db, int R, int C, int rms, float* dbb_part,
-                void* dbb, float* stage, int accum_mask, hipStream_t s) {
+                void* dbb, float* stage, int accum_mask, int defer, hipStream_t s) {
   const int ch = (C / 8 + 63) / 64;
   const int P = vcx_ln_bwd_partials(R, C);
   dim3 grid(ln_bwd_blocks(R, C));
@@ -883,6 +925,7 @@
                                            (const bf16*)x, (const bf16*)w, mean, rstd, (const bf16*)nullptr,
                                            (bf16*)dx, dw_part, db_part, R, C, rms, dbb_part));
   }
+  if (defer) return;
   const float* ps[3] = {dw_part, nullptr, nullptr};
   void* os[3] = {dw, nullptr, nullptr};
   int slot_mask = accum_mask & 1;
@@ -902,6 +945,21 @@
 
 void vcx_colsum_f32(const float* part, void* out, int P, int C, int accumulate, float* stage, hipStream_t s) {
   colsums(part, nullptr, nullptr, out, nullptr, nullptr, 1, P, C, stage, s, accumulate ? 1 : 0);
+}
+
+int vcx_colsum_finish_many(const vcx::ColsumJob* jobs, int n, float* stage, int64_t stage_floats, hipStream_t s) {
+  int launches = 0;
+  for (int i = 0; i < n;) {
+    ColsumTable tab{};
+    i = pack_colsum_jobs(jobs, n, i, &tab);
+    if (i < 0 || colsum_stage_floats(tab) > stage_floats) return -1;
+    if (tab.njobs == 0) break;
+    const int gx = colsum_grid_x(tab);
+    hipLaunchKernelGGL(colsum_stage1_many_kernel, dim3(gx, VCX_COLSUM_NB, tab.njobs), dim3(256), 0, s, tab, stage);
+    hipLaunchKernelGGL(colsum_stage2_many_kernel, dim3(gx, tab.njobs), dim3(64), 0, s, tab, (const float*)stage);
+    launches += 2;
+  }
+  return launches;
 }
 
 void vcx_colsum_bf16(const void* y, float* part, void* out, int R, int F, int accumulate, float* stage,
diff --git a/distributedvolunteercomputing_amd/csrc/kernels/vcx_api.h b/distributedvolunteercomputing_amd/csrc/kernels/vcx_api.h
--- a/distributedvolunteercomputing_amd/csrc/kernels/vcx_api.h
+++ b/distributedvolunteercomputing_amd/csrc/kernels/vcx_api.h
@@ -2,6 +2,7 @@
 #include <hip/hip_runtime.h>
 #include <stdint.h>
 
+#include "colsum_table.h"
 #include "job_table.h"
 
 void vcx_grad_sumsq(const void* g, int64_t n, float* ostate, hipStream_t s);
@@ -61,7 +62,7 @@
                 float* rstd, int R, int C, float eps, int rms, const void* bb, hipStream_t s);
 int vcx_bias_gelu_partials(int R);
 void vcx_bias_gelu_fwd(const void* x, const void* b, void* y, int R, int F, hipStream_t s);
-constexpr int VCX_COLSUM_NB = 32;
+constexpr int VCX_COLSUM_NB = vcx::COLSUM_NB;
 void vcx_bias_gelu_bwd(const void* x, const void* b, const void* dy, void* dx, float* part, void* db, int R, int F,
                        float* stage, int accumulate, hipStream_t s);
 void vcx_colsum_f32(const float* part, void* out, int P, int C, int accumulate, float* stage, hipStream_t s);
@@ -70,7 +71,8 @@
 int vcx_ln_bwd_partials(int R, int C);
 void vcx_ln_bwd(const void* dy, const void* x, const void* w, const float* mean, const float* rstd, const void* dres,
                 void* dx, float* dw_part, float* db_part, void* dw, void* db, int R, int C, int rms, float* dbb_part,
-                void* dbb, float* stage, int accum_mask, hipStream_t s);
+                void* dbb, float* stage, int accum_mask, int defer, hipStream_t s);
+int vcx_colsum_finish_many(const vcx::ColsumJob* jobs, int n, float* stage, int64_t stage_floats, hipStream_t s);
 void vcx_gelu_fwd(const void* x, void* y, int64_t n, hipStream_t s);
 void vcx_gelu_bwd(const void* x, const void* dy, void* dx, int64_t n, hipStream_t s);
 void vcx_swiglu_fwd(const void* gu, void* y, int64_t R, int F, hipStream_t s);
diff --git a/distributedvolunteercomputing_amd/ops/__init__.py b/distributedvolunteercomputing_amd/ops/__init__.py
--- a/distributedvolunteercomputing_amd/ops/__init__.py
+++ b/distributedvolunteercomputing_amd/ops/__init__.py
@@ -1,4 +1,5 @@
 from ._lib import available as native_available, native
+from ._deferred import ColsumPool, deferred_colsums
 from .activations import bias_gelu, gelu, swiglu
 from .attention import causal_attention, fused_bias_grad_ok, gqa_attention
 from .embedding import embed
diff --git a/distributedvolunteercomputing_amd/ops/_deferred.py b/distributedvolunteercomputing_amd/ops/_deferred.py
--- /dev/null
+++ b/distributedvolunteercomputing_amd/ops/_deferred.py
@@ -0,0 +1,101 @@
+from __future__ import annotations
+
+import contextlib
+
+import torch
+
+from .. import config
+from ._lib import native
+
+_ACTIVE: list = []
+
+
+class ColsumPool:
+
+    def __init__(self):
+        self._bufs: list[torch.Tensor] = []
+        self._next = 0
+        self._round_open = False
+        self._jobs: list[tuple[torch.Tensor, torch.Tensor, bool, bool]] = []
+        self._outs: set[int] = set()
+        self._stage: torch.Tensor | None = None
+        self.launches = 0
+
+    def _begin(self):
+        if self._round_open:
+            return
+        if self._jobs:
+            self.finish()
+        self._round_open = True
+        self._next = 0
+
+        def _end():
+            self._round_open = False
+
+        torch.autograd.Variable._execution_engine.queue_callback(_end)
+
+    def partials(self, shape, device, zero: bool = False) -> torch.Tensor:
+        self._begin()
+        k = self._next
+        self._next += 1
+        shape = tuple(int(s) for s in shape)
+        buf = self._bufs[k] if k < len(self._bufs) else None
+        if buf is None or tuple(buf.shape) != shape or buf.device != device:
+            buf = (torch.zeros if zero else torch.empty)(shape, device=device, dtype=torch.float32)
+            if k < len(self._bufs):
+                self._bufs[k] = buf
+            else:
+                self._bufs.append(buf)
+        return buf
+
+    def nbytes(self) -> int:
+        return sum(b.numel() * 4 for b in self._bufs)
+
+    def stage_nbytes(self) -> int:
+        return 0 if self._stage is None else self._stage.numel() * 4
+
+    def register(self, part: torch.Tensor, out: torch.Tensor, accumulate: bool = True, zero_src: bool = False):
+        self._begin()
+        if out.data_ptr() in self._outs:
+            self.finish()
+        self._outs.add(out.data_ptr())
+        self._jobs.append((part, out, bool(accumulate), bool(zero_src)))
+
+    def pending(self) -> int:
+        return len(self._jobs)
+
+    def finish(self) -> int:
+        jobs, self._jobs = self._jobs, []
+        self._outs = set()
+        self.launches = 0
+        if not jobs:
+            return 0
+        C = native()
+        jobs.sort(key=lambda j: j[1].numel())
+        need = C.colsum_finish_stage_floats([j[1].numel() for j in jobs])
+        dev = jobs[0][0].device
+        if self._stage is None or self._stage.numel() < need or self._stage.device != dev:
+            self._stage = torch.empty(need, device=dev, dtype=torch.float32)
+        self.launches = int(C.colsum_finish_many([j[0] for j in jobs], [j[1] for j in jobs], [j[2] for j in jobs],
+                                                 [j[3] for j in jobs], self._stage))
+        return self.launches
+
+
+_DEFAULT = ColsumPool()
+
+
+def active() -> ColsumPool | None:
+    if _ACTIVE and config.get().colsum_defer:
+        return _ACTIVE[-1]
+    return None
+
+
+@contextlib.contextmanager
+def deferred_colsums(pool: ColsumPool | None = None):
+    pool = _DEFAULT if pool is None else pool
+    _ACTIVE.append(pool)
+    try:
+        yield pool
+    finally:
+        _ACTIVE.pop()
+        pool.finish()
diff --git a/distributedvolunteercomputing_amd/ops/attention.py b/distributedvolunteercomputing_amd/ops/attention.py
--- a/distributedvolunteercomputing_amd/ops/attention.py
+++ b/distributedvolunteercomputing_amd/ops/attention.py
@@ -5,6 +5,7 @@
 import torch
 import torch.nn.functional as F
 
+from . import _deferred
 from ._lib import grad_buffer, native, use_native
 
 
@@ -26,6 +27,13 @@
         if bias is None or not ctx.needs_input_grad[2]:
             return C.attn_bwd(qkv, out, dout.contiguous(), lse, ctx.scale), None, None
         gb = grad_buffer(bias)
+        pool = _deferred.active()
+        if pool is not None and gb is not None:
+            B, T = qkv.shape[0], qkv.shape[1]
+            part = pool.partials((C.attn_bias_partials(B, T), bias.numel()), qkv.device)
+            dqkv = C.attn_bwd_bias(qkv, out, dout.contiguous(), lse, ctx.scale, gb, part, True)[0]
+            pool.register(part, gb.view(-1), accumulate=True)
+            return dqkv, None, None
         dqkv, db = C.attn_bwd_bias(qkv, out, dout.contiguous(), lse, ctx.scale, gb)
         return dqkv, None, (None if gb is not None else db.view_as(bias))
 
diff --git a/distributedvolunteercomputing_amd/ops/linear.py b/distributedvolunteercomputing_amd/ops/linear.py
--- a/distributedvolunteercomputing_amd/ops/linear.py
+++ b/distributedvolunteercomputing_amd/ops/linear.py
@@ -5,6 +5,7 @@
 
 
 from .. import config
+from . import _deferred
 from ._lib import grad_buffer, native, use_native
 
 MIN_ROWS_PER_SPLIT = 2048
@@ -357,7 +358,7 @@
                 dx = gemm_f(dy2, transpose_weight(w) if wt is None else wt).view(x.shape)
             elif narrow_gemm_ok(dy2.shape[0], K, N, dy2):
                 dx = narrow_gemm(dy2, transpose_weight(w) if wt is None else wt).view(x.shape)
-            elif dgrad_ps_ok(dy2.shape[0], K, N, dy2):
+            elif dgrad_ps_ok(dy2.shape[0], K, N, dy2) and not (wt is not None and config.get().dgrad_nt_attn):
                 dx = torch.empty(dy2.shape[0], K, device=dy2.device, dtype=dy2.dtype)
                 native().gemm_ps(dy2, transpose_weight(w) if wt is None else wt, dx)
                 dx = dx.view(x.shape)
@@ -439,7 +440,11 @@
         dy2 = dy.reshape(-1, dy.shape[-1]).contiguous()
         M, F_ = pre.shape
         gb = grad_buffer(b1) if ctx.needs_input_grad[2] else None
-        cs = _colsum_buffer(F_, dy.device) if gb is not None else torch.zeros(F_, device=dy.device, dtype=torch.float32)
+        pool = _deferred.active() if gb is not None else None
+        if pool is not None:
+            cs = pool.partials((F_,), dy.device, zero=True)
+        else:
+            cs = _colsum_buffer(F_, dy.device) if gb is not None else torch.zeros(F_, device=dy.device, dtype=torch.float32)
         dpre = torch.empty_like(pre)
         w1t = ctx.w1t
         w2t = transpose_weight(w2) if ctx.w2t is None else ctx.w2t
@@ -451,7 +456,9 @@
         dw1, _ = _param_grads(dpre, x2, w1, None, ctx.needs_input_grad[1], False)
         db1 = None
         if ctx.needs_input_grad[2]:
-            if gb is not None:
+            if pool is not None:
+                pool.register(cs, gb, accumulate=True, zero_src=True)
+            elif gb is not None:
                 C.add_f32_into_bf16(cs, gb, True, True)
             else:
                 db1 = cs.to(b1.dtype)
diff --git a/distributedvolunteercomputing_amd/ops/norm.py b/distributedvolunteercomputing_amd/ops/norm.py
--- a/distributedvolunteercomputing_amd/ops/norm.py
+++ b/distributedvolunteercomputing_amd/ops/norm.py
@@ -2,6 +2,7 @@
 
 import torch
 
+from . import _deferred
 from ._lib import grad_buffer, native, use_native
 
 
@@ -50,6 +51,16 @@
         dres = None if dx_res is None else dx_res.contiguous()
         pw, pbias, pbb = ctx.params
         gw, gb, gbb = grad_buffer(pw), grad_buffer(pbias) if ctx.has_bias else None, grad_buffer(pbb) if ctx.has_bb else None
+        pool = _deferred.active()
+        if pool is not None and gw is not None and (gb is not None) == ctx.has_bias and (gbb is not None) == ctx.has_bb:
+            outs = [g for g in (gw, gb, gbb) if g is not None]
+            Cw = x.shape[-1]
+            parts = pool.partials((len(outs), C.ln_bwd_partials(x.numel() // Cw, Cw), Cw), x.device)
+            dx = C.ln_bwd(dy.contiguous(), x, w, mean, rstd, dres, ctx.has_bias, ctx.rms, ctx.has_bb, gw, gb, gbb,
+                          parts, True)[0]
+            for k, g in enumerate(outs):
+                pool.register(parts[k], g, accumulate=True)
+            return dx, (dx if ctx.has_b else None), None, None, None, None, None
         dx, dw, dbias, dbb = C.ln_bwd(dy.contiguous(), x, w, mean, rstd, dres, ctx.has_bias, ctx.rms, ctx.has_bb,
                                       gw, gb, gbb)
         dw = None if gw is not None else dw
diff --git a/distributedvolunteercomputing_amd/parallel/local_sgd.py b/distributedvolunteercomputing_amd/parallel/local_sgd.py
--- a/distributedvolunteercomputing_amd/parallel/local_sgd.py
+++ b/distributedvolunteercomputing_amd/parallel/local_sgd.py
@@ -91,6 +91,7 @@
         self.delta = torch.zeros(n, dtype=cfg.comm_dtype, device=self.device)
         self.outer_mom = torch.zeros(n, dtype=torch.float32, device=self.device) if cfg.outer_momentum > 0 else None
         self.ostate = ops.new_ostate(self.device, cfg.lr)
+        self._colsums = ops.ColsumPool()
         self.membership = membership
         self.group = membership.group if membership is not None else group
         self.compressor = compressor
@@ -111,7 +112,8 @@
     def forward_backward(self, x, y):
         self.flat.zero_grad()
         loss = self.model(x, y)
-        loss.backward()
+        with ops.deferred_colsums(self._colsums):
+            loss.backward()
         return loss
 
     def optimizer_step(self):
```

Measured after the change: 1124 samples/s (median of 6 runs). 1.01x the previous value.
